# HamidGadirov/OpticalFlowSciVis

Measured on AMD Instinct MI355X. Metric: volume-pairs/sec, Flow-3D unsupervised train step (fwd+loss+bwd+AdamW), higher is better.
Workload: dtype f32

## Files before the change

### include/flowsci_hip.h

```cpp
#ifndef FLOWSCI_HIP_H
#define FLOWSCI_HIP_H

#ifdef __cplusplus
extern "C" {
#endif

typedef void* fs_stream_t;

enum {
  FS_OK = 0,
  FS_ERR_NULLPTR = 1,
  FS_ERR_SHAPE = 2,
  FS_ERR_ARG = 3,
  FS_ERR_LAUNCH = 4,
  FS_ERR_UNSUPPORTED = 5
};

#define FS_ABI_VERSION 460
int fs_version(void);
const char* fs_error_string(int code);

int fs_warp3d_fwd(const float* in, const float* flow, float* out,
                  int B, int C, const int* in_dhw, int D, int H, int W, fs_stream_t stream);
int fs_warp3d_bwd(const float* in, const float* flow, const float* grad_out,
                  float* grad_in, float* grad_flow,
                  int B, int C, const int* in_dhw, int D, int H, int W, fs_stream_t stream);

int fs_warp3d_pair_fwd(const float* img0, const float* img1, const float* flow6,
                       float* out0, float* out1,
                       int B, int C, const int* in_dhw, int D, int H, int W, fs_stream_t stream);
int fs_warp3d_pair_bwd(const float* img0, const float* img1, const float* flow6,
                       const float* grad_out0, const float* grad_out1,
                       float* grad_img0, float* grad_img1, float* grad_flow6,
                       int B, int C, const int* in_dhw, int D, int H, int W, fs_stream_t stream);
int fs_warp3d_pair_bwd_acc(const float* img0, const float* img1, const float* flow6,
                           const float* grad_out0, const float* grad_out1,
                           float* grad_img0, float* grad_img1,
                           const float* grad_flow_add, float* grad_flow6,
                           int B, int C, const int* in_dhw, int D, int H, int W, fs_stream_t stream);

int fs_upsample_warp3d_pair_fwd(const float* img0, const float* img1, const float* delta,
                                const float* prev_flow, float* flow_out, float* out0, float* out1,
                                int B, int C, const int* in_dhw, int Ds, int Hs, int Ws, int factor,
                                float scale, fs_stream_t stream);
int fs_upsample_warp3d_pair_bwd(const float* img0, const float* img1, const float* flow6,
                                const float* grad_out0, const float* grad_out1,
                                const float* grad_flow_add, float* grad_flow_total, float* grad_delta,
                                float* ws, int B, int C, const int* in_dhw, int Ds, int Hs, int Ws,
                                int factor, float scale, fs_stream_t stream);
int fs_warp3d_pair_bwd_acc3(const float* img0, const float* img1, const float* flow6,
                            const float* grad_out0, long long gout_batch_stride0, const float* grad_out1,
                            long long gout_batch_stride1, float* grad_img0, float* grad_img1,
                            const float* add0, long long batch_stride0, const float* add1, long long batch_stride1,
                            const float* add2, long long batch_stride2, float* grad_flow6,
                            int B, int C, const int* in_dhw, int D, int H, int W, fs_stream_t stream);
int fs_upsample_warp3d_pair_bwd3(const float* img0, const float* img1, const float* flow6,
                                 const float* grad_out0, long long gout_batch_stride0, const float* grad_out1,
                                 long long gout_batch_stride1, const float* add0, long long batch_stride0, const float* add1, long long batch_stride1,
                                 const float* add2, long long batch_stride2, float* grad_flow_total, float* grad_delta,
                                 float* ws, int B, int C, const int* in_dhw, int Ds, int Hs, int Ws,
                                 int factor, float scale, fs_stream_t stream);

enum { FS_W3_KERNEL_GATHER = 0, FS_W3_KERNEL_RC = 1 };
int fs_warp3d_kernel_id(const float* in0, const float* in1, const float* flow, int B, int C, const int* in_dhw,
                        int D, int H, int W, int backward, int with_grad_in);

enum { FS_WARP2D_RIFE = 0, FS_WARP2D_PWC = 1, FS_WARP2D_PHOTO = 2, FS_WARP2D_DILATED = 3 };

int fs_warp2d_fwd(const float* in, const float* flow, const float* start, float* out,
                  int B, int C, const int* in_hw, int H, int W, int mode, int with_mask,
                  fs_stream_t stream);
int fs_warp2d_bwd(const float* in, const float* flow, const float* start,
                  const float* grad_out, float* grad_in, float* grad_flow,
                  int B, int C, const int* in_hw, int H, int W, int mode, int with_mask,
                  fs_stream_t stream);

int fs_warp2d_pair_fwd(const float* img0, const float* img1, const float* flow4,
                       float* out0, float* out1,
                       int B, int C, const int* in_hw, int H, int W, int mode, fs_stream_t stream);
int fs_warp2d_pair_bwd(const float* img0, const float* img1, const float* flow4,
                       const float* grad_out0, const float* grad_out1,
                       float* grad_img0, float* grad_img1, float* grad_flow4,
                       int B, int C, const int* in_hw, int H, int W, int mode, fs_stream_t stream);

enum { FS_OCC_ALL = 0, FS_OCC_OBJ = 1, FS_OCC_OUT = 2 };
int fs_occ_check2d(const float* flow_f, const float* flow_b, float* occ_f, float* occ_b,
                   int B, int H, int W, float alpha1, float alpha2_over_scale, int mode,
                   fs_stream_t stream);

int fs_corr2d_fwd(const float* f1, const float* f2, float* out,
                  int B, int C, int H, int W, int max_displacement, fs_stream_t stream);
int fs_corr2d_bwd(const float* f1, const float* f2, const float* grad_out,
                  float* grad_f1, float* grad_f2,
                  int B, int C, int H, int W, int max_displacement, fs_stream_t stream);

int fs_plane_moments(const float* f, float* stats, int planes, int S, fs_stream_t stream);
int fs_plane_norm_bwd(const float* f, const float* stats, const float* grad_n, float* grad_f,
                      int planes, int S, fs_stream_t stream);
int fs_corr2d_norm_fwd(const float* f1, const float* f2, const float* stats1, const float* stats2,
                       float* out, int B, int C, int H, int W, int max_displacement,
                       fs_stream_t stream);
int fs_corr2d_norm_bwd(const float* f1, const float* f2, const float* stats1, const float* stats2,
                       const float* grad_out, float* grad_n1, float* grad_n2,
                       int B, int C, int H, int W, int max_displacement, fs_stream_t stream);

int fs_corr2d_pair_fwd(const float* f1a, const float* f2a, const float* f1b, const float* f2b,
                       const float* stats, float* outa, float* outb,
                       int B, int C, int H, int W, int max_displacement, fs_stream_t stream);
int fs_corr2d_pair_bwd(const float* f1a, const float* f2a, const float* f1b, const float* f2b,
                       const float* stats, const float* grad_outa, const float* grad_outb,
                       float* grad_f1a, float* grad_f2a, float* grad_f1b, float* grad_f2b,
                       int B, int C, int H, int W, int max_displacement, fs_stream_t stream);
int fs_plane_moments4(const float* fa, const float* fb, const float* fc, const float* fd, float* stats,
                      int planes, int S, fs_stream_t stream);
int fs_plane_norm_bwd4(const float* fa, const float* fb, const float* fc, const float* fd,
                       const float* stats, const float* grad_na, const float* grad_nb,
                       const float* grad_nc, const float* grad_nd, float* grad_fa, float* grad_fb,
                       float* grad_fc, float* grad_fd, int planes, int S, fs_stream_t stream);

int fs_corr3d_fwd(const float* f1, const float* f2, float* out,
                  int B, int C, int D, int H, int W, int max_displacement, fs_stream_t stream);
int fs_corr3d_bwd(const float* f1, const float* f2, const float* grad_out,
                  float* grad_f1, float* grad_f2,
                  int B, int C, int D, int H, int W, int max_displacement, fs_stream_t stream);

enum { FS_PEN_ABS_ROBUST = 0, FS_PEN_CHARBONNIER = 1, FS_PEN_L1_EPS = 2, FS_PEN_L1 = 3 };
#define FS_REDUCE_BLOCKS 1024

int fs_robust_sum(const float* x, const float* y, const float* w, float* sums, float* ws,
                  int B, int C, int S, int H, int W, int border, int mode, float q, float eps,
                  fs_stream_t stream);
int fs_robust_sum_bwd(const float* x, const float* y, const float* w, const float* coef,
                      float* grad_x, float* grad_y,
                      int B, int C, int S, int H, int W, int border, int mode, float q, float eps,
                      fs_stream_t stream);

int fs_wssim_fwd(const float* x, const float* y, const float* weight, float* sums, float* ws,
                 int B, int C, int H, int W, int use_occ, fs_stream_t stream);
int fs_wssim_bwd(const float* x, const float* y, const float* weight, const float* coef,
                 float* grad_x, float* grad_y, int B, int C, int H, int W, int use_occ,
                 fs_stream_t stream);

int fs_census_dist_fwd(const float* img1, const float* img2, float* dist,
                       int B, int H, int W, int max_distance, fs_stream_t stream);
int fs_census_dist_bwd(const float* img1, const float* img2, const float* grad_dist,
                       float* grad_img1, float* grad_img2,
                       int B, int H, int W, int max_distance, fs_stream_t stream);

int fs_merge_fwd(const float* w0, const float* w1, const float* mask_logit,
                 float* merged, float* sigmoid_out, int B, int C, int S, fs_stream_t stream);
int fs_merge_bwd(const float* w0, const float* w1, const float* mask_logit,
                 const float* grad_merged, const float* grad_sigmoid,
                 float* grad_w0, float* grad_w1, float* grad_mask_logit,
                 int B, int C, int S, fs_stream_t stream);
int fs_distill_fwd(const float* merged_i, const float* merged_tea, const float* gt,
                   const float* flow_i, const float* flow_tea, float* sums, float* ws,
                   int B, int C, int F, int S, fs_stream_t stream);
int fs_distill_bwd(const float* merged_i, const float* merged_tea, const float* gt,
                   const float* flow_i, const float* flow_tea, const float* coef,
                   float* grad_flow_i, int B, int C, int F, int S, fs_stream_t stream);
int fs_distill3_fwd(const float* merged0, const float* merged1, const float* merged2,
                    const float* merged_tea, const float* gt, const float* flow0, const float* flow1,
                    const float* flow2, const float* flow_tea, float* sums, float* ws,
                    int B, int C, int F, int S, fs_stream_t stream);
int fs_distill3_bwd(const float* merged0, const float* merged1, const float* merged2,
                    const float* merged_tea, const float* gt, const float* flow0, const float* flow1,
                    const float* flow2, const float* flow_tea, const float* coef,
                    float* grad_flow0, float* grad_flow1, float* grad_flow2,
                    int B, int C, int F, int S, fs_stream_t stream);

int fs_interp3d_bwd(const float* grad_out, float* grad_in, float* ws, int B, int C,
                    int Din, int Hin, int Win, int Dout, int Hout, int Wout,
                    int factor, int upsample, fs_stream_t stream);
int fs_interp3d_bwd_scaled(const float* grad_out, float* grad_in, float* ws, int B, int C,
                           int Din, int Hin, int Win, int Dout, int Hout, int Wout,
                           int factor, int upsample, float scale, fs_stream_t stream);

int fs_downsample3d_fwd(const float* in, float* out, int B, int C, int Din, int Hin, int Win,
                        int factor, float scale, fs_stream_t stream);
int fs_downsample3d_fwd_ms(const float* const* src, const long long* batch_strides, float* out, int B, int C,
                           int Din, int Hin, int Win, int factor, float scale, fs_stream_t stream);

int fs_resize2d_fwd(const float* in, float* out, int B, int C, int Hin, int Win, int Hout, int Wout,
                    int factor, int upsample, float scale, fs_stream_t stream);
int fs_resize2d_bwd(const float* grad_out, float* grad_in, int B, int C, int Hin, int Win, int Hout,
                    int Wout, int factor, int upsample, float scale, fs_stream_t stream);

int fs_upsample3d_scale_add(const float* small, const float* prev, float* out, int B, int C,
                            int Din, int Hin, int Win, int factor, float scale, fs_stream_t stream);

int fs_laploss2d_sizes(int N, int H, int W, int levels, long long* sgn_floats,
                       long long* ws_fwd_floats, long long* ws_bwd_floats);
int fs_laploss2d_fwd(const float* input, const float* target, float* sgn, float* ws, float* loss,
                     int N, int H, int W, int levels, fs_stream_t stream);
int fs_laploss2d_bwd(const float* sgn, const float* grad_loss, float* ws, float* grad_diff,
                     int N, int H, int W, int levels, fs_stream_t stream);

int fs_laploss3d_sizes(int N, int D, int H, int W, int levels, long long* sgn_floats,
                       long long* ws_fwd_floats, long long* ws_bwd_floats);
int fs_laploss3d_fwd(const float* input, const float* target, float* sgn, float* ws, float* loss,
                     int N, int D, int H, int W, int levels, fs_stream_t stream);
int fs_laploss3d_bwd(const float* sgn, const float* grad_loss, float* ws, float* grad_diff,
                     int N, int D, int H, int W, int levels, fs_stream_t stream);

long long fs_conv3d_fwd_ws_floats(int Cin, int Cout, int kernel);
int fs_conv3d_fwd(const float* x, const float* w, const float* bias, float* y, float* ws,
                  int B, int Cin, int Cout, int Di, int Hi, int Wi, int Do, int Ho, int Wo,
                  int kernel, int stride, int pad, int wmode, fs_stream_t stream);

int fs_conv3d_fwd_add(const float* x, const float* w, const float* bias, const float* addend, float* y,
                      float* ws, int B, int Cin, int Cout, int Di, int Hi, int Wi, int Do, int Ho, int Wo,
                      int kernel, int stride, int pad, int wmode, fs_stream_t stream);
long long fs_conv3d_fwd_dprelu_part_floats(int B, int Cout, int Do, int Ho, int Wo);
long long fs_conv3d_fwd_dprelu_part_floats_k3(int B, int Cout, int Do, int Ho, int Wo);
int fs_conv3d_fwd_dprelu(const float* x, const float* w, const float* act_y, const float* prelu_weight,
                         int num_prelu_weights, float* grad_act_y, float* grad_prelu_weight, float* grad_bias,
                         float* part, float* ws, int B, int Cin, int Cout, int Di, int Hi, int Wi, int Do, int Ho, int Wo,
                         int kernel, int stride, int pad, fs_stream_t stream);
int fs_conv3d_fwd_prelu(const float* x, const float* w, const float* bias, const float* prelu_weight,
                        const float* residual, float* y, float* z, float* ws,
                        int B, int Cin, int Cout, int Di, int Hi, int Wi, int Do, int Ho, int Wo,
                        int kernel, int stride, int pad, int num_prelu_weights, fs_stream_t stream);
int fs_conv3d_tr_prelu(const float* x, const float* w, const float* bias, const float* prelu_weight,
                       float* y, float* z, float* ws,
                       int B, int Cin, int Cout, int Di, int Hi, int Wi, int Dout, int Hout, int Wout,
                       int num_prelu_weights, fs_stream_t stream);
int fs_conv3d_tr_add(const float* x, const float* w, const float* bias, const float* addend, float* y,
                     float* ws, int B, int Cin, int Cout, int Di, int Hi, int Wi,
                     int Dout, int Hout, int Wout, fs_stream_t stream);
long long fs_conv3d_tr_ws_floats(int Cin, int Cout);
int fs_conv3d_tr(const float* x, const float* w, const float* bias, float* y, float* ws,
                 int B, int Cin, int Cout, int Di, int Hi, int Wi, int Dout, int Hout, int Wout,
                 fs_stream_t stream);

#define FS_PRELU_MAX_CHUNKS 64
int fs_prelu_bwd(const float* x, const float* grad_out, const float* weight,
                 float* grad_x, float* grad_weight, float* grad_bias, float* ws,
                 int B, int C, int S, int num_weights, fs_stream_t stream);

int fs_conv3d_wrw(const float* g, const float* src, float* dw, int B, int Cg, int Cs,
                  int Do, int Ho, int Wo, int Di, int Hi, int Wi,
                  int kernel, int stride, int pad, fs_stream_t stream);
enum { FS_WRW_KERNEL_BRICK = 0,
       FS_WRW_KERNEL_DMA = 1,
       FS_WRW_KERNEL_WINO23 = 2,
       FS_WRW_KERNEL_WINO43 = 3,
       FS_WRW_KERNEL_S3 = 4        };
int fs_conv3d_wrw_kernel_id(const float* g, const float* src, int B, int Cg, int Cs,
                            int Do, int Ho, int Wo, int Di, int Hi, int Wi, int kernel, int stride, int pad);

int fs_conv3d_fwd_prelu_ms(const float* const* src, const long long* batch_strides, const float* w, const float* bias,
                           const float* prelu_weight, float* y, float* z, float* ws,
                           int B, int Cin, int Cout, int Di, int Hi, int Wi, int Do, int Ho, int Wo,
                           int kernel, int stride, int pad, int num_prelu_weights, fs_stream_t stream);
int fs_conv3d_wrw_ms(const float* g, const float* const* src, const long long* batch_strides, float* dw,
                     int B, int Cg, int Cs, int Do, int Ho, int Wo, int Di, int Hi, int Wi,
                     int kernel, int stride, int pad, fs_stream_t stream);

long long fs_conv3d_wrw_det_ws_floats(const float* g, const float* src, const float* const* src_planes,
                                      const long long* batch_strides, int B, int Cg, int Cs,
                                      int Do, int Ho, int Wo, int Di, int Hi, int Wi, int kernel, int stride, int pad);
int fs_conv3d_wrw_det(const float* g, const float* src, const float* const* src_planes, const long long* batch_strides,
                      float* dw, float* ws, long long ws_floats, int B, int Cg, int Cs,
                      int Do, int Ho, int Wo, int Di, int Hi, int Wi, int kernel, int stride, int pad,
                      fs_stream_t stream);

typedef struct FsWprepJob {
  const float* w;
  float* ws;
  int kind;
  int total;
  int p[6];
} FsWprepJob;
int fs_conv3d_fwd_wprep_jobs(FsWprepJob* jobs_host, int cap, const float* x, const float* w, float* ws,
                             int B, int Cin, int Cout, int Di, int Hi, int Wi, int Do, int Ho, int Wo,
                             int kernel, int stride, int pad, int wmode);
int fs_conv3d_tr_wprep_jobs(FsWprepJob* jobs_host, int cap, const float* x, const float* w, float* ws, int B, int Cin,
                            int Cout, int Di, int Hi, int Wi, int Dout, int Hout, int Wout, int has_prelu_out);
int fs_conv3d_wprep_batch(const FsWprepJob* jobs_dev, int njobs, fs_stream_t stream);

long long fs_frame_metrics2d_ws_bytes(int N, int C, int H, int W);
long long fs_frame_metrics3d_ws_bytes(int N, int C, int D, int H, int W);
int fs_frame_metrics2d(const float* x, const float* y, int N, int C, int H, int W, double L, double* ws,
                       double* out_sse, double* out_ssim_sum, fs_stream_t stream);
int fs_frame_metrics3d(const float* x, const float* y, int N, int C, int D, int H, int W, double L, double* ws,
                       double* out_sse, double* out_ssim_sum, fs_stream_t stream);

#define FS_FLOW_METRICS_K 13
#define FS_FM_MAX_EPE 5
enum { FS_FLOW_DISP = 0, FS_FLOW_RIFE3D = 1 };
long long fs_flow_metrics2d_ws_bytes(int N, int C, int H, int W);
long long fs_flow_metrics3d_ws_bytes(int N, int C, int D, int H, int W, int convention);
int fs_flow_metrics2d(const float* pred, const float* gt, int N, int C, int H, int W, long long pred_bstride,
                      long long gt_bstride, const unsigned char* valid, const unsigned char* noc, float tau_abs,
                      float tau_rel, float* epe_map, double* ws, double* out, fs_stream_t stream);
int fs_flow_metrics3d(const float* pred, const float* gt, int N, int C, int D, int H, int W, long long pred_bstride,
                      long long gt_bstride, const unsigned char* valid, const unsigned char* noc, int convention,
                      float tau_abs, float tau_rel, float* epe_map, double* ws, double* out, fs_stream_t stream);

#define FS_FLOW_CONSISTENCY_K 13
#define FS_FC_MAX_R 7
enum { FS_FC_NOT_VALID = 0, FS_FC_CONSISTENT = 1, FS_FC_OCCLUDED = 2, FS_FC_OUTGOING = 3, FS_FC_NONFINITE = 4 };
long long fs_flow_consistency2d_ws_bytes(int N, int C, int H, int W);
long long fs_flow_consistency3d_ws_bytes(int N, int C, int D, int H, int W);
int fs_flow_consistency2d(const float* flow_f, const float* flow_b, int N, int C, int H, int W, long long f_bstride,
                          long long b_bstride, const float* img0, const float* img1, const unsigned char* valid,
                          double alpha1, double alpha2, unsigned char* class_map, float* res_map, double* ws,
                          double* out, fs_stream_t stream);
int fs_flow_consistency3d(const float* flow_f, const float* flow_b, int N, int C, int D, int H, int W,
                          long long f_bstride, long long b_bstride, const float* img0, const float* img1,
                          const unsigned char* valid, double alpha1, double alpha2, unsigned char* class_map,
                          float* res_map, double* ws, double* out, fs_stream_t stream);

enum { FS_ADV_ALIVE = 0, FS_ADV_OUT = 1, FS_ADV_NONFINITE = 2 };
enum { FS_ADV_EULER = 0, FS_ADV_RK2 = 1, FS_ADV_RK4 = 2 };
int fs_advect2d(const float* flows, int K, int C, int H, int W, long long flow_sstride, const float* pos_in,
                long long pos_cstride, long long P, float* traj, long long traj_sstride, long long traj_cstride,
                unsigned char* status, int* steps, int method, int substeps, double scale, fs_stream_t stream);
int fs_advect3d(const float* flows, int K, int C, int D, int H, int W, long long flow_sstride, const float* pos_in,
                long long pos_cstride, long long P, float* traj, long long traj_sstride, long long traj_cstride,
                unsigned char* status, int* steps, int method, int substeps, double scale, fs_stream_t stream);

#define FS_FTLE_K 9
#define FS_FTLE_MIN 7
#define FS_FTLE_MAX 8
enum { FS_FTLE_NOT_VALID = 0, FS_FTLE_OK = 1, FS_FTLE_ENDED = 2, FS_FTLE_NONFINITE = 3, FS_FTLE_COLLAPSED = 4 };
long long fs_ftle2d_ws_bytes(int C, int Gh, int Gw);
long long fs_ftle3d_ws_bytes(int C, int Gd, int Gh, int Gw);
int fs_ftle2d(const float* map, long long map_cstride, const unsigned char* status, const unsigned char* valid, int C,
              int Gh, int Gw, const double* inv_h, const double* inv_2h, double inv_T, int accept_out, float* ftle,
              unsigned char* cls, float* cg, double* ws, double* out, fs_stream_t stream);
int fs_ftle3d(const float* map, long long map_cstride, const unsigned char* status, const unsigned char* valid, int C,
              int Gd, int Gh, int Gw, const double* inv_h, const double* inv_2h, double inv_T, int accept_out,
              float* ftle, unsigned char* cls, float* cg, double* ws, double* out, fs_stream_t stream);

enum { FS_VG_DIV = 1, FS_VG_VORT = 2, FS_VG_VMAG = 4, FS_VG_Q = 8, FS_VG_L2 = 16, FS_VG_J = 32, FS_VG_ALL = 63 };
enum { FS_VG_FLAG_Q = 1, FS_VG_FLAG_L2 = 2, FS_VG_FLAG_NONFINITE = 128 };
#define FS_VG_K 20
#define FS_VG_STEPS_PER_LAUNCH 256
long long fs_velgrad2d_ws_bytes(int K, int C, int H, int W);
long long fs_velgrad3d_ws_bytes(int K, int C, int D, int H, int W);
int fs_velgrad2d(const float* flows, int K, int C, int H, int W, long long flow_sstride, const double* inv_h,
                 const double* inv_2h, const double* scale, unsigned fields, float* out, unsigned char* flags,
                 double* ws, double* summary, fs_stream_t stream);
int fs_velgrad3d(const float* flows, int K, int C, int D, int H, int W, long long flow_sstride, const double* inv_h,
                 const double* inv_2h, const double* scale, unsigned fields, float* out, unsigned char* flags,
                 double* ws, double* summary, fs_stream_t stream);

#define FS_REGION_TILE2_H 32
#define FS_REGION_TILE2_W 64
#define FS_REGION_TILE3_D 8
#define FS_REGION_TILE3_H 8
#define FS_REGION_TILE3_W 32
#define FS_REGION_MAX_WEIGHTS 8
#define FS_REGION_STEPS_PER_LAUNCH 32768
#define FS_REGION_FOLLOW_MAX_EXTENT 16777216
enum { FS_REGION_OUT = -1, FS_REGION_TO_BACKGROUND = -2 };
long long fs_label_regions2d_ws_bytes(int K, int H, int W);
long long fs_label_regions3d_ws_bytes(int K, int D, int H, int W);
int fs_label_regions2d(const unsigned char* mask, int K, int H, int W, long long mask_sstride, int require, int reject,
                       int conn, int* labels, int* n_regions, int* status, int* ws, fs_stream_t stream);
int fs_label_regions3d(const unsigned char* mask, int K, int D, int H, int W, long long mask_sstride, int require,
                       int reject, int conn, int* labels, int* n_regions, int* status, int* ws, fs_stream_t stream);
int fs_region_stats2d(const int* labels, const int* rank, const long long* offsets, const float* weights, int K, int F,
                      int H, int W, long long R, long long* count, long long* coord_sum, int* bbox, double* wsum,
                      float* wmin, float* wmax, fs_stream_t stream);
int fs_region_stats3d(const int* labels, const int* rank, const long long* offsets, const float* weights, int K, int F,
                      int D, int H, int W, long long R, long long* count, long long* coord_sum, int* bbox, double* wsum,
                      float* wmin, float* wmax, fs_stream_t stream);
int fs_region_follow2d(const int* labels, const float* flows, int K, int C, int H, int W, long long flow_sstride,
                       int* dst, fs_stream_t stream);
int fs_region_follow3d(const int* labels, const float* flows, int K, int C, int D, int H, int W, long long flow_sstride,
                       int* dst, fs_stream_t stream);

enum { FS_RC_DVR = 0, FS_RC_MIP = 1 };
#define FS_RC_BRICK 8
#define FS_RC_MAX_TF 1024
#define FS_RC_MAX_STEPS 4194304
int fs_brick_range3d(const float* volumes, int K, int D, int H, int W, long long sstride, float* range,
// ... 60 lines not shown
```

### opticalflowscivis_amd/_lib.py

```python
import ctypes
import os

import torch

_HERE = os.path.dirname(os.path.abspath(__file__))
PRODUCT_LIB_PATH = os.path.join(_HERE, "csrc", "libflowsci_hip.so")
LIB_PATH = os.environ.get("FLOWSCI_HIP_LIBRARY") or PRODUCT_LIB_PATH
ABLATION = LIB_PATH != PRODUCT_LIB_PATH


def ablation_env(name):
    return os.environ.get(name) if ABLATION else None


def switches():
    return {"library": "ablation build: " + LIB_PATH if ABLATION else "product",
            "env": {k: v for k, v in sorted(os.environ.items()) if k.startswith("FLOWSCI_")}}

ABI_VERSION = 460

_f32p = ctypes.c_void_p
_int = ctypes.c_int
_uint = ctypes.c_uint
_float = ctypes.c_float
_stream = ctypes.c_void_p
_intp = ctypes.POINTER(ctypes.c_int)
_i64p = ctypes.POINTER(ctypes.c_longlong)
_i64 = ctypes.c_longlong
_ptrv = ctypes.POINTER(ctypes.c_void_p)
_double = ctypes.c_double
_f64p = ctypes.POINTER(ctypes.c_double)

class FsWprepJob(ctypes.Structure):
    _fields_ = [("w", ctypes.c_void_p), ("ws", ctypes.c_void_p), ("kind", ctypes.c_int), ("total", ctypes.c_int),
                ("p", ctypes.c_int * 6)]


_jobp = ctypes.POINTER(FsWprepJob)

SIGNATURES = {
    "fs_version": [],
    "fs_error_string": [_int],
    "fs_warp3d_fwd": [_f32p] * 3 + [_int, _int, _intp, _int, _int, _int, _stream],
    "fs_warp3d_bwd": [_f32p] * 5 + [_int, _int, _intp, _int, _int, _int, _stream],
    "fs_warp3d_pair_fwd": [_f32p] * 5 + [_int, _int, _intp, _int, _int, _int, _stream],
    "fs_warp3d_pair_bwd": [_f32p] * 8 + [_int, _int, _intp, _int, _int, _int, _stream],
    "fs_warp3d_pair_bwd_acc": [_f32p] * 9 + [_int, _int, _intp, _int, _int, _int, _stream],
    "fs_warp3d_pair_bwd_acc3": [_f32p] * 3 + [_f32p, _i64, _f32p, _i64] + [_f32p] * 2 + [_f32p, _i64, _f32p, _i64, _f32p, _i64, _f32p, _int, _int, _intp, _int, _int,
                                _int, _stream],
    "fs_upsample_warp3d_pair_bwd3": [_f32p] * 3 + [_f32p, _i64, _f32p, _i64] + [_f32p, _i64, _f32p, _i64, _f32p, _i64] + [_f32p] * 3 +
                                    [_int, _int, _intp, _int, _int, _int, _int, _float, _stream],
    "fs_upsample_warp3d_pair_fwd": [_f32p] * 7 + [_int, _int, _intp, _int, _int, _int, _int, _float, _stream],
    "fs_upsample_warp3d_pair_bwd": [_f32p] * 9 + [_int, _int, _intp, _int, _int, _int, _int, _float, _stream],
    "fs_warp2d_pair_fwd": [_f32p] * 5 + [_int, _int, _intp, _int, _int, _int, _stream],
    "fs_warp2d_pair_bwd": [_f32p] * 8 + [_int, _int, _intp, _int, _int, _int, _stream],
    "fs_interp3d_bwd_scaled": [_f32p] * 3 + [_int] * 10 + [_float, _stream],
    "fs_downsample3d_fwd": [_f32p] * 2 + [_int] * 6 + [_float, _stream],
    "fs_downsample3d_fwd_ms": [_ptrv, _i64p, _f32p] + [_int] * 6 + [_float, _stream],
    "fs_resize2d_fwd": [_f32p] * 2 + [_int] * 8 + [_float, _stream],
    "fs_resize2d_bwd": [_f32p] * 2 + [_int] * 8 + [_float, _stream],
    "fs_occ_check2d": [_f32p] * 4 + [_int] * 3 + [_float, _float, _int, _stream],
    "fs_laploss2d_sizes": [_int] * 4 + [_i64p] * 3,
    "fs_laploss2d_fwd": [_f32p] * 5 + [_int] * 4 + [_stream],
    "fs_laploss2d_bwd": [_f32p] * 4 + [_int] * 4 + [_stream],
    "fs_laploss3d_sizes": [_int] * 5 + [_i64p] * 3,
    "fs_laploss3d_fwd": [_f32p] * 5 + [_int] * 5 + [_stream],
    "fs_laploss3d_bwd": [_f32p] * 4 + [_int] * 5 + [_stream],
    "fs_conv3d_fwd_ws_floats": [_int] * 3,
    "fs_conv3d_fwd": [_f32p] * 5 + [_int] * 13 + [_stream],
    "fs_upsample3d_scale_add": [_f32p] * 3 + [_int] * 6 + [_float, _stream],
    "fs_conv3d_fwd_dprelu_part_floats": [_int] * 5,
    "fs_conv3d_fwd_dprelu_part_floats_k3": [_int] * 5,
    "fs_conv3d_fwd_dprelu": [_f32p] * 4 + [_int] + [_f32p] * 5 + [_int] * 12 + [_stream],
    "fs_conv3d_fwd_prelu": [_f32p] * 8 + [_int] * 13 + [_stream],
    "fs_conv3d_fwd_add": [_f32p] * 6 + [_int] * 13 + [_stream],
    "fs_conv3d_tr_prelu": [_f32p] * 7 + [_int] * 10 + [_stream],
    "fs_conv3d_tr_add": [_f32p] * 6 + [_int] * 9 + [_stream],
    "fs_conv3d_tr_ws_floats": [_int] * 2,
    "fs_conv3d_tr": [_f32p] * 5 + [_int] * 9 + [_stream],
    "fs_plane_moments": [_f32p] * 2 + [_int] * 2 + [_stream],
    "fs_plane_norm_bwd": [_f32p] * 4 + [_int] * 2 + [_stream],
    "fs_corr2d_norm_fwd": [_f32p] * 5 + [_int] * 5 + [_stream],
    "fs_corr2d_norm_bwd": [_f32p] * 7 + [_int] * 5 + [_stream],
    "fs_corr2d_pair_fwd": [_f32p] * 7 + [_int] * 5 + [_stream],
    "fs_corr2d_pair_bwd": [_f32p] * 11 + [_int] * 5 + [_stream],
    "fs_plane_moments4": [_f32p] * 5 + [_int] * 2 + [_stream],
    "fs_plane_norm_bwd4": [_f32p] * 13 + [_int] * 2 + [_stream],
    "fs_corr2d_fwd": [_f32p] * 3 + [_int] * 5 + [_stream],
    "fs_corr2d_bwd": [_f32p] * 5 + [_int] * 5 + [_stream],
    "fs_robust_sum": [_f32p] * 5 + [_int] * 7 + [_float, _float, _stream],
    "fs_robust_sum_bwd": [_f32p] * 6 + [_int] * 7 + [_float, _float, _stream],
    "fs_census_dist_fwd": [_f32p] * 3 + [_int] * 4 + [_stream],
    "fs_census_dist_bwd": [_f32p] * 5 + [_int] * 4 + [_stream],
    "fs_merge_fwd": [_f32p] * 5 + [_int] * 3 + [_stream],
    "fs_merge_bwd": [_f32p] * 8 + [_int] * 3 + [_stream],
    "fs_distill3_fwd": [_f32p] * 11 + [_int] * 4 + [_stream],
    "fs_distill3_bwd": [_f32p] * 13 + [_int] * 4 + [_stream],
    "fs_distill_fwd": [_f32p] * 7 + [_int] * 4 + [_stream],
    "fs_distill_bwd": [_f32p] * 7 + [_int] * 4 + [_stream],
    "fs_interp3d_bwd": [_f32p] * 3 + [_int] * 10 + [_stream],
    "fs_prelu_bwd": [_f32p] * 7 + [_int] * 4 + [_stream],
    "fs_corr3d_fwd": [_f32p] * 3 + [_int] * 6 + [_stream],
    "fs_corr3d_bwd": [_f32p] * 5 + [_int] * 6 + [_stream],
    "fs_conv3d_wrw": [_f32p] * 3 + [_int] * 12 + [_stream],
    "fs_conv3d_wrw_kernel_id": [_f32p] * 2 + [_int] * 12,
    "fs_warp3d_kernel_id": [_f32p] * 3 + [_int, _int, _intp] + [_int] * 5,
    "fs_conv3d_wrw_det_ws_floats": [_f32p, _f32p, _ptrv, _i64p] + [_int] * 12,
    "fs_conv3d_wrw_det": [_f32p, _f32p, _ptrv, _i64p, _f32p, _f32p, _i64] + [_int] * 12 + [_stream],
    "fs_conv3d_fwd_prelu_ms": [_ptrv, _i64p] + [_f32p] * 6 + [_int] * 13 + [_stream],
    "fs_conv3d_wrw_ms": [_f32p, _ptrv, _i64p, _f32p] + [_int] * 12 + [_stream],
    "fs_wssim_fwd": [_f32p] * 5 + [_int] * 5 + [_stream],
    "fs_wssim_bwd": [_f32p] * 6 + [_int] * 5 + [_stream],
    "fs_conv3d_fwd_wprep_jobs": [_jobp, _int, _f32p, _f32p, _f32p] + [_int] * 13,
    "fs_conv3d_tr_wprep_jobs": [_jobp, _int, _f32p, _f32p, _f32p] + [_int] * 10,
    "fs_conv3d_wprep_batch": [_f32p, _int, _stream],
    "fs_warp2d_fwd": [_f32p, _f32p, _f32p, _f32p, _int, _int, _intp, _int, _int, _int, _int, _stream],
    "fs_warp2d_bwd": [_f32p, _f32p, _f32p, _f32p, _f32p, _f32p, _int, _int, _intp, _int, _int, _int, _int,
                      _stream],
    "fs_frame_metrics2d_ws_bytes": [_int] * 4,
    "fs_frame_metrics3d_ws_bytes": [_int] * 5,
    "fs_frame_metrics2d": [_f32p] * 2 + [_int] * 4 + [_double] + [_f32p] * 3 + [_stream],
    "fs_frame_metrics3d": [_f32p] * 2 + [_int] * 5 + [_double] + [_f32p] * 3 + [_stream],
    "fs_flow_metrics2d_ws_bytes": [_int] * 4,
    "fs_flow_metrics3d_ws_bytes": [_int] * 6,
    "fs_flow_metrics2d": [_f32p] * 2 + [_int] * 4 + [_i64] * 2 + [_f32p] * 2 + [_float] * 2 + [_f32p] * 3 + [_stream],
    "fs_flow_metrics3d": [_f32p] * 2 + [_int] * 5 + [_i64] * 2 + [_f32p] * 2 + [_int] + [_float] * 2 + [_f32p] * 3 +
                         [_stream],
    "fs_flow_consistency2d_ws_bytes": [_int] * 4,
    "fs_flow_consistency3d_ws_bytes": [_int] * 5,
    "fs_flow_consistency2d": [_f32p] * 2 + [_int] * 4 + [_i64] * 2 + [_f32p] * 3 + [_double] * 2 + [_f32p] * 4 + [_stream],
    "fs_flow_consistency3d": [_f32p] * 2 + [_int] * 5 + [_i64] * 2 + [_f32p] * 3 + [_double] * 2 + [_f32p] * 4 + [_stream],
    "fs_advect2d": [_f32p, _int, _int, _int, _int, _i64, _f32p, _i64, _i64, _f32p, _i64, _i64, _f32p, _f32p, _int, _int,
                    _double, _stream],
    "fs_advect3d": [_f32p, _int, _int, _int, _int, _int, _i64, _f32p, _i64, _i64, _f32p, _i64, _i64, _f32p, _f32p, _int,
                    _int, _double, _stream],
    "fs_ftle2d_ws_bytes": [_int] * 3,
    "fs_ftle3d_ws_bytes": [_int] * 4,
    "fs_ftle2d": [_f32p, _i64, _f32p, _f32p] + [_int] * 3 + [_f64p, _f64p, _double, _int] + [_f32p] * 5 + [_stream],
    "fs_ftle3d": [_f32p, _i64, _f32p, _f32p] + [_int] * 4 + [_f64p, _f64p, _double, _int] + [_f32p] * 5 + [_stream],
    "fs_velgrad2d_ws_bytes": [_int] * 4,
    "fs_velgrad3d_ws_bytes": [_int] * 5,
    "fs_velgrad2d": [_f32p] + [_int] * 4 + [_i64, _f64p, _f64p, _f64p, _uint] + [_f32p] * 4 + [_stream],
    "fs_velgrad3d": [_f32p] + [_int] * 5 + [_i64, _f64p, _f64p, _f64p, _uint] + [_f32p] * 4 + [_stream],
    "fs_label_regions2d_ws_bytes": [_int] * 3,
    "fs_label_regions3d_ws_bytes": [_int] * 4,
    "fs_label_regions2d": [_f32p] + [_int] * 3 + [_i64] + [_int] * 3 + [_f32p] * 4 + [_stream],
    "fs_label_regions3d": [_f32p] + [_int] * 4 + [_i64] + [_int] * 3 + [_f32p] * 4 + [_stream],
    "fs_region_stats2d": [_f32p] * 4 + [_int] * 4 + [_i64] + [_f32p] * 6 + [_stream],
    "fs_region_stats3d": [_f32p] * 4 + [_int] * 5 + [_i64] + [_f32p] * 6 + [_stream],
    "fs_region_follow2d": [_f32p] * 2 + [_int] * 4 + [_i64, _f32p, _stream],
    "fs_region_follow3d": [_f32p] * 2 + [_int] * 5 + [_i64, _f32p, _stream],
    "fs_brick_range3d": [_f32p] + [_int] * 4 + [_i64, _f32p, _f32p, _stream],
    "fs_raycast3d_ws_bytes": [_int] * 4,
    "fs_raycast3d": [_f32p] + [_int] * 4 + [_i64, _f32p, _f32p, _int, _double, _double, _double, _f64p, _int, _double,
                     _int, _int] + [_f32p] * 5 + [_stream],
    "fs_iso3d_ws_bytes": [_int] * 4,
    "fs_iso_count3d": [_f32p] + [_int] * 4 + [_i64, _double, _f32p, _stream],
    "fs_iso_emit3d": [_f32p] + [_int] * 4 + [_i64, _double, _f64p, _f32p, _f32p, _i64, _i64, _f32p, _int] + [_f32p] * 5 +
                     [_stream],
    "fs_lic2d_ws_bytes": [_int] * 3,
    "fs_lic3d_ws_bytes": [_int] * 4,
    "fs_lic2d": [_f32p, _int, _int, _int, _int, _i64, _f32p, _i64, _f32p, _int, _double, _double, _int, _f32p, _f32p, _f32p,
                 _f32p, _stream],
    "fs_lic3d": [_f32p, _int, _int, _int, _int, _int, _i64, _f32p, _i64, _f32p, _int, _double, _double, _int, _f32p, _f32p,
                 _f32p, _f32p, _stream],
    "fs_triplet_gather": [_f32p, _int, _i64, _int, _int, _int, _f32p, _int, _int, _int, _int, _f32p, _stream],
    "fs_series_stats_ws_bytes": [_int, _i64],
    "fs_series_stats": [_f32p, _int, _int, _i64, _f32p, _f32p, _stream],
    "fs_series_encode_ws_bytes": [_int] * 5,
    "fs_series_encode": [_f32p] + [_int] * 5 + [_f32p] + [_int] * 4 + [_float, _float, _f32p, _f32p, _stream],
    "fs_census3d_dist_fwd": [_f32p] * 3 + [_int] * 5 + [_stream],
    "fs_census3d_dist_bwd": [_f32p] * 5 + [_int] * 5 + [_stream],
    "fs_flow_smooth3d_fwd": [_f32p] * 4 + [_int] * 5 + [_float] * 3 + [_stream],
    "fs_flow_smooth3d_bwd": [_f32p] * 4 + [_int] * 5 + [_float] * 3 + [_stream],
}
_RESTYPES = {"fs_error_string": ctypes.c_char_p, "fs_conv3d_fwd_ws_floats": ctypes.c_longlong,
             "fs_conv3d_wrw_det_ws_floats": ctypes.c_longlong,
             "fs_frame_metrics2d_ws_bytes": ctypes.c_longlong, "fs_frame_metrics3d_ws_bytes": ctypes.c_longlong,
             "fs_flow_metrics2d_ws_bytes": ctypes.c_longlong, "fs_flow_metrics3d_ws_bytes": ctypes.c_longlong,
             "fs_flow_consistency2d_ws_bytes": ctypes.c_longlong, "fs_flow_consistency3d_ws_bytes": ctypes.c_longlong,
             "fs_ftle2d_ws_bytes": ctypes.c_longlong, "fs_ftle3d_ws_bytes": ctypes.c_longlong,
             "fs_velgrad2d_ws_bytes": ctypes.c_longlong, "fs_velgrad3d_ws_bytes": ctypes.c_longlong,
             "fs_label_regions2d_ws_bytes": ctypes.c_longlong, "fs_label_regions3d_ws_bytes": ctypes.c_longlong,
             "fs_raycast3d_ws_bytes": ctypes.c_longlong, "fs_iso3d_ws_bytes": ctypes.c_longlong,
             "fs_lic2d_ws_bytes": ctypes.c_longlong, "fs_lic3d_ws_bytes": ctypes.c_longlong,
             "fs_series_stats_ws_bytes": ctypes.c_longlong, "fs_series_encode_ws_bytes": ctypes.c_longlong,
             "fs_conv3d_tr_ws_floats": ctypes.c_longlong, "fs_conv3d_fwd_dprelu_part_floats": ctypes.c_longlong,
             "fs_conv3d_fwd_dprelu_part_floats_k3": ctypes.c_longlong}


class FlowsciLibraryError(RuntimeError):
    pass


class FlowsciKernelError(RuntimeError):
    pass


_lib = None


def lib():
    global _lib
    if _lib is not None:
        return _lib
    if not os.path.exists(LIB_PATH):
        raise FlowsciLibraryError(
            "libflowsci_hip.so not found at %s -- build it with "
            "`python -c 'import __graft_entry__ as g; g.build()'` or "
            "`make -C opticalflowscivis_amd/csrc`.  There is no CPU fallback." % LIB_PATH)
    handle = ctypes.CDLL(LIB_PATH)
    for name, argtypes in SIGNATURES.items():
        try:
            fn = getattr(handle, name)
        except AttributeError as e:
            raise FlowsciLibraryError("libflowsci_hip.so does not export %s" % name) from e
        fn.argtypes = argtypes
        fn.restype = _RESTYPES.get(name, _int)
    got = handle.fs_version()
    if got != ABI_VERSION:
        raise FlowsciLibraryError(
            "libflowsci_hip.so at %s reports ABI version %d, this binding was written for %d: argument lists "
            "differ between them (include/flowsci_hip.h, FS_ABI_VERSION) -- rebuild with "
            "`make -C opticalflowscivis_amd/csrc`" % (LIB_PATH, got, ABI_VERSION))
    _lib = handle
    return _lib


def check(code, what):
    if code != 0:
        msg = lib().fs_error_string(code)
        raise FlowsciKernelError("%s failed: %s (code %d)" % (what, msg.decode() if msg else "?", code))
```

### opticalflowscivis_amd/convgrad.py

```python
import os

import torch
import torch.nn as nn
import torch.nn.functional as F


def _tuple(v, nd):
    return tuple(v) if isinstance(v, (tuple, list)) else (v,) * nd


_stock_seen = set()


def _note_stock_path(what, x, w, stride, padding):
    if x.dim() != 5 or not x.is_cuda or x.dtype != torch.float32:
        return
    key = (what, tuple(x.shape[1:]), tuple(w.shape), tuple(stride), tuple(padding))
    if key in _stock_seen:
        return
    _stock_seen.add(key)
    import warnings
    warnings.warn("opticalflowscivis_amd: %s of a 3-D convolution runs on stock ATen / MIOpen kernels, not on the HIP "
                  "implicit-GEMM kernels (input %s, weight %s, stride %s, padding %s: unsupported geometry or beyond "
                  "32-bit offsets)" % (what, tuple(x.shape), tuple(w.shape), tuple(stride), tuple(padding)),
# ... 74 lines not shown
    _note_stock_path("the input gradient", gy, w, stride, padding)
    return torch.ops.aten.convolution_backward(
        gy, x, w, None, list(stride), list(padding), [1] * nd, transposed, [0] * nd, 1,
        [True, False, False])[0]


def _conv_grad_weight(x, w, gy, stride, padding, transposed):
    k = tuple(w.shape[2:])
    nd = x.dim() - 2
    src, g = (gy, x) if transposed else (x, gy)
    if nd == 3 and src.is_cuda and src.dtype == torch.float32:
        from . import ops
        if ops.conv3d_wrw_supported(k, stride, padding) and ops.conv3d_wrw_fits(src.shape[2:], g.shape[2:]):
            return ops.conv3d_wrw(g, src, k[0], stride[0], padding[0])
    _note_stock_path("the weight gradient", x, w, stride, padding)
    return torch.ops.aten.convolution_backward(
        gy, x, w, None, list(stride), list(padding), [1] * nd, transposed, [0] * nd, 1,
        [False, True, False])[1]


class _ConvFn(torch.autograd.Function):
    @staticmethod
    def forward(ctx, x, w, b, stride, padding, transposed):
        y = _conv_forward(x, w, b, stride, padding, transposed)
        ctx.save_for_backward(x, w)
        ctx.cfg = (stride, padding, transposed, b is not None)
        return y

    @staticmethod
    def backward(ctx, gy):
        x, w = ctx.saved_tensors
        stride, padding, transposed, has_bias = ctx.cfg
        nd = x.dim() - 2
        gy = gy.contiguous()
        gx = gw = gb = None
        if ctx.needs_input_grad[0]:
            gx = _conv_grad_input(x, w, gy, stride, padding, transposed)
        if ctx.needs_input_grad[1]:
            gw = _conv_grad_weight(x, w, gy, stride, padding, transposed)
        if has_bias and ctx.needs_input_grad[2]:
            gb = gy.sum(dim=(0,) + tuple(range(2, 2 + nd)))
        return gx, gw, gb, None, None, None


class _ConvTrAddFn(torch.autograd.Function):

    @staticmethod
    def forward(ctx, x, w, b, addend, stride, padding):
        from . import ops
        y = ops.conv3d_tr(x, w, b, None, None, addend)
        ctx.save_for_backward(x, w)
        ctx.cfg = (stride, padding, b is not None)
        return y

    @staticmethod
    def backward(ctx, gy):
        x, w = ctx.saved_tensors
        stride, padding, has_bias = ctx.cfg
        gy = gy.contiguous()
        gx = gw = gb = None
        if ctx.needs_input_grad[0]:
            gx = _conv_grad_input(x, w, gy, stride, padding, True)
        if ctx.needs_input_grad[1]:
            gw = _conv_grad_weight(x, w, gy, stride, padding, True)
        if has_bias and ctx.needs_input_grad[2]:
            gb = gy.sum(dim=(0, 2, 3, 4))
        return gx, gw, gb, (gy if ctx.needs_input_grad[3] else None), None, None


class _ConvPReLUFn(torch.autograd.Function):

    @staticmethod
    def forward(ctx, x, w, b, a, stride, padding, transposed):
        y, z = _conv_forward(x, w, b, stride, padding, transposed, a)
        ctx.save_for_backward(x, w, y, a)
        ctx.cfg = (stride, padding, transposed, b is not None)
        return z

    @staticmethod
    def backward(ctx, gz):
        from . import ops
        x, w, y, a = ctx.saved_tensors
        stride, padding, transposed, has_bias = ctx.cfg
        gy, ga, gb = ops.prelu_backward(y, gz.contiguous(), a, want_bias_grad=has_bias)
        gx = gw = None
        if ctx.needs_input_grad[0]:
            gx = _conv_grad_input(x, w, gy, stride, padding, transposed)
        if ctx.needs_input_grad[1]:
            gw = _conv_grad_weight(x, w, gy, stride, padding, transposed)
        return gx, gw, gb, ga, None, None, None


class _ConvPReLUCatFn(torch.autograd.Function):

    @staticmethod
    def forward(ctx, w, b, a, stride, padding, *pieces):
        from . import ops
        k = w.shape[2]
        res = ops.conv3d_fwd_prelu_ms(pieces, w, b, a, k, stride[0], padding[0])
        ctx.ms = res is not None
        if res is None:
            x = torch.cat(pieces, 1)
            y, z = _conv_forward(x, w, b, stride, padding, False, a)
            ctx.save_for_backward(w, y, a, x)
        else:
            y, z = res
            ctx.save_for_backward(w, y, a, *pieces)
        ctx.cfg = (stride, padding, b is not None, [int(t.shape[1]) for t in pieces])
        return z

    @staticmethod
    def backward(ctx, gz):
        from . import ops
        w, y, a = ctx.saved_tensors[:3]
        src = ctx.saved_tensors[3:]
        stride, padding, has_bias, splits = ctx.cfg
        gy, ga, gb = ops.prelu_backward(y, gz.contiguous(), a, want_bias_grad=has_bias)
        need = ctx.needs_input_grad[5:]
        gx = None
        if any(need):
            k3 = tuple(w.shape[2:])
            hip = _hip_tr_ok(gy, w.shape[1], k3, stride, padding) and all(
                n in (2 * m, 2 * m + 1) for n, m in zip(src[0].shape[2:], gy.shape[2:]))
            gx = _conv_grad_input(src[0] if (hip or not ctx.ms) else torch.cat(src, 1), w, gy, stride, padding, False)
        gw = None
        if ctx.needs_input_grad[0]:
            if ctx.ms:
                gw = ops.conv3d_wrw_ms(gy, src, w.shape[2], stride[0], padding[0])
                if gw is None:
                    gw = _conv_grad_weight(torch.cat(src, 1), w, gy, stride, padding, False)
            else:
                gw = _conv_grad_weight(src[0], w, gy, stride, padding, False)
        gp = [None] * len(splits)
        if gx is not None:
            gp = [g if n else None for g, n in zip(gx.split(splits, 1), need)]
        return (gw, gb, ga, None, None) + tuple(gp)


def conv_prelu_cat(block, pieces):
    conv, act = block[0], block[1]
    x0 = pieces[0]
    if _ab_env("FLOWSCI_CONV0_CAT") == "1":
        return None
    if not (_hip_autograd(x0) and x0.dim() == 5 and x0.dtype == torch.float32 and isinstance(conv, Conv3d)
            and act.weight.numel() in (1, conv.out_channels) and conv.groups == 1
            and _tuple(conv.dilation, 3) == (1, 1, 1) and conv.padding_mode == "zeros"
            and tuple(conv.weight.shape[2:]) == (4, 4, 4) and _tuple(conv.stride, 3) == (2, 2, 2)
            and sum(int(t.shape[1]) for t in pieces) == conv.in_channels <= 12 and conv.out_channels <= 32):
        return None
    return _ConvPReLUCatFn.apply(conv.weight, conv.bias, act.weight, _tuple(conv.stride, 3), _tuple(conv.padding, 3),
                                 *pieces)


class _HeadFn(torch.autograd.Function):

    @staticmethod
    def forward(ctx, x, w1, b1, a1, w2, b2, addend):
        from . import ops
        y1, z1 = ops.conv3d_tr(x, w1, b1, None, a1)
        out = ops.conv3d_tr(z1, w2, b2, None, None, addend)
        ctx.save_for_backward(x, w1, a1, y1, z1, w2)
        ctx.has = (b1 is not None, b2 is not None, addend is not None)
        return out

    @staticmethod
    def backward(ctx, gout):
        from . import ops
        x, w1, a1, y1, z1, w2 = ctx.saved_tensors
        s3, p3 = (2, 2, 2), (1, 1, 1)
        gout = gout.contiguous()
        gw2 = _conv_grad_weight(z1, w2, gout, s3, p3, True) if ctx.needs_input_grad[4] else None
        gb2 = gout.sum(dim=(0, 2, 3, 4)) if (ctx.has[1] and ctx.needs_input_grad[5]) else None
        fused = ops.conv3d_deconv_grad_input_dprelu(gout, w2, y1, a1)
        if fused is not None:
            gy1, ga1, gb1 = fused
        else:
            gz1 = _conv_grad_input(z1, w2, gout, s3, p3, True)
            gy1, ga1, gb1 = ops.prelu_backward(y1, gz1, a1, want_bias_grad=ctx.has[0])
        if not ctx.has[0]:
            gb1 = None
        gw1 = _conv_grad_weight(x, w1, gy1, s3, p3, True) if ctx.needs_input_grad[1] else None
        gx = _conv_grad_input(x, w1, gy1, s3, p3, True) if ctx.needs_input_grad[0] else None
        return gx, gw1, gb1, ga1, gw2, gb2, (gout if (ctx.has[2] and ctx.needs_input_grad[6]) else None)


def head_fused_ok(head, x, addend):
    d1, act, d2 = head[0], head[1], head[2]
    if not (_hip_autograd(x) and x.dim() == 5 and x.dtype == torch.float32 and isinstance(d1, ConvTranspose3d)
            and isinstance(d2, ConvTranspose3d) and isinstance(act, nn.PReLU)):
        return False
    for d in (d1, d2):
        if not (_tuple(d.kernel_size, 3) == (4, 4, 4) and _tuple(d.stride, 3) == (2, 2, 2) and _tuple(d.padding, 3) == (1, 1, 1)
                and d.groups == 1 and _tuple(d.dilation, 3) == (1, 1, 1) and _tuple(d.output_padding, 3) == (0, 0, 0)):
            return False
    if act.weight.numel() not in (1, d1.out_channels):
        return False
    if not (_hip_tr_ok(x, d1.out_channels, (4, 4, 4), (2, 2, 2), (1, 1, 1))):
        return False
    mid = tuple(2 * n for n in x.shape[2:])
    from . import ops
    return ops.conv3d_tr_supported(d2.out_channels, (4, 4, 4), (2, 2, 2), (1, 1, 1)) and ops.conv3d_tr_fits(mid) and \
        (addend is None or (addend.is_cuda and addend.dtype == torch.float32))


_FUSE_2D = _ab_env("FLOWSCI_CONV2D_UNFUSED") != "1"


class ConvPReLU(nn.Sequential):

    def forward(self, x):
        conv, act = self[0], self[1]
        nd = x.dim() - 2
        kinds = {3: (Conv3d, ConvTranspose3d), 2: (nn.Conv2d, nn.ConvTranspose2d) if _FUSE_2D else ()}.get(nd, ())
        if (_hip_autograd(x) and x.dtype == torch.float32 and kinds and isinstance(conv, kinds)
                and act.weight.numel() in (1, conv.out_channels) and conv.groups == 1
                and _tuple(conv.dilation, nd) == (1,) * nd and getattr(conv, "padding_mode", "zeros") == "zeros"
                and _tuple(getattr(conv, "output_padding", 0), nd) == (0,) * nd):
            return _ConvPReLUFn.apply(x, conv.weight, conv.bias, act.weight, _tuple(conv.stride, nd),
                                      _tuple(conv.padding, nd), isinstance(conv, kinds[1]))
        return act(conv(x))


class _ResUnitFn(torch.autograd.Function):

    @staticmethod
    def forward(ctx, x, w1, b1, a1, w2, b2, a2):
        from . import ops
        k, p = w1.shape[2], (w1.shape[2] - 1) // 2
        y1, z1 = ops.conv3d_fwd(x, w1, b1, k, 1, p, 0, a1)
        y2, out = ops.conv3d_fwd(z1, w2, b2, k, 1, p, 0, a2, x)
        ctx.save_for_backward(x, w1, a1, y1, z1, w2, a2, y2)
        ctx.has_bias = (b1 is not None, b2 is not None)
        return out

    @staticmethod
    def backward(ctx, gout):
        from . import ops
        x, w1, a1, y1, z1, w2, a2, y2 = ctx.saved_tensors
        k, p = w1.shape[2], (w1.shape[2] - 1) // 2
        s3, p3 = (1, 1, 1), (p, p, p)
        gout = gout.contiguous()
        gy2, ga2, gb2 = ops.prelu_backward(y2, gout, a2, want_bias_grad=ctx.has_bias[1])
        gw2 = _conv_grad_weight(z1, w2, gy2, s3, p3, False) if ctx.needs_input_grad[4] else None
        fused = ops.conv3d_k3_grad_input_dprelu(gy2, w2, y1, a1) if k == 3 else None
        if fused is not None:
            gy1, ga1, gb1 = fused
            if not ctx.has_bias[0]:
                gb1 = None
        else:
            gz1 = ops.conv3d_fwd(gy2, w2, None, k, 1, p, 1)
            gy1, ga1, gb1 = ops.prelu_backward(y1, gz1, a1, want_bias_grad=ctx.has_bias[0])
        gw1 = _conv_grad_weight(x, w1, gy1, s3, p3, False) if ctx.needs_input_grad[1] else None
        gx = ops.conv3d_fwd(gy1, w1, None, k, 1, p, 1, None, gout) if ctx.needs_input_grad[0] else None
        return gx, gw1, gb1, ga1, gw2, gb2, ga2


def res_unit(block, x):
    ok = (_hip_autograd(x) and x.dim() == 5 and x.dtype == torch.float32 and len(block) == 2 and
          all(isinstance(m, ConvPReLU) and isinstance(m[0], Conv3d) and isinstance(m[1], nn.PReLU) for m in block))
    if ok:
        for m in block:
            c = m[0]
            kk = tuple(c.weight.shape[2:])
            ok = ok and (kk == (3, 3, 3) and _tuple(c.stride, 3) == (1, 1, 1) and _tuple(c.padding, 3) == (1, 1, 1)
                         and c.groups == 1 and _tuple(c.dilation, 3) == (1, 1, 1) and c.padding_mode == "zeros"
                         and c.in_channels == c.out_channels == x.shape[1]
                         and m[1].weight.numel() in (1, c.out_channels)
                         and _hip_fwd_ok(x, c.out_channels, x.shape[2:], kk, (1, 1, 1), (1, 1, 1)))
    if not ok:
        return block(x) + x
    (c1, p1), (c2, p2) = block[0], block[1]
    return _ResUnitFn.apply(x, c1.weight, c1.bias, p1.weight, c2.weight, c2.bias, p2.weight)


def _hip_autograd(x):
    return x.is_cuda and torch.is_grad_enabled()


class Conv3d(nn.Conv3d):
    def forward(self, x):
        if not _hip_autograd(x):
            st, pd, k = _tuple(self.stride, 3), _tuple(self.padding, 3), tuple(self.weight.shape[2:])
            if x.dim() == 5 and self.padding_mode == "zeros" and self.groups == 1 and _tuple(self.dilation, 3) == (1, 1, 1) \
                    and _hip_fwd_ok(x, self.weight.shape[0], [_conv_out(n, kk, s, p) for n, kk, s, p in
                                                              zip(x.shape[2:], k, st, pd)], k, st, pd):
                from . import ops
                return ops.conv3d_fwd(x, self.weight, None if self.bias is None else self.bias.detach(),
                                      k[0], st[0], pd[0], 0)
            return super().forward(x)
        return _ConvFn.apply(x, self.weight, self.bias, _tuple(self.stride, 3), _tuple(self.padding, 3), False)


class ConvTranspose3d(nn.ConvTranspose3d):
    def _plain(self):
        return (self.groups == 1 and _tuple(self.dilation, 3) == (1, 1, 1) and
                _tuple(self.output_padding, 3) == (0, 0, 0))

    def forward(self, x, addend=None):
        st, pd, k = _tuple(self.stride, 3), _tuple(self.padding, 3), tuple(self.weight.shape[2:])
        hip = x.dim() == 5 and self._plain() and _hip_tr_ok(x, self.weight.shape[1], k, st, pd)
        if addend is not None:
            if hip and tuple(addend.shape[2:]) == tuple(2 * n for n in x.shape[2:]) and \
                    addend.shape[1] == self.weight.shape[1] and addend.dtype == torch.float32:
                if _hip_autograd(x):
                    return _ConvTrAddFn.apply(x, self.weight, self.bias, addend, st, pd)
                from . import ops
# ... 19 lines not shown
```

### opticalflowscivis_amd/csrc/convfwd.hip

```cpp
#include <cstdint>
#include <cstdlib>
#include <type_traits>

#include "common.hpp"

namespace {

typedef float f32x16 __attribute__((ext_vector_type(16)));

struct FP {
  int B, Cin, Cout, CoutP;
  int Di, Hi, Wi, Do, Ho, Wo;
  int pad;
  int tz, ty, tx;
  long long tiles;
  const float* slope;
  float* Z;
  int nslope;
  const float* addend;
  const float* dy;
  const float* dslope;
  int dnslope;
  float* dpart;
  int nsrc;
// ... 244 lines not shown
#pragma unroll
    for (int k = 0; k < NXW; ++k) {
      const int i = 256 * (wv + 4 * k) + 4 * lane;
      const int c = i / CHS, r1 = i - c * CHS;
      const int z = r1 / PS, r2 = r1 - z * PS;
      const int y = r2 / XP, x = r2 - y * XP;
      const int gz = gz0 + z, gy = gy0 + y, gx = gx0 + x;
      const bool ok = i < NX && gz >= 0 && gz < p.Di && gy >= 0 && gy < p.Hi && gx >= 0 && gx < p.Wi;
      xoff[k] = ok ? (((unsigned)gz * p.Hi + gy) * p.Wi + gx) * 4u : DMA_OOB;
      xch[k] = i < NX ? c : CI - 1;
    }
#pragma unroll
    for (int k = 0; k < NWW; ++k) {
      const int i = 256 * (wv + 4 * k) + 4 * lane;
      const int row = i / CP, j = i - row * CP;
      woff[k] = i < NW ? ((unsigned)row * (unsigned)p.CoutP + (unsigned)j) * 4u : DMA_OOB;
    }
    auto stage = [&](int c0, int buf) {
      __amdgpu_buffer_rsrc_t rx[CI];
#pragma unroll
      for (int c = 0; c < CI; ++c) {
        const int ch = c0 + c;
        const bool live = ch < p.Cin;
        const int chc = live ? ch : 0;
        const float* base = p.nsrc ? p.src[chc] + (size_t)b * (size_t)p.sbs[chc]
                                   : X + ((size_t)b * p.Cin + chc) * xvol;
        rx[c] = __builtin_amdgcn_make_buffer_rsrc((void*)base, (short)0, live ? (int)((unsigned)xvol * 4u) : 0, 0x00020000);
      }
      __amdgpu_buffer_rsrc_t rw = __builtin_amdgcn_make_buffer_rsrc(
          (void*)(Wt + (size_t)c0 * K3 * p.CoutP + co0), (short)0, 0x7fffffff, 0x00020000);
      float* base = lds + buf * BUF;
#pragma unroll
      for (int k = 0; k < NXW; ++k)
        if (256 * (wv + 4 * k) < NXL) {
#pragma unroll
          for (int c = 0; c < CI; ++c)
            if (256 * (wv + 4 * k) < (c + 1) * CHS && 256 * (wv + 4 * k) + 256 > c * CHS)
              if (xch[k] == c)
                __builtin_amdgcn_raw_ptr_buffer_load_lds(rx[c], (lds_ptr_t)(base + 256 * (wv + 4 * k)), 16, xoff[k], 0, 0, 0);
        }
#pragma unroll
      for (int k = 0; k < NWW; ++k)
        if (256 * (wv + 4 * k) < NWL)
          __builtin_amdgcn_raw_ptr_buffer_load_lds(rw, (lds_ptr_t)(base + NXL + 256 * (wv + 4 * k)), 16, woff[k], 0, 0, 0);
    };
    stage(0, 0);
    asm volatile("s_waitcnt vmcnt(0)" ::: "memory");
    __builtin_amdgcn_s_barrier();
    int buf = 0;
    for (int c0 = 0; c0 < p.Cin; c0 += CI) {
      if (c0 + CI < p.Cin) stage(c0 + CI, buf ^ 1);
      asm volatile("s_waitcnt vmcnt(0)" ::: "memory");
      __builtin_amdgcn_s_barrier();
      buf ^= 1;
    }
#else
    (void)xvol; (void)NXW; (void)NWW; (void)DMA_OOB;
#endif
    return;
  }

  const int ly = col / TW, lx = col % TW;
  const int rr0 = wv * NT;
  const int wz = rr0 / TY, wy = rr0 % TY;
  const int bBo = kh * (CI / 2) * CHS + (wz * S) * PS + ((wy * R + ly) * S) * XP + lx * S + XL - p.pad;
  const int aBo = NXL + kh * (CI / 2) * K3 * CP + col;

  f32x16 acc[MT][NT];
#pragma unroll
  for (int m = 0; m < MT; ++m)
#pragma unroll
    for (int n = 0; n < NT; ++n)
#pragma unroll
      for (int r = 0; r < 16; ++r) acc[m][n][r] = 0.f;

  __builtin_amdgcn_s_barrier();
  int buf = 0;
  for (int c0 = 0; c0 < p.Cin; c0 += CI) {
    const float* bB = lds + buf * BUF + bBo;
    const float* aB = lds + buf * BUF + aBo;
    auto lds_ops = [&](int j, float (&a)[MT], float (&bq)[NT]) {
      const int cl = j / K3, tap = j - cl * K3;
      const int kz = tap / (K * K), ky = (tap / K) % K, kx = tap % K;
#pragma unroll
      for (int m = 0; m < MT; ++m) a[m] = aB[(cl * K3 + tap) * CP + m * 32];
#pragma unroll
      for (int n = 0; n < NT; ++n) bq[n] = bB[cl * CHS + kz * PS + (ky + n * R * S) * XP + kx];
    };
    auto mma = [&](const float (&a)[MT], const float (&bq)[NT]) {
#pragma unroll
      for (int n = 0; n < NT; ++n)
#pragma unroll
        for (int m = 0; m < MT; ++m)
          acc[m][n] = __builtin_amdgcn_mfma_f32_32x32x2f32(a[m], bq[n], acc[m][n], 0, 0, 0);
    };
    float a0[MT], b0[NT], a1[MT], b1[NT];
    lds_ops(0, a0, b0);
#pragma unroll
    for (int j = 0; j < NP; j += 2) {
      if (j + 1 < NP) lds_ops(j + 1, a1, b1);
      __builtin_amdgcn_sched_barrier(0);
#ifdef FS_ABLATION
      if (p.ab & 8) continue;
#endif
      mma(a0, b0);
      if (j + 2 < NP) lds_ops(j + 2, a0, b0);
      __builtin_amdgcn_sched_barrier(0);
      if (j + 1 < NP) mma(a1, b1);
    }
    __builtin_amdgcn_s_barrier();
    buf ^= 1;
  }

#include "convfwd_epilogue.hpp"
}

#ifdef FS_ABLATION
#include "convwino.hpp"
#include "convwino4.hpp"
#endif
#include "convwino2d.hpp"
#include "convfwd_s3.hpp"

template <int K, int S, int CI, int MT, int NT, int TZ, int TY, int TW>
int launch_ws(const float* X, const float* Wt, const float* bias, float* Y, FP& p, hipStream_t st) {
  constexpr int TYR = TY * (32 / TW);
  p.tz = fs::cdiv(p.Do, TZ); p.ty = fs::cdiv(p.Ho, TYR); p.tx = fs::cdiv(p.Wo, TW);
  p.tiles = (long long)p.B * p.tz * p.ty * p.tx;
  const int mgroups = p.CoutP / (32 * MT);
  if (p.tiles >= (1ll << 31) || mgroups > 65535) return FS_ERR_SHAPE;
#ifdef FS_ABLATION
  static const int fwd_ab = (int)FS_AB_ENV_LL("FLOWSCI_FWD_AB", 0);
  p.ab = fwd_ab;
#endif
  hipLaunchKernelGGL((conv3d_fwd_ws_kernel<K, S, CI, MT, NT, TZ, TY, TW>), dim3((unsigned)p.tiles, mgroups),
                     dim3(512), 0, st, X, Wt, bias, Y, p);
  FS_LAUNCH_CHECK();
  return FS_OK;
}

template <int K, int S, int CI, int MT, int NT, int TZ, int TY, int TW>
int launch(const float* X, const float* Wt, const float* bias, float* Y, FP& p, hipStream_t st) {
  constexpr int TYR = TY * (32 / TW);
  p.tz = fs::cdiv(p.Do, TZ); p.ty = fs::cdiv(p.Ho, TYR); p.tx = fs::cdiv(p.Wo, TW);
  p.tiles = (long long)p.B * p.tz * p.ty * p.tx;
  const int mgroups = p.CoutP / (32 * MT);
  if (p.tiles >= (1ll << 31) || mgroups > 65535) return FS_ERR_SHAPE;
  hipLaunchKernelGGL((conv3d_fwd_kernel<K, S, CI, MT, NT, TZ, TY, TW>), dim3((unsigned)p.tiles, mgroups),
                     dim3(256), 0, st, X, Wt, bias, Y, p);
  FS_LAUNCH_CHECK();
  return FS_OK;
}

constexpr int kFinishBlocks = 128;
__global__ __launch_bounds__(256) void dprelu_finish1_kernel(const float* __restrict__ part, int rows, int CP,
                                                             double* __restrict__ partial) {
  const int CP2 = 2 * CP;
  const int col = threadIdx.x % CP2, sub = threadIdx.x / CP2, nsub = 256 / CP2;
  const int chunk = (rows + kFinishBlocks - 1) / kFinishBlocks;
  const int r0 = blockIdx.x * chunk, r1 = min(rows, r0 + chunk);
  const float* src = part + (size_t)blockIdx.y * rows * CP2;
  double s = 0.0;
  for (int r = r0 + sub; r < r1; r += nsub) s += (double)src[(size_t)r * CP2 + col];
  __shared__ double red[256];
  red[threadIdx.x] = s;
  __syncthreads();
  if (sub == 0) {
    double t = red[col];
    for (int k = 1; k < nsub; ++k) t += red[k * CP2 + col];
    partial[((size_t)blockIdx.y * kFinishBlocks + blockIdx.x) * CP2 + col] = t;
  }
}
__global__ __launch_bounds__(64) void dprelu_finish2_kernel(const double* __restrict__ partial, int CP, int Cout,
                                                            float* __restrict__ ga, float* __restrict__ gb, int nslope) {
  const bool bias_blk = (int)blockIdx.x >= nslope;
  const int c = bias_blk ? blockIdx.x - nslope : blockIdx.x;
  const bool all = !bias_blk && nslope == 1 && Cout != 1;
  const int c_lo = all ? 0 : c, c_hi = all ? Cout : c + 1;
  double s = 0.0;
  for (int cc = c_lo; cc < c_hi; ++cc) {
    const double* src = partial + (size_t)(cc / CP) * kFinishBlocks * 2 * CP + (cc % CP) * 2 + (bias_blk ? 1 : 0);
    for (int g = threadIdx.x; g < kFinishBlocks; g += 64) s += src[(size_t)g * 2 * CP];
  }
  __shared__ double red[64];
  red[threadIdx.x] = s;
  __syncthreads();
  for (int st = 32; st > 0; st >>= 1) {
    if ((int)threadIdx.x < st) red[threadIdx.x] += red[threadIdx.x + st];
    __syncthreads();
  }
  if (threadIdx.x == 0) (bias_blk ? gb : ga)[c] = (float)red[0];
}

void wt_dims(int Cin, int Cout, int kernel, int* CinP, int* CoutP) {
  const int ci = (kernel == 3) ? 4 : 2;
  *CinP = (Cin + ci - 1) / ci * ci;
  *CoutP = (Cout <= 32 && kernel == 4) ? 32 : (Cout + 63) / 64 * 64;
}

}

extern "C" long long fs_conv3d_fwd_ws_floats(int Cin, int Cout, int kernel) {
  if (Cin < 1 || Cout < 1 || (kernel != 3 && kernel != 4)) return -1;
  int cinp, coutp;
  wt_dims(Cin, Cout, kernel, &cinp, &coutp);
  const long long direct = (long long)cinp * kernel * kernel * kernel * coutp;
  constexpr int wino_uch = FS_WINO2D_UCH > FS_WINO4_UCH ? FS_WINO2D_UCH : (FS_WINO4_UCH > FS_WINO_UCH ? FS_WINO4_UCH : FS_WINO_UCH);
  const long long wino = (kernel == 3 && coutp == 64) ? (long long)cinp * wino_uch : 0;
  const long long s3 = (kernel == 4 && coutp <= 64) ? s3_slab_words(Cin, coutp) : 0;
  const long long m = direct > wino ? direct : wino;
  return m > s3 ? m : s3;
}

struct DPrelu {
  const float* act_y = nullptr;
  const float* slope = nullptr;
  int nslope = 0;
  float* part = nullptr;
  float* ga = nullptr;
  float* gb = nullptr;
};

struct MultiSrc {
  const float* const* src;
  const long long* batch_strides;
};

static int conv3d_fwd_impl(const float* x, const float* w, const float* bias, const float* slope, int nslope,
                           const float* addend, float* y, float* z, float* ws, int B, int Cin, int Cout, int Di, int Hi, int Wi, int Do,
                           int Ho, int Wo, int kernel, int stride, int pad, int wmode, fs_stream_t stream,
                           const DPrelu* dp = nullptr, const MultiSrc* ms = nullptr, WprepPlan* plan = nullptr) {
  if (ms == nullptr && plan == nullptr) FS_REQUIRE_PTR(x);
  if (plan == nullptr) FS_REQUIRE_PTR(y);
  FS_REQUIRE_PTR(ws);
  if (z != nullptr && (slope == nullptr || (nslope != 1 && nslope != Cout))) return FS_ERR_ARG;
  if ((((uintptr_t)y | (uintptr_t)z | (uintptr_t)addend | (uintptr_t)(dp ? dp->act_y : nullptr)) & 15) != 0) return FS_ERR_ARG;
  if (B < 1 || Cin < 1 || Cout < 1 || Di < 1 || Hi < 1 || Wi < 1 || Do < 1 || Ho < 1 || Wo < 1)
    return FS_ERR_SHAPE;
  if (!((kernel == 3 && stride == 1) || (kernel == 4 && stride == 2)) || pad < 0 || pad >= kernel ||
      (wmode != 0 && wmode != 1))
    return FS_ERR_ARG;
  if (Do != (Di + 2 * pad - kernel) / stride + 1 || Ho != (Hi + 2 * pad - kernel) / stride + 1 ||
      Wo != (Wi + 2 * pad - kernel) / stride + 1)
    return FS_ERR_SHAPE;
  if ((long long)Di * Hi * Wi >= (1ll << 31) || (long long)Do * Ho * Wo >= (1ll << 31)) return FS_ERR_SHAPE;
  if ((long long)(kernel == 3 ? 4 : 2) * Di * Hi * Wi * 4 >= (1ll << 32)) return FS_ERR_SHAPE;
  FP p;
  p.B = B; p.Cin = Cin; p.Cout = Cout; p.Di = Di; p.Hi = Hi; p.Wi = Wi; p.Do = Do; p.Ho = Ho; p.Wo = Wo;
  p.pad = pad;
  p.slope = slope; p.Z = z; p.nslope = nslope; p.addend = addend;
  p.dy = dp ? dp->act_y : nullptr; p.dslope = dp ? dp->slope : nullptr; p.dnslope = dp ? dp->nslope : 0;
  p.dpart = dp ? dp->part : nullptr;
  p.nsrc = 0;
  bool ms_aligned = true;
  if (ms != nullptr) {
    if (Cin > 12) return FS_ERR_UNSUPPORTED;
    p.nsrc = Cin;
    const long long vol = (long long)Di * Hi * Wi;
    for (int c = 0; c < Cin; ++c) {
      if (ms->src[c] == nullptr) return FS_ERR_NULLPTR;
      if (ms->batch_strides[c] < vol) return FS_ERR_ARG;
      p.src[c] = ms->src[c]; p.sbs[c] = ms->batch_strides[c];
      ms_aligned = ms_aligned && ((uintptr_t)ms->src[c] & 15) == 0 && ms->batch_strides[c] % 4 == 0;
    }
  }
  int cinp;
  wt_dims(Cin, Cout, kernel, &cinp, &p.CoutP);
  hipStream_t st = (hipStream_t)stream;
  auto dp_finish = [&](int CP, int rows_per_brick = 4) {
    const long long rows = p.tiles * rows_per_brick;
    const int mg = p.CoutP / CP;
    double* partial = reinterpret_cast<double*>(dp->part + (rows * mg * CP * 2 + 1) / 2 * 2);
    hipLaunchKernelGGL(dprelu_finish1_kernel, dim3(kFinishBlocks, mg), dim3(256), 0, st, dp->part, (int)rows, CP, partial);
    hipLaunchKernelGGL(dprelu_finish2_kernel, dim3(dp->nslope + Cout), dim3(64), 0, st, partial, CP, Cout, dp->ga, dp->gb,
                       dp->nslope);
    return hipGetLastError() == hipSuccess ? FS_OK : FS_ERR_LAUNCH;
  };
  const int K3 = kernel * kernel * kernel;
  p.Di = Di; p.Hi = Hi; p.Wi = Wi;
  if (wino2d_ok(p, x, ws, Cin, Cout, kernel, stride, ms != nullptr) &&
      (dp == nullptr || (bias == nullptr && z == nullptr && addend == nullptr))) {
    wprep_do(wprep_job(FS_WPREP_WINO2D, w, ws, (long long)cinp * FS_WINO2D_UCH, Cout, Cin, cinp, wmode), plan, st);
    if (plan != nullptr) return FS_OK;
    const int rc = launch_wino2d(x, ws, bias, y, p, st);
    if (rc != FS_OK || dp == nullptr) return rc;
    return dp_finish(64, wino2d_part_rows());
  }
#ifdef FS_ABLATION
  if (wino4_ok(p, x, ws, Cin, Cout, kernel, stride, ms != nullptr) &&
      (dp == nullptr || (bias == nullptr && z == nullptr && addend == nullptr))) {
    wprep_do(wprep_job(FS_WPREP_WINO4, w, ws, (long long)cinp * FS_WINO4_UCH, Cout, Cin, cinp, wmode), plan, st);
    if (plan != nullptr) return FS_OK;
    const int rc = launch_wino4(x, ws, bias, y, p, st);
    if (rc != FS_OK || dp == nullptr) return rc;
    return dp_finish(64);
  }
  if (wino_ok(p, x, ws, Cin, Cout, kernel, stride, ms != nullptr) &&
      (dp == nullptr || (bias == nullptr && z == nullptr && addend == nullptr))) {
    wprep_do(wprep_job(FS_WPREP_WINO, w, ws, (long long)cinp * FS_WINO_UCH, Cout, Cin, cinp, wmode), plan, st);
    if (plan != nullptr) return FS_OK;
    const int rc = launch_wino(x, ws, bias, y, p, st);
    if (rc != FS_OK || dp == nullptr) return rc;
    return dp_finish(64);
  }
#endif
  static const bool no_s3 = FS_AB_ENV("FLOWSCI_FWD_NO_S3");
  if (!no_s3 && kernel == 4 && stride == 2 && pad == 1 && wmode == 0 && (p.CoutP == 32 || p.CoutP == 64) && Wi % 4 == 0 &&
      ms_aligned && (((ms ? (uintptr_t)0 : (uintptr_t)x) | (uintptr_t)ws) & 15) == 0 &&
      (long long)Di * Hi * Wi * 4 < (1ll << 31) &&
      (long long)B * Do * fs::cdiv(Ho, S3_TY) * fs::cdiv(Wo, S3_TW) >= 256 &&
      (dp == nullptr || (p.CoutP == 32 && bias == nullptr && z == nullptr && addend == nullptr))) {
    const int cp = p.CoutP;
    wprep_do(wprep_job(FS_WPREP_S3K4, w, ws, s3_slab_words(Cin, p.CoutP), Cout, Cin, (Cin + 1) / 2, cp, 0, 0), plan, st);
    if (plan != nullptr) return FS_OK;
    int rc;
#ifdef FS_ABLATION
    static const int s3_nlw = (int)FS_AB_ENV_LL("FLOWSCI_S3_NLW", 4);
    if (s3_nlw == 8) rc = p.CoutP == 32 ? launch_s3<1, S3_NMW, 8>(x, ws, bias, y, p, st) : launch_s3<2, S3_NMW, 8>(x, ws, bias, y, p, st);
    else
#endif
    rc = p.CoutP == 32 ? launch_s3<1, S3_NMW, 4>(x, ws, bias, y, p, st) : launch_s3<2, S3_NMW, 4>(x, ws, bias, y, p, st);
    if (rc != FS_OK || dp == nullptr) return rc;
    return dp_finish(32, S3_NMW);
  }
  wprep_do(wprep_job(FS_WPREP_FWD, w, ws, (long long)cinp * K3 * p.CoutP, Cout, Cin, K3, cinp, p.CoutP, wmode), plan, st);
  if (plan != nullptr) return FS_OK;
  static const bool reg_only = FS_AB_ENV("FLOWSCI_FWD_REG");
  const bool ws_ok = !reg_only && Wi % 4 == 0 && Wo > 16 && (((ms ? (uintptr_t)0 : (uintptr_t)x) | (uintptr_t)ws) & 15) == 0 &&
                     ms_aligned && (long long)(kernel == 3 ? 4 : 2) * Di * Hi * Wi * 4 < (1ll << 31);
  if (ms != nullptr && !(kernel == 4 && ws_ok && dp == nullptr)) return FS_ERR_UNSUPPORTED;
  if (kernel == 3) {
    const bool wide = Wo > 16;
    const long long big = (long long)B * fs::cdiv(Do, 2) * fs::cdiv(Ho, wide ? 8 : 16) * fs::cdiv(Wo, wide ? 32 : 16) *
                          (p.CoutP / 64);
    const bool ws3 = !reg_only && Wi % 4 == 0 && (((ms ? (uintptr_t)0 : (uintptr_t)x) | (uintptr_t)ws) & 15) == 0 &&
                     (long long)4 * Di * Hi * Wi * 4 < (1ll << 31);
    if (dp != nullptr && (bias != nullptr || z != nullptr || addend != nullptr || !ws3)) return FS_ERR_UNSUPPORTED;
    int rc = FS_ERR_UNSUPPORTED, cp = 0;
    const long long small = (long long)B * Do * fs::cdiv(Ho, wide ? 4 : 8) * fs::cdiv(Wo, wide ? 32 : 16) * (p.CoutP / 64);
    if (big >= 512) {
      if (ws3 && wide) { rc = launch_ws<3, 1, 4, 2, 4, 2, 8, 32>(x, ws, bias, y, p, st); cp = 64; }
      else if (dp != nullptr) return FS_ERR_UNSUPPORTED;
      else if (wide) return launch<3, 1, 4, 2, 4, 2, 8, 32>(x, ws, bias, y, p, st);
      else return launch<3, 1, 4, 2, 4, 2, 8, 16>(x, ws, bias, y, p, st);
    } else if (small < 256) {
// ... 142 lines not shown
```

### opticalflowscivis_amd/csrc/convtr.hip

```cpp
#include <cstdint>
#include <cstdlib>

#include "common.hpp"

namespace {

typedef float f32x16 __attribute__((ext_vector_type(16)));

struct TP {
  int B, Cin, Cout;
  int CoutT;
  int Di, Hi, Wi;
  int Dout, Hout, Wout;
  int Dq, Hq, Wq;
  int tz, ty, tx;
  long long tiles;
  const float* slope;
  float* Z;
  int nslope;
  const float* addend;
  const float* Ybase;
  long long wslice;
#ifdef FS_ABLATION
  int ab = 0;
#endif
};

__device__ __forceinline__ void tr_slice(TP& p, const float*& Wt, const float*& bias, float*& Y) {
  const int sl = blockIdx.y;
  if (sl == 0) return;
  const size_t off = (size_t)sl * 32 * ((size_t)p.Dout * p.Hout * p.Wout);
  Wt += (size_t)sl * p.wslice;
  if (bias) bias += 32 * sl;
  Y += off;
  if (p.Z) p.Z += off;
  if (p.slope && p.nslope != 1) p.slope += 32 * sl;
  if (p.addend) p.addend += off;
  p.Ybase += off;
}

__device__ __forceinline__ constexpr int tap_d(int p, int a) { return p == 0 ? (a == 0 ? 0 : -1) : (a == 0 ? 1 : 0); }
__device__ __forceinline__ constexpr int tap_k(int p, int a) { return p == 0 ? (a == 0 ? 1 : 3) : (a == 0 ? 0 : 2); }

#include "wprep.hpp"

__device__ __forceinline__ void store8(float* __restrict__ yc, const float (&v)[8], int qz, int qy, int qx,
                                       const TP& p, float* __restrict__ zc = nullptr, float sl = 0.f) {
  const float* __restrict__ ac = p.addend ? p.addend + (yc - p.Ybase) : nullptr;
#pragma unroll
  for (int pz = 0; pz < 2; ++pz)
#pragma unroll
    for (int py = 0; py < 2; ++py) {
      const int z = 2 * qz + pz, y = 2 * qy + py, x = 2 * qx;
      if (z >= p.Dout || y >= p.Hout || x >= p.Wout) continue;
      float* row = yc + ((size_t)z * p.Hout + y) * p.Wout + x;
      float v0 = v[(pz * 2 + py) * 2], v1 = v[(pz * 2 + py) * 2 + 1];
      if (ac != nullptr) {
        const float* arow = ac + (row - yc);
        v0 += arow[0];
        if (x + 1 < p.Wout) v1 += arow[1];
      }
      if ((p.Wout & 1) == 0) {
        *reinterpret_cast<float2*>(row) = make_float2(v0, v1);
      } else {
        row[0] = v0;
        if (x + 1 < p.Wout) row[1] = v1;
      }
      if (zc != nullptr) {
        float* zrow = zc + (row - yc);
        const float z0 = v0 > 0.f ? v0 : sl * v0, z1 = v1 > 0.f ? v1 : sl * v1;
        if ((p.Wout & 1) == 0) {
          *reinterpret_cast<float2*>(zrow) = make_float2(z0, z1);
        } else {
          zrow[0] = z0;
          if (x + 1 < p.Wout) zrow[1] = z1;
        }
      }
    }
}

__device__ __forceinline__ void store8_quad(float* __restrict__ yc, const float (&v)[8], int qz, int qy, int qx, bool ok,
                                            const TP& p, float* __restrict__ zc = nullptr, float sl = 0.f) {
  const float* __restrict__ ac = p.addend ? p.addend + (yc - p.Ybase) : nullptr;
  const bool evn = (qx & 1) == 0;
#pragma unroll
  for (int pz = 0; pz < 2; ++pz) {
    const float a0 = v[(pz * 2 + 0) * 2], a1 = v[(pz * 2 + 0) * 2 + 1];
    const float b0 = v[(pz * 2 + 1) * 2], b1 = v[(pz * 2 + 1) * 2 + 1];
    const float k0 = evn ? a0 : b0, k1 = evn ? a1 : b1;
    const float r0 = __uint_as_float(__builtin_amdgcn_update_dpp(0u, __float_as_uint(evn ? b0 : a0), 0xB1, 0xF, 0xF, false));
    const float r1 = __uint_as_float(__builtin_amdgcn_update_dpp(0u, __float_as_uint(evn ? b1 : a1), 0xB1, 0xF, 0xF, false));
    float4 o = evn ? make_float4(k0, k1, r0, r1) : make_float4(r0, r1, k0, k1);
    const int z = 2 * qz + pz, y = 2 * qy + (evn ? 0 : 1), x0 = 2 * (evn ? qx : qx - 1);
    if (!ok || z >= p.Dout || y >= p.Hout || x0 >= p.Wout) continue;
    float* row = yc + ((size_t)z * p.Hout + y) * p.Wout + x0;
    if (x0 + 3 < p.Wout) {
      if (ac != nullptr) {
        const float4 a4 = *reinterpret_cast<const float4*>(ac + (row - yc));
        o.x += a4.x; o.y += a4.y; o.z += a4.z; o.w += a4.w;
      }
      *reinterpret_cast<float4*>(row) = o;
      if (zc != nullptr)
        *reinterpret_cast<float4*>(zc + (row - yc)) = make_float4(o.x > 0.f ? o.x : sl * o.x, o.y > 0.f ? o.y : sl * o.y,
                                                                  o.z > 0.f ? o.z : sl * o.z, o.w > 0.f ? o.w : sl * o.w);
    } else {
      const float ov[4] = {o.x, o.y, o.z, o.w};
#pragma unroll
      for (int e = 0; e < 4; ++e)
        if (x0 + e < p.Wout) {
          const float w = ov[e] + (ac != nullptr ? ac[(row - yc) + e] : 0.f);
          row[e] = w;
          if (zc != nullptr) zc[(row - yc) + e] = w > 0.f ? w : sl * w;
        }
    }
  }
}

template <int TZ, int TY>
__global__ __launch_bounds__(256, 2) void convtr_mfma_kernel(const float* __restrict__ X,
                                                          const float* __restrict__ Wt_,
                                                          const float* __restrict__ bias_,
                                                          float* __restrict__ Y_, TP p) {
  const float* Wt = Wt_;
  const float* bias = bias_;
  float* Y = Y_;
  tr_slice(p, Wt, bias, Y);
  static_assert(TZ * TY == 4, "one 32-position row per wave");
  constexpr int CI = 4;
  constexpr int ZT = TZ + 2, YT = TY + 2, XT = 34;
  constexpr int PS = YT * XT, CHS = ZT * PS;
  constexpr int NX = CI * CHS, NW = CI * 64 * 32;
  __shared__ float sX[NX];
  __shared__ __attribute__((aligned(16))) float sW[NW];

  const int t = threadIdx.x, lane = t & 63, wv = t >> 6;
  const int col = lane & 31, kh = lane >> 5;
  long long tile = blockIdx.x;
  {
    const long long per = p.tiles / 8;
    if (per > 0 && tile < per * 8) tile = (tile & 7) * per + (tile >> 3);
  }
  const int txi = (int)(tile % p.tx); tile /= p.tx;
  const int tyi = (int)(tile % p.ty); tile /= p.ty;
  const int tzi = (int)(tile % p.tz);
  const int b = (int)(tile / p.tz);
  const int qz0 = tzi * TZ, qy0 = tyi * TY, qx0 = txi * 32;
  const int wz = wv / TY, wy = wv % TY;

  const float* bB = sX + kh * 2 * CHS + (wz + 1) * PS + (wy + 1) * XT + (col + 1);
  const float* aB = sW + kh * 2 * 64 * 32 + col;

  f32x16 acc[8];
#pragma unroll
  for (int c = 0; c < 8; ++c)
#pragma unroll
    for (int r = 0; r < 16; ++r) acc[c][r] = 0.f;

  const size_t xvol = (size_t)p.Di * p.Hi * p.Wi;
  constexpr int ITX = (NX + 255) / 256, ITW = NW / 4 / 256;
  unsigned xoff[ITX];
#pragma unroll
  for (int it = 0; it < ITX; ++it) {
    const int i = t + 256 * it;
    const int c = i / CHS, r1 = i - c * CHS;
    const int z = r1 / PS, r2 = r1 - z * PS;
    const int y = r2 / XT, x = r2 - y * XT;
    const int gz = qz0 - 1 + z, gy = qy0 - 1 + y, gx = qx0 - 1 + x;
    const bool ok = i < NX && gz >= 0 && gz < p.Di && gy >= 0 && gy < p.Hi && gx >= 0 && gx < p.Wi;
    xoff[it] = ok ? ((unsigned)c * (unsigned)xvol + ((unsigned)gz * p.Hi + gy) * p.Wi + gx) * 4u : ~0u;
  }
  float rX[ITX];
  float4 rW[ITW];
  auto fetch = [&](int c0) {
    const char* xb = reinterpret_cast<const char*>(X + ((size_t)b * p.Cin + c0) * xvol);
#pragma unroll
// ... 719 lines not shown
              }
          };
          t3_bf16x8 ba[2][3], bb[2][3];
          load_b(0, ba[0]);
          if (NT > 1) load_b(1, ba[1]);
#pragma unroll
          for (int n = 0; n < NT; n += 4) {
            if (n + 2 < NT) { load_b(n + 2, bb[0]); if (n + 3 < NT) load_b(n + 3, bb[1]); }
            __builtin_amdgcn_sched_barrier(0);
            mma_pair(n, ba[0], ba[1], n + 1 < NT);
            if (n + 2 < NT) {
              if (n + 4 < NT) { load_b(n + 4, ba[0]); if (n + 5 < NT) load_b(n + 5, ba[1]); }
              __builtin_amdgcn_sched_barrier(0);
              mma_pair(n + 2, bb[0], bb[1], n + 3 < NT);
            }
          }
          done = true;
        }
      }
      if (!done) {
        const float* aB = lds + (size_t)(c0 + kq) * WSCI + col;
        float av[8][RT];
#pragma unroll
        for (int d = 0; d < 8; ++d)
#pragma unroll
          for (int rt = 0; rt < RT; ++rt) av[d][rt] = aB[(d * RT + rt) * 16];
        const float* bB = lds + bBo + buf * NXL;
        float xa[2][8], xb[2][8];
        auto load_x = [&](int n, float (&xn)[8]) {
#pragma unroll
          for (int d = 0; d < 8; ++d) xn[d] = bB[16 * n - ((d >> 2) & 1) * PS - ((d >> 1) & 1) * XP - (d & 1)];
        };
        auto mma_pair = [&](int n, const float (&x0)[8], const float (&x1)[8], bool two) {
#pragma unroll
          for (int d = 0; d < 8; ++d)
#pragma unroll
            for (int rt = 0; rt < RT; ++rt) {
              acc[rt][n] = __builtin_amdgcn_mfma_f32_16x16x4f32(av[d][rt], x0[d], acc[rt][n], 0, 0, 0);
              if (two) acc[rt][n + 1] = __builtin_amdgcn_mfma_f32_16x16x4f32(av[d][rt], x1[d], acc[rt][n + 1], 0, 0, 0);
            }
        };
        if constexpr (RT == 6) {
#pragma unroll
          for (int n = 0; n < NT; n += 2) {
            load_x(n, xa[0]);
            if (n + 1 < NT) load_x(n + 1, xa[1]);
            __builtin_amdgcn_sched_barrier(0);
            mma_pair(n, xa[0], xa[1], n + 1 < NT);
            __builtin_amdgcn_sched_barrier(0);
          }
        } else {
          load_x(0, xa[0]);
          if (NT > 1) load_x(1, xa[1]);
#pragma unroll
          for (int n = 0; n < NT; n += 4) {
            if (n + 2 < NT) { load_x(n + 2, xb[0]); if (n + 3 < NT) load_x(n + 3, xb[1]); }
            __builtin_amdgcn_sched_barrier(0);
            mma_pair(n, xa[0], xa[1], n + 1 < NT);
            if (n + 2 < NT) {
              if (n + 4 < NT) { load_x(n + 4, xa[0]); if (n + 5 < NT) load_x(n + 5, xa[1]); }
              __builtin_amdgcn_sched_barrier(0);
              mma_pair(n + 2, xb[0], xb[1], n + 3 < NT);
            }
          }
        }
      }
      TSTAMP(0);
      __builtin_amdgcn_s_barrier();
      TSTAMP(1);
      buf ^= 1;
    }

    const int qz = qz0 + wz, qy = qy0 + wy;
    if (qz <= p.Di && qy <= p.Hi) {
      const size_t yvol = (size_t)p.Dout * p.Hout * p.Wout;
      const bool evn = (col & 1) == 0;
      const int slot = 4 * (kq & 1) + (evn ? 0 : 1) + 2 * (lane >> 5);
#pragma unroll
      for (int rt = 0; rt < RT; ++rt) {
        const int item = 8 * rt + slot;
        const int pzy = item / p.Cout, co = item - pzy * p.Cout;
        const int zo = 2 * qz - (pzy >> 1), yo = 2 * qy - (pzy & 1);
        const bool iok = item < 4 * p.Cout && zo >= 0 && zo < p.Dout && yo >= 0 && yo < p.Hout;
        const float bv = (bias && iok) ? bias[co] : 0.f;
        float* __restrict__ row = Y + (((size_t)b * p.Cout + (iok ? co : 0)) * p.Dout + (iok ? zo : 0)) * ((size_t)p.Hout * p.Wout) +
                                  (size_t)(iok ? yo : 0) * p.Wout;
        const float* __restrict__ arow = p.addend ? p.addend + (row - Y) : nullptr;
        (void)yvol;
        float4 apre[NT];
        if (arow != nullptr) {
#pragma unroll
          for (int n = 0; n < NT; ++n) {
            const int qa = evn ? q0 + 16 * n + col : q0 + 16 * n + col - 1;
            const int x0 = 2 * qa - 1;
            const bool full = iok && qa >= 1 && qa + 1 < qend && x0 + 3 < p.Wout;
            apre[n] = full ? *reinterpret_cast<const float4*>(arow + x0) : make_float4(0.f, 0.f, 0.f, 0.f);
          }
        }
#pragma unroll
        for (int n = 0; n < NT; ++n) {
          const int q = q0 + 16 * n + col;
          const auto s0 = __builtin_amdgcn_permlane32_swap(__float_as_uint(acc[rt][n][0]), __float_as_uint(acc[rt][n][2]),
                                                           false, false);
          const auto s1 = __builtin_amdgcn_permlane32_swap(__float_as_uint(acc[rt][n][1]), __float_as_uint(acc[rt][n][3]),
                                                           false, false);
          const unsigned keep_e = evn ? s0[0] : s1[0], keep_o = evn ? s0[1] : s1[1];
          const unsigned send_e = evn ? s1[0] : s0[0], send_o = evn ? s1[1] : s0[1];
          const float re = __uint_as_float(__builtin_amdgcn_update_dpp(0u, send_e, 0xB1, 0xF, 0xF, false)) + bv;
          const float ro = __uint_as_float(__builtin_amdgcn_update_dpp(0u, send_o, 0xB1, 0xF, 0xF, false)) + bv;
          const float ke = __uint_as_float(keep_e) + bv, ko = __uint_as_float(keep_o) + bv;
          const int qa = evn ? q : q - 1;
          float4 v = evn ? make_float4(ko, ke, ro, re) : make_float4(ro, re, ko, ke);
          if (iok) {
            const int x0 = 2 * qa - 1;
            const bool full = qa >= 1 && qa + 1 < qend && x0 + 3 < p.Wout;
            if (full) {
              if (arow) { v.x += apre[n].x; v.y += apre[n].y; v.z += apre[n].z; v.w += apre[n].w; }
              *reinterpret_cast<float4*>(row + x0) = v;
            } else {
              const float vv[4] = {v.x, v.y, v.z, v.w};
#pragma unroll
              for (int e = 0; e < 4; ++e) {
                const int x = x0 + e, pos = qa + (e >> 1);
                if (pos >= 0 && pos < qend && x >= 0 && x < p.Wout) row[x] = vv[e] + (arow ? arow[x] : 0.f);
              }
            }
          }
        }
      }
    }
    TSTAMP(2);
  }
#ifdef FS_TR_STAMPS
  if (blockIdx.x == 3 && lane == 0) {
    for (int i = 0; i < 8; ++i) fs_tr_dbg[wv * 8 + i] = dt[i];
    fs_tr_dbg[wv * 8 + 7] = (unsigned long long)(t1 - t0);
  }
#endif
}

static int tr_ncu() {
  static int ncu_of[64] = {};
  int dev = 0;
  if (hipGetDevice(&dev) != hipSuccess || dev < 0 || dev >= 64) dev = 0;
  int ncu = ncu_of[dev];
  if (ncu == 0) {
    int n = 0;
    if (hipDeviceGetAttribute(&n, hipDeviceAttributeMultiprocessorCount, dev) != hipSuccess || n < 1) n = 256;
    ncu_of[dev] = ncu = n;
  }
  return ncu;
}

template <int RT, int NT, int CINP = 32>
void launch_p8(const float* x, const float* ws, const float* bias, float* y, const TP& p, hipStream_t st) {
  const int ncu = tr_ncu();
  const long long nwg = p.tiles < ncu ? p.tiles : ncu;
  const int per = (int)((p.tiles + nwg - 1) / nwg);
  const unsigned grid = (unsigned)((p.tiles + per - 1) / per);
  hipLaunchKernelGGL((convtr_p8_kernel<RT, NT, CINP>), dim3(grid), dim3(512), 0, st, x, ws, bias, y, p, per);
}

template <int CO, int NP>
__global__ __launch_bounds__(256) void convtr_valu_kernel(const float* __restrict__ X, const float* __restrict__ W,
                                                          const float* __restrict__ bias, float* __restrict__ Y,
                                                          TP p) {
  const int Hq2 = (p.Hq + NP - 1) / NP;
  const long long nq = (long long)p.B * p.Dq * Hq2 * p.Wq;
  const long long e = (long long)blockIdx.x * 256 + threadIdx.x;
  if (e >= nq) return;
  const int qx = (int)(e % p.Wq);
  long long r = e / p.Wq;
  const int qy = (int)(r % Hq2) * NP; r /= Hq2;
  const int qz = (int)(r % p.Dq);
  const int b = (int)(r / p.Dq);

  constexpr int NY = NP + 2;
  int off[3 * NY * 3];
#pragma unroll
  for (int dz = 0; dz < 3; ++dz)
#pragma unroll
    for (int dy = 0; dy < NY; ++dy)
#pragma unroll
      for (int dx = 0; dx < 3; ++dx) {
        const int z = qz + dz - 1, y = qy + dy - 1, x = qx + dx - 1;
        const bool ok = z >= 0 && z < p.Di && y >= 0 && y < p.Hi && x >= 0 && x < p.Wi;
        off[(dz * NY + dy) * 3 + dx] = ok ? (z * p.Hi + y) * p.Wi + x : -1;
      }

  float acc[NP][CO][8];
#pragma unroll
  for (int co = 0; co < CO; ++co) {
    const float bv = (bias && co < p.Cout) ? bias[co] : 0.f;
#pragma unroll
    for (int q = 0; q < NP; ++q)
#pragma unroll
      for (int c = 0; c < 8; ++c) acc[q][co][c] = bv;
  }
  const size_t xvol = (size_t)p.Di * p.Hi * p.Wi;
  const float* xc = X + (size_t)b * p.Cin * xvol;
  for (int ci = 0; ci < p.Cin; ++ci, xc += xvol) {
    float xn[3 * NY * 3];
#pragma unroll
    for (int i = 0; i < 3 * NY * 3; ++i) xn[i] = off[i] >= 0 ? xc[off[i]] : 0.f;
    const float* wc = W + (size_t)ci * p.Cout * 64;
#pragma unroll
    for (int co = 0; co < CO; ++co) {
      if (co < p.Cout) {
#pragma unroll
        for (int cls = 0; cls < 8; ++cls) {
          const int pz = cls >> 2, py = (cls >> 1) & 1, px = cls & 1;
#pragma unroll
          for (int tp = 0; tp < 8; ++tp) {
            const int a = tp >> 2, bb = (tp >> 1) & 1, c = tp & 1;
            const int kidx = (tap_k(pz, a) * 4 + tap_k(py, bb)) * 4 + tap_k(px, c);
            const float wv = wc[co * 64 + kidx];
#pragma unroll
            for (int q = 0; q < NP; ++q) {
              const int didx = ((tap_d(pz, a) + 1) * NY + (tap_d(py, bb) + 1 + q)) * 3 + (tap_d(px, c) + 1);
              acc[q][co][cls] = fmaf(xn[didx], wv, acc[q][co][cls]);
            }
          }
        }
      }
    }
  }
  const size_t yvol = (size_t)p.Dout * p.Hout * p.Wout;
#pragma unroll
  for (int q = 0; q < NP; ++q)
#pragma unroll
    for (int co = 0; co < CO; ++co)
      if (co < p.Cout && qy + q < p.Hq)
        store8(Y + ((size_t)b * p.Cout + co) * yvol, acc[q][co], qz, qy + q, qx, p,
               p.Z ? p.Z + ((size_t)b * p.Cout + co) * yvol : nullptr, p.Z ? p.slope[p.nslope == 1 ? 0 : co] : 0.f);
}

template <int CO>
void launch_valu(const float* x, const float* w, const float* bias, float* y, const TP& p, hipStream_t st) {
  constexpr int NP = 2;
  const long long nq = (long long)p.B * p.Dq * ((p.Hq + NP - 1) / NP) * p.Wq;
  hipLaunchKernelGGL((convtr_valu_kernel<CO, NP>), dim3((unsigned)((nq + 255) / 256)), dim3(256), 0, st, x, w, bias,
                     y, p);
}

}

#ifdef FS_TR_STAMPS
extern "C" int fs_debug_tr_stamps(unsigned long long* out) {
  return hipMemcpyFromSymbol(out, HIP_SYMBOL(fs_tr_dbg), sizeof(unsigned long long) * 32) == hipSuccess ? 0 : 1;
}
#endif

extern "C" long long fs_conv3d_tr_ws_floats(int Cin, int Cout) {
  if (Cin < 1 || Cout < 1 || (Cout > 32 && (Cout % 32 != 0 || Cout > 128))) return -1;
  const int slices = Cout > 32 ? Cout / 32 : 1;
  if (Cout > 32) Cout = 32;
  const long long cinp = (Cin + 3) / 4 * 4;
  long long p8 = Cout <= 12 ? cinp * p8_ws_ci(Cout <= 2 ? 1 : (Cout <= 6 ? 3 : 6)) : 0;
  if (Cout <= 6 && cinp <= 32 && p8_split_words((int)cinp, Cout <= 2 ? 1 : 3) > p8) p8 = p8_split_words((int)cinp, Cout <= 2 ? 1 : 3);
  long long cls = Cout <= 6 ? 0 : cinp * 64 * (Cout <= 16 ? 16 : 32);
  if (Cout > 16 && t3_slab_words(Cin) > cls) cls = t3_slab_words(Cin);
  if (Cout <= 16 && t3_slab_words16(Cin) > cls) cls = t3_slab_words16(Cin);
  return (p8 > cls ? p8 : cls) * slices;
}

static int conv3d_tr_slice(const float* x, const float* w, const float* bias, const float* slope, int nslope,
                          const float* addend, float* y, float* z, float* ws, int B, int Cin, int Cout, int Di,
                          int Hi, int Wi, int Dout, int Hout, int Wout, fs_stream_t stream, int CoutT = 0, int slices = 1,
                          WprepPlan* plan = nullptr) {
  FS_REQUIRE_PTR(x);
  if (plan == nullptr) FS_REQUIRE_PTR(y);
  if (z != nullptr && (slope == nullptr || (nslope != 1 && nslope != Cout))) return FS_ERR_ARG;
  if (B < 1 || Cin < 1 || Cout < 1 || Di < 1 || Hi < 1 || Wi < 1) return FS_ERR_SHAPE;
  if (Cout > 32) return FS_ERR_ARG;
  if (CoutT == 0) CoutT = Cout;
  if ((Dout != 2 * Di && Dout != 2 * Di + 1) || (Hout != 2 * Hi && Hout != 2 * Hi + 1) ||
      (Wout != 2 * Wi && Wout != 2 * Wi + 1))
    return FS_ERR_SHAPE;
  if ((long long)Di * Hi * Wi >= (1ll << 31) || (long long)Dout * Hout * Wout >= (1ll << 31))
    return FS_ERR_SHAPE;
  if ((long long)4 * Di * Hi * Wi * 4 >= (1ll << 32)) return FS_ERR_SHAPE;
  TP p;
  p.B = B; p.Cin = Cin; p.Cout = Cout; p.CoutT = CoutT; p.Di = Di; p.Hi = Hi; p.Wi = Wi;
  p.Dout = Dout; p.Hout = Hout; p.Wout = Wout;
  p.Dq = (Dout + 1) / 2; p.Hq = (Hout + 1) / 2; p.Wq = (Wout + 1) / 2;
  p.slope = slope; p.Z = z; p.nslope = nslope;
  p.addend = addend; p.Ybase = y;
  p.wslice = 0;
  hipStream_t st = (hipStream_t)stream;
  if ((long long)B * p.Dq * p.Hq * p.Wq >= (1ll << 31) * 256) return FS_ERR_SHAPE;
  static const bool reg_only = FS_AB_ENV("FLOWSCI_TR_REG");
  static const bool p8_all = FS_AB_ENV("FLOWSCI_TR_P8_ALL");
  static const bool s3_small = FS_AB_ENV("FLOWSCI_TR_S3_SMALL");
  if (!s3_small && Cout <= (p8_all ? 12 : 6) && !reg_only && z == nullptr && ws != nullptr && Cin <= (Cout <= 6 ? 64 : 32) && Dout == 2 * Di && Hout == 2 * Hi &&
      Wout == 2 * Wi && Wi % 4 == 0 && (((uintptr_t)x | (uintptr_t)ws) & 15) == 0 &&
      (long long)4 * Di * Hi * Wi * 4 < (1ll << 31)) {
    const int rt = Cout <= 2 ? 1 : (Cout <= 6 ? 3 : 6);
    const bool wide = Wi > 64 && rt < 6;
    p.tz = fs::cdiv(Di + 1, 2); p.ty = fs::cdiv(Hi + 1, 2); p.tx = fs::cdiv(Wi, wide ? 128 : 64);
    p.tiles = (long long)B * p.tz * p.ty * p.tx;
    if (p.tiles >= 16 && p.tiles < (1ll << 31)) {
      const int cinp = (Cin + 3) / 4 * 4;
      static const bool p8_no_s3 = FS_AB_ENV("FLOWSCI_TR_P8_NO_S3");
      const bool split = Cin <= 32 && rt <= 3 && !p8_no_s3;
#ifdef FS_ABLATION
      if (!split) p.ab = 256;
#endif
      wprep_do(wprep_job(FS_WPREP_P8, w, ws, split ? p8_split_words(cinp, rt) : (long long)cinp * p8_ws_ci(rt), Cin, Cout, cinp, rt,
                         split ? 1 : 0), plan, st);
      if (plan != nullptr) return FS_OK;
      if (Cin > 32) {
        if (rt == 1) { if (wide) launch_p8<1, 9, 64>(x, ws, bias, y, p, st); else launch_p8<1, 5, 64>(x, ws, bias, y, p, st); }
        else { if (wide) launch_p8<3, 9, 64>(x, ws, bias, y, p, st); else launch_p8<3, 5, 64>(x, ws, bias, y, p, st); }
      } else if (rt == 1) { if (wide) launch_p8<1, 9>(x, ws, bias, y, p, st); else launch_p8<1, 5>(x, ws, bias, y, p, st); }
      else if (rt == 3) { if (wide) launch_p8<3, 9>(x, ws, bias, y, p, st); else launch_p8<3, 5>(x, ws, bias, y, p, st); }
      else launch_p8<6, 5>(x, ws, bias, y, p, st);
      FS_LAUNCH_CHECK();
      return FS_OK;
    }
  }
  if (Cout <= 6 && !s3_small) {
    if (plan != nullptr) return FS_OK;
    if (w == nullptr) return FS_ERR_NULLPTR;
    if (Cout == 1) launch_valu<1>(x, w, bias, y, p, st);
    else if (Cout <= 2) launch_valu<2>(x, w, bias, y, p, st);
    else if (Cout <= 4) launch_valu<4>(x, w, bias, y, p, st);
    else launch_valu<6>(x, w, bias, y, p, st);
    FS_LAUNCH_CHECK();
    return FS_OK;
  }
  FS_REQUIRE_PTR(ws);
  const int cinp = (Cin + 3) / 4 * 4;
  p.tz = fs::cdiv(p.Dq, 2); p.ty = fs::cdiv(p.Hq, 2); p.tx = fs::cdiv(p.Wq, 32);
  p.tiles = (long long)B * p.tz * p.ty * p.tx;
  if (p.tiles >= (1ll << 31)) return FS_ERR_SHAPE;
#ifdef FS_ABLATION
  static const int tr_ab = (int)FS_AB_ENV_LL("FLOWSCI_TR_AB", 0);
  p.ab = tr_ab;
#endif
  const bool ws_ok = !reg_only && Wi % 4 == 0 && (((uintptr_t)x | (uintptr_t)ws) & 15) == 0 && p.tiles * slices >= 128 &&
                     (long long)4 * Di * Hi * Wi * 4 < (1ll << 31);
  static const bool no_s3 = FS_AB_ENV("FLOWSCI_TR_NO_S3");
  const long long t3 = (long long)B * fs::cdiv(Di, T3_TZ) * fs::cdiv(Hi, T3_TY) * fs::cdiv(Wi, T3_TW);
  const bool t3_ok = !no_s3 && !reg_only && Dout == 2 * Di && Hout == 2 * Hi && Wout == 2 * Wi && Wi % 4 == 0 &&
                     (((uintptr_t)x | (uintptr_t)ws) & 15) == 0 && (long long)Di * Hi * Wi * 4 < (1ll << 31) &&
                     t3 * slices >= 256 && t3 < (1ll << 31) && (long long)32 * Dout * Hout * Wout * 4 < (1ll << 32);
  if (Cout <= 16) {
    if (t3_ok && slices == 1) {
      wprep_do(wprep_job(FS_WPREP_TRS3_16, w, ws, t3_slab_words16(Cin), Cin, Cout, (Cin + 3) / 4, p.CoutT), plan, st);
      if (plan != nullptr) return FS_OK;
      p.tz = fs::cdiv(Di, T3_TZ); p.ty = fs::cdiv(Hi, T3_TY); p.tx = fs::cdiv(Wi, T3_TW);
      p.tiles = t3;
      const int ncu = tr_ncu();
      const long long gx = ncu < p.tiles ? ncu : p.tiles;
      hipLaunchKernelGGL(convtr_s3_kernel<true>, dim3((unsigned)gx, 1), dim3(64 * (T3_NMW + T3_NLW)), 0, st, x,
                         reinterpret_cast<const unsigned*>(ws), bias, y, p);
      FS_LAUNCH_CHECK();
      return FS_OK;
    }
    wprep_do(wprep_job(FS_WPREP_TR16, w, ws, (long long)cinp * 64 * 16, Cin, Cout, cinp), plan, st);
    if (plan != nullptr) return FS_OK;
    if (ws_ok)
      hipLaunchKernelGGL((convtr_mfma16_ws_kernel<2, 2>), dim3((unsigned)p.tiles), dim3(512), 0, st, x, ws, bias, y, p);
    else
      hipLaunchKernelGGL((convtr_mfma16_kernel<2, 2>), dim3((unsigned)p.tiles), dim3(256), 0, st, x, ws, bias, y, p);
  } else {
    if (t3_ok) {
      p.wslice = t3_slab_words(Cin);
      for (int sl = 0; sl < slices; ++sl)
        wprep_do(wprep_job(FS_WPREP_TRS3, w ? w + (size_t)sl * 32 * 64 : nullptr, ws + (size_t)sl * p.wslice, p.wslice, Cin,
                           Cout, (Cin + 3) / 4, p.CoutT), plan, st);
      if (plan != nullptr) return FS_OK;
      p.tz = fs::cdiv(Di, T3_TZ); p.ty = fs::cdiv(Hi, T3_TY); p.tx = fs::cdiv(Wi, T3_TW);
      p.tiles = t3;
      const int ncu = tr_ncu();
      long long gx = ncu / slices < 1 ? 1 : ncu / slices;
      if (gx > p.tiles) gx = p.tiles;
      hipLaunchKernelGGL(convtr_s3_kernel<false>, dim3((unsigned)gx, slices), dim3(64 * (T3_NMW + T3_NLW)), 0, st, x,
                         reinterpret_cast<const unsigned*>(ws), bias, y, p);
      FS_LAUNCH_CHECK();
      return FS_OK;
    }
    p.wslice = (long long)cinp * 64 * 32;
    for (int sl = 0; sl < slices; ++sl)
      wprep_do(wprep_job(FS_WPREP_TR32, w ? w + (size_t)sl * 32 * 64 : nullptr, ws + (size_t)sl * p.wslice, p.wslice, Cin,
                         Cout, cinp, p.CoutT), plan, st);
    if (plan != nullptr) return FS_OK;
    if (ws_ok)
      hipLaunchKernelGGL((convtr_mfma_ws_kernel<2, 2>), dim3((unsigned)p.tiles, slices), dim3(512), 0, st, x, ws, bias, y, p);
    else
      hipLaunchKernelGGL((convtr_mfma_kernel<2, 2>), dim3((unsigned)p.tiles, slices), dim3(256), 0, st, x, ws, bias, y, p);
  }
  FS_LAUNCH_CHECK();
  return FS_OK;
}

static int conv3d_tr_impl(const float* x, const float* w, const float* bias, const float* slope, int nslope,
                          const float* addend, float* y, float* z, float* ws, int B, int Cin, int Cout, int Di,
                          int Hi, int Wi, int Dout, int Hout, int Wout, fs_stream_t stream, WprepPlan* plan = nullptr) {
  if (plan == nullptr && (((uintptr_t)y | (uintptr_t)z | (uintptr_t)addend) & 15) != 0) return FS_ERR_ARG;
  if (Cout <= 32) return conv3d_tr_slice(x, w, bias, slope, nslope, addend, y, z, ws, B, Cin, Cout, Di, Hi, Wi, Dout, Hout,
                                         Wout, stream, 0, 1, plan);
  if (Cout % 32 != 0 || Cout > 128 || Dout < 1 || Hout < 1 || Wout < 1) return FS_ERR_ARG;
  return conv3d_tr_slice(x, w, bias, slope, nslope == 1 ? 1 : (nslope ? 32 : 0), addend, y, z, ws, B, Cin, 32, Di, Hi, Wi, Dout,
                         Hout, Wout, stream, Cout, Cout / 32, plan);
}

extern "C" int fs_conv3d_tr_wprep_jobs(FsWprepJob* jobs_host, int cap, const float* x, const float* w, float* ws, int B,
                                       int Cin, int Cout, int Di, int Hi, int Wi, int Dout, int Hout, int Wout,
                                       int has_prelu_out) {
  FS_ENTER();
  if (jobs_host == nullptr || w == nullptr) return -FS_ERR_NULLPTR;
  if (cap < 0) return -FS_ERR_ARG;
  WprepPlan plan = {jobs_host, cap, 0};
  static const float one = 1.f;
  float* zdummy = has_prelu_out ? ws : nullptr;
  const int rc = conv3d_tr_impl(x, w, nullptr, has_prelu_out ? &one : nullptr, has_prelu_out ? 1 : 0, nullptr, nullptr,
                                zdummy, ws, B, Cin, Cout, Di, Hi, Wi, Dout, Hout, Wout, nullptr, &plan);
  return rc == FS_OK ? plan.n : -rc;
}

extern "C" int fs_conv3d_tr(const float* x, const float* w, const float* bias, float* y, float* ws, int B,
                            int Cin, int Cout, int Di, int Hi, int Wi, int Dout, int Hout, int Wout,
                            fs_stream_t stream) {
  FS_ENTER();
  return conv3d_tr_impl(x, w, bias, nullptr, 0, nullptr, y, nullptr, ws, B, Cin, Cout, Di, Hi, Wi, Dout, Hout, Wout,
                        stream);
}

extern "C" int fs_conv3d_tr_add(const float* x, const float* w, const float* bias, const float* addend, float* y,
                                float* ws, int B, int Cin, int Cout, int Di, int Hi, int Wi, int Dout, int Hout,
                                int Wout, fs_stream_t stream) {
  FS_ENTER();
  FS_REQUIRE_PTR(addend);
  return conv3d_tr_impl(x, w, bias, nullptr, 0, addend, y, nullptr, ws, B, Cin, Cout, Di, Hi, Wi, Dout, Hout, Wout,
                        stream);
}

extern "C" int fs_conv3d_tr_prelu(const float* x, const float* w, const float* bias, const float* prelu_weight,
                                  float* y, float* z, float* ws, int B, int Cin, int Cout, int Di, int Hi, int Wi,
                                  int Dout, int Hout, int Wout, int num_prelu_weights, fs_stream_t stream) {
  FS_ENTER();
  FS_REQUIRE_PTR(prelu_weight); FS_REQUIRE_PTR(z);
  return conv3d_tr_impl(x, w, bias, prelu_weight, num_prelu_weights, nullptr, y, z, ws, B, Cin, Cout, Di, Hi, Wi,
                        Dout, Hout, Wout, stream);
}
```

### opticalflowscivis_amd/csrc/convtr_s3.hpp

```cpp
#pragma once

typedef __bf16 t3_bf16x8 __attribute__((ext_vector_type(8)));
typedef unsigned t3_u32x4 __attribute__((ext_vector_type(4)));
typedef unsigned t3_u32x2 __attribute__((ext_vector_type(2)));
typedef int t3_i32x4 __attribute__((ext_vector_type(4)));
typedef const volatile __attribute__((address_space(3))) t3_u32x2* t3_lds_v64;

constexpr int T3_TZ = 2, T3_TY = 3, T3_TW = 32;
constexpr int T3_NMW = 8, T3_NLW = 4;
constexpr int T3_ZT = T3_TZ + 2, T3_YT = T3_TY + 2, T3_XP = 40;
constexpr int T3_NROW = T3_ZT * T3_YT;
constexpr int T3_NQ = T3_XP / 4;
constexpr int T3_ROWB = T3_XP * 8;
constexpr int T3_PIECEB = (T3_NROW + 1) * T3_ROWB;
constexpr int T3_INB = 3 * T3_PIECEB;
constexpr int T3_WB32 = 8 * 2 * 3 * 1024;
constexpr int T3_WORDS32 = T3_WB32 / 4;
static_assert(T3_NROW * T3_NQ <= 64 * T3_NLW, "one (row, piece) item per loader lane");

inline long long t3_slab_words(int Cin) { return (long long)((Cin + 3) / 4) * T3_WORDS32; }
constexpr int T3_WB16 = 8 * 3 * 1024;
inline long long t3_slab_words16(int Cin) { return (long long)((Cin + 3) / 4) * (T3_WB16 / 4); }

constexpr int T3_PA[6] = {2, 0, 1, 1, 0, 0}, T3_PB[6] = {0, 2, 1, 0, 1, 0};

__device__ __forceinline__ void t3_split_store(const t3_u32x4 (&ld)[4], unsigned char* dst, int pieceb) {
  const unsigned u[4][4] = {{ld[0].x, ld[0].y, ld[0].z, ld[0].w}, {ld[1].x, ld[1].y, ld[1].z, ld[1].w},
                            {ld[2].x, ld[2].y, ld[2].z, ld[2].w}, {ld[3].x, ld[3].y, ld[3].z, ld[3].w}};
  unsigned h[3][4][2];
#pragma unroll
  for (int i = 0; i < 4; ++i)
#pragma unroll
    for (int cp = 0; cp < 2; ++cp) {
      float ra = __uint_as_float(u[2 * cp][i]), rc = __uint_as_float(u[2 * cp + 1][i]);
      h[0][i][cp] = s3_pack(ra, rc);
      ra -= __uint_as_float(h[0][i][cp] << 16); rc -= __uint_as_float(h[0][i][cp] & 0xffff0000u);
      asm volatile("" : "+v"(ra), "+v"(rc));
      h[1][i][cp] = s3_pack(ra, rc);
      ra -= __uint_as_float(h[1][i][cp] << 16); rc -= __uint_as_float(h[1][i][cp] & 0xffff0000u);
      asm volatile("" : "+v"(ra), "+v"(rc));
      h[2][i][cp] = s3_pack(ra, rc);
    }
#pragma unroll
  for (int pc = 0; pc < 3; ++pc) {
    const t3_u32x4 v0 = {h[pc][0][0], h[pc][0][1], h[pc][1][0], h[pc][1][1]};
    const t3_u32x4 v1 = {h[pc][2][0], h[pc][2][1], h[pc][3][0], h[pc][3][1]};
    *reinterpret_cast<t3_u32x4*>(dst + pc * pieceb) = v0;
    *reinterpret_cast<t3_u32x4*>(dst + pc * pieceb + 16) = v1;
  }
}

template <bool M16>
__global__ __launch_bounds__(64 * (T3_NMW + T3_NLW), 1) void convtr_s3_kernel(const float* __restrict__ X,
                                                                             const unsigned* __restrict__ Ws_,
                                                                             const float* __restrict__ bias_,
                                                                             float* __restrict__ Y_, TP p) {
  constexpr int NMW = T3_NMW, NLW = T3_NLW;
  constexpr int WOFF = 2 * T3_INB;
  constexpr int T3_WB = M16 ? T3_WB16 : T3_WB32;
  [[maybe_unused]] constexpr int T3_WORDS = T3_WB / 4;
  constexpr int NWW = T3_WB / 1024 / NLW;
  constexpr int STG1 = 4 * 256 * 16;
  constexpr int NSTG = M16 ? 2 : 1;
  constexpr int STGB = NSTG * STG1;
  static_assert(WOFF + 2 * T3_WB + STGB + 256 <= 160 * 1024, "the stages fit the CU's LDS");
  __shared__ __attribute__((aligned(16))) unsigned char lds[WOFF + 2 * T3_WB + STGB + 256];
  float* const sBias = reinterpret_cast<float*>(lds + WOFF + 2 * T3_WB + STGB);
  float* const sSlope = sBias + 32;

  const float* wd = reinterpret_cast<const float*>(Ws_);
  const float* bias = bias_;
  float* Y = Y_;
  tr_slice(p, wd, bias, Y);

  const int t = threadIdx.x, lane = t & 63;
  const int wave = __builtin_amdgcn_readfirstlane(t >> 6);
  const int col = lane & 31, kh = lane >> 5;
  const int NS = (p.Cin + 3) / 4;
  const size_t xvol = (size_t)p.Di * p.Hi * p.Wi;
  const int G = gridDim.x;
  int place = blockIdx.x;
  if ((G & 7) == 0) place = (place & 7) * (G >> 3) + (place >> 3);
  const int nbr = (int)((p.tiles - place + G - 1) / G);
  auto brick_origin = [&](int i, int& b, int& qz0, int& qy0, int& qx0) {
    unsigned tile = (unsigned)((long long)i * G + place);
    const int txi = (int)(tile % (unsigned)p.tx); tile /= (unsigned)p.tx;
    const int tyi = (int)(tile % (unsigned)p.ty); tile /= (unsigned)p.ty;
    const int tzi = (int)(tile % (unsigned)p.tz);
    b = __builtin_amdgcn_readfirstlane((int)(tile / (unsigned)p.tz));
    qz0 = __builtin_amdgcn_readfirstlane(tzi * T3_TZ);
    qy0 = __builtin_amdgcn_readfirstlane(tyi * T3_TY);
    qx0 = __builtin_amdgcn_readfirstlane(txi * T3_TW);
  };

  if (wave >= NMW) {
#if defined(__HIP_DEVICE_COMPILE__)
    __builtin_amdgcn_s_setprio(3);
    const unsigned* Ws = reinterpret_cast<const unsigned*>(wd);
    const int lw = wave - NMW;
    const int item = lw * 64 + lane;
    const bool act = item < T3_NROW * T3_NQ;
    const int row = act ? item / T3_NQ : T3_NROW, jq = item % T3_NQ;
    const int zr = row / T3_YT, yr = row - zr * T3_YT;
    const unsigned loff = (unsigned)(row * T3_ROWB + jq * 32);
    const unsigned volB = (unsigned)(xvol * 4u);
    unsigned char* const stg = lds + WOFF + 2 * T3_WB + (lw * 64 + lane) * 16;
    int l_i = 0, l_s = 0, l_b = 0;
    unsigned goffA = DMA_OOB, goffB = DMA_OOB;
    auto l_brick = [&]() {
      int qz0, qy0, qx0;
      brick_origin(l_i, l_b, qz0, qy0, qx0);
      const int gz = qz0 - 1 + zr, gy = qy0 - 1 + yr, gx = qx0 - 4 + 4 * jq;
      const bool ok = act && gz >= 0 && gz < p.Di && gy >= 0 && gy < p.Hi && gx >= 0 && gx + 3 < p.Wi;
      const unsigned v = ok ? (((unsigned)gz * (unsigned)p.Hi + (unsigned)gy) * (unsigned)p.Wi + (unsigned)gx) * 4u : DMA_OOB;
      if (l_i & 1) goffB = v; else goffA = v;
    };
    l_brick();
    auto issue_stage = [&](int sbuf) {
      unsigned char* const dst = lds + WOFF + 2 * T3_WB + sbuf * STG1 + lw * 64 * 16;
#pragma unroll
      for (int c = 0; c < 4; ++c) {
        const int ch = 4 * l_s + c;
        const int chc = ch < p.Cin ? ch : 0;
        const unsigned long long a = (unsigned long long)(X + ((size_t)l_b * p.Cin + chc) * xvol);
        t3_i32x4 r;
        r[0] = __builtin_amdgcn_readfirstlane((int)(unsigned)a);
        r[1] = __builtin_amdgcn_readfirstlane((int)((unsigned)(a >> 32) & 0xffffu));
        r[2] = __builtin_amdgcn_readfirstlane(ch < p.Cin ? (int)volB : 0);
        r[3] = 0x00020000;
        const unsigned m0v = (unsigned)(unsigned long long)(lds_ptr_t)(dst + c * 4096);
        if (l_i & 1)
          asm volatile("s_nop 4\n\ts_mov_b32 m0, %0\n\ts_nop 0\n\tbuffer_load_dwordx4 %1, %2, 0 offen lds" ::"s"(m0v), "v"(goffB), "s"(r) : "memory");
        else
          asm volatile("s_nop 4\n\ts_mov_b32 m0, %0\n\ts_nop 0\n\tbuffer_load_dwordx4 %1, %2, 0 offen lds" ::"s"(m0v), "v"(goffA), "s"(r) : "memory");
      }
    };
    auto advance = [&]() {
      if (++l_s == NS) { l_s = 0; if (l_i + 1 < nbr) { ++l_i; l_brick(); } }
    };
    unsigned woff[NWW];
#pragma unroll
    for (int k = 0; k < NWW; ++k) {
      woff[k] = (unsigned)(1024 * (lw + NLW * k) + 16 * lane);
      asm volatile("" : "+v"(woff[k]));
    }
    auto issue_wdma = [&](int s, int buf) {
      const unsigned* src = Ws + (size_t)s * T3_WORDS;
      __amdgpu_buffer_rsrc_t rw = __builtin_amdgcn_make_buffer_rsrc((void*)src, (short)0, T3_WB, 0x00020000);
      unsigned char* dst = lds + WOFF + buf * T3_WB;
#pragma unroll
      for (int k = 0; k < NWW; ++k) {
        const int i = lw + NLW * k;
        __builtin_amdgcn_raw_ptr_buffer_load_lds(rw, (lds_ptr_t)(dst + 1024 * i), 16, woff[k], 0, 0, 0);
      }
    };
    auto convert = [&](int buf, const t3_u32x4 (&ld)[4]) { t3_split_store(ld, lds + buf * T3_INB + loff, T3_PIECEB); };
    const int total = nbr * NS;
    issue_stage(0);
    if constexpr (NSTG == 2) {
      if (total > 1) { advance(); issue_stage(1); }
    }
    int s = 0;
    for (int g = 0; g < total; ++g) {
      if (NSTG == 2 && g + 1 < total) asm volatile("s_waitcnt vmcnt(4)" ::: "memory");
      else asm volatile("s_waitcnt vmcnt(0)" ::: "memory");
      t3_u32x4 ld[4];
      const unsigned char* sp = stg + (NSTG == 2 ? (g & 1) * STG1 : 0);
#pragma unroll
      for (int c = 0; c < 4; ++c) ld[c] = *reinterpret_cast<const t3_u32x4*>(sp + c * 4096);
      asm volatile("s_waitcnt lgkmcnt(0)" ::: "memory");
      __builtin_amdgcn_sched_barrier(0);
      issue_wdma(s, g & 1);
      const bool more = g + NSTG < total;
      if (more) {
        advance();
        issue_stage(NSTG == 2 ? (g & 1) : 0);
      }
      __builtin_amdgcn_sched_barrier(0);
#ifdef FS_ABLATION
      if (!(p.ab & 32))
#endif
      convert(g & 1, ld);
      if (more) asm volatile("s_waitcnt vmcnt(4)" ::: "memory");
      else asm volatile("s_waitcnt vmcnt(0)" ::: "memory");
      asm volatile("s_waitcnt lgkmcnt(0)" ::: "memory");
      __builtin_amdgcn_s_barrier();
      if (++s == NS) s = 0;
    }
#else
    (void)xvol; (void)NWW;
#endif
    return;
  }

  if constexpr (M16) {
    typedef float t3_f32x4 __attribute__((ext_vector_type(4)));
    const int cg = wave & 3, g = wave >> 2;
    const int pz = cg >> 1, py = cg & 1;
    const int n16 = lane & 15, kq = lane >> 4, ay = kq >> 1, ax = kq & 1;
    if (t < 32) {
      sBias[t] = (bias != nullptr && t < p.Cout) ? bias[t] : 0.f;
      sSlope[t] = (p.Z != nullptr) ? p.slope[p.nslope == 1 ? 0 : (t < p.Cout ? t : 0)] : 0.f;
    }
    const unsigned bO = (unsigned)(((g + 1) * T3_YT + (1 + py - ay)) * T3_ROWB + (n16 + 4 - ax) * 8);
    const unsigned aO = (unsigned)(WOFF + (cg * 2) * 3 * 1024 + (kq * 16 + n16) * 16);
    const int dz0 = pz * T3_YT * T3_ROWB, dz1 = (pz - 1) * T3_YT * T3_ROWB;
    const size_t yvol = (size_t)p.Dout * p.Hout * p.Wout;
    int gs = 0;
    for (int bi = 0; bi < nbr; ++bi) {
      t3_f32x4 acc[2][T3_TY][2];
#pragma unroll
      for (int px = 0; px < 2; ++px)
#pragma unroll
        for (int y = 0; y < T3_TY; ++y)
#pragma unroll
          for (int h = 0; h < 2; ++h) acc[px][y][h] = t3_f32x4{0.f, 0.f, 0.f, 0.f};
      for (int s = 0; s < NS; ++s, ++gs) {
        __builtin_amdgcn_s_barrier();
        const unsigned char* sb = lds + (gs & 1) * T3_INB + bO;
        const unsigned char* sw = lds + (gs & 1) * T3_WB + aO;
#ifdef FS_ABLATION
        if (p.ab & 64) continue;
#endif
        auto read_b = [&](int px, int i, t3_bf16x8 (&bq)[3]) {
          const int y = i >> 1, h = i & 1;
#pragma unroll
          for (int pc = 0; pc < 3; ++pc) {
            const unsigned char* q = sb + pc * T3_PIECEB + y * T3_ROWB + (16 * h + px) * 8;
            const t3_u32x2 lo = *(t3_lds_v64)(lds_ptr_t)(q + dz0), hi = *(t3_lds_v64)(lds_ptr_t)(q + dz1);
            const t3_u32x4 v = {lo.x, lo.y, hi.x, hi.y};
            bq[pc] = __builtin_bit_cast(t3_bf16x8, v);
          }
        };
#pragma unroll
        for (int px = 0; px < 2; ++px) {
          t3_bf16x8 a[3], b0[3], b1[3];
#pragma unroll
          for (int pc = 0; pc < 3; ++pc)
            a[pc] = __builtin_bit_cast(t3_bf16x8, *reinterpret_cast<const t3_u32x4*>(sw + (px * 3 + pc) * 1024));
          read_b(px, 0, b0);
#pragma unroll
          for (int i = 0; i < 2 * T3_TY; i += 2) {
            read_b(px, i + 1, b1);
            __builtin_amdgcn_sched_barrier(0);
#ifdef FS_ABLATION
            if (!(p.ab & 128))
#endif
#pragma unroll
            for (int q6 = 0; q6 < 6; ++q6)
              acc[px][i >> 1][i & 1] = __builtin_amdgcn_mfma_f32_16x16x32_bf16(a[T3_PA[q6]], b0[T3_PB[q6]], acc[px][i >> 1][i & 1], 0, 0, 0);
            if (i + 2 < 2 * T3_TY) read_b(px, i + 2, b0);
            __builtin_amdgcn_sched_barrier(0);
#ifdef FS_ABLATION
            if (!(p.ab & 128))
#endif
#pragma unroll
            for (int q6 = 0; q6 < 6; ++q6)
              acc[px][(i + 1) >> 1][(i + 1) & 1] = __builtin_amdgcn_mfma_f32_16x16x32_bf16(a[T3_PA[q6]], b1[T3_PB[q6]], acc[px][(i + 1) >> 1][(i + 1) & 1], 0, 0, 0);
          }
        }
      }
#ifdef FS_ABLATION
      if (p.ab & 4) continue;
#endif
      int b, qz0, qy0, qx0;
      brick_origin(bi, b, qz0, qy0, qx0);
      const int qz = qz0 + g;
      if (qz >= p.Dq) continue;
      const unsigned yv = (unsigned)yvol;
      const size_t sb0 = (size_t)b * p.CoutT * yvol;
      float* const yb = Y + sb0;
      const float* const ab = p.addend != nullptr ? p.addend + (Y - p.Ybase) + sb0 : nullptr;
      float* const zb = p.Z != nullptr ? p.Z + sb0 : nullptr;
      int kqe = kq;
      asm volatile("" : "+v"(kqe));
      const bool evn = (n16 & 1) == 0;
#pragma unroll
      for (int y = 0; y < T3_TY; ++y) {
        const int qy = qy0 + y;
        if (qy >= p.Hq) break;
#pragma unroll
        for (int h = 0; h < 2; ++h) {
          const int qx = qx0 + 16 * h + n16, qxe = evn ? qx : qx - 1;
          const bool xin = qxe < p.Wq;
          const unsigned lo = 4u * (unsigned)kqe * yv + ((unsigned)(2 * qz + pz) * (unsigned)p.Hout + (unsigned)(2 * qy + py)) * (unsigned)p.Wout + 2u * (unsigned)qxe;
#pragma unroll
          for (int r = 0; r < 4; r += 2) {
            const float a0 = acc[0][y][h][r], a1 = acc[1][y][h][r], b0 = acc[0][y][h][r + 1], b1 = acc[1][y][h][r + 1];
            const float s0 = evn ? b0 : a0, s1 = evn ? b1 : a1;
            const float r0 = __uint_as_float(__builtin_amdgcn_update_dpp(0u, __float_as_uint(s0), 0xB1, 0xF, 0xF, false));
            const float r1 = __uint_as_float(__builtin_amdgcn_update_dpp(0u, __float_as_uint(s1), 0xB1, 0xF, 0xF, false));
            float4 o = evn ? make_float4(a0, a1, r0, r1) : make_float4(r0, r1, b0, b1);
            const int rr = evn ? r : r + 1;
            const int co = 4 * kqe + rr;
            if (co >= p.Cout || !xin) continue;
            const unsigned lo2 = lo + (unsigned)rr * yv;
            const float bv = sBias[co];
            o.x += bv; o.y += bv; o.z += bv; o.w += bv;
            if (ab != nullptr) {
              const float4 a4 = *reinterpret_cast<const float4*>(ab + lo2);
              o.x += a4.x; o.y += a4.y; o.z += a4.z; o.w += a4.w;
            }
            *reinterpret_cast<float4*>(yb + lo2) = o;
            if (zb != nullptr) {
              const float sl = sSlope[co];
              *reinterpret_cast<float4*>(zb + lo2) = make_float4(o.x > 0.f ? o.x : sl * o.x, o.y > 0.f ? o.y : sl * o.y,
                                                                 o.z > 0.f ? o.z : sl * o.z, o.w > 0.f ? o.w : sl * o.w);
            }
          }
        }
      }
    }
    return;
  }
  const int wv = wave;
  if (t < 32) {
    sBias[t] = (bias != nullptr && t < p.Cout) ? bias[t] : 0.f;
    sSlope[t] = (p.Z != nullptr) ? p.slope[p.nslope == 1 ? 0 : (t < p.Cout ? t : 0)] : 0.f;
  }
  const int cg = wv & 3, g = wv >> 2;
  const int pz = cg >> 1, py = cg & 1;
  const unsigned bO = (unsigned)(((g + 1) * T3_YT + (1 + py - kh)) * T3_ROWB + (col + 4) * 8);
  const unsigned aO = (unsigned)(WOFF + (cg * 2) * 2 * 3 * 1024 + (kh * 32 + col) * 16);
  const size_t yvol = (size_t)p.Dout * p.Hout * p.Wout;
  int gs = 0;
  for (int bi = 0; bi < nbr; ++bi) {
    f32x16 acc[2][T3_TY];
#pragma unroll
    for (int px = 0; px < 2; ++px)
#pragma unroll
      for (int y = 0; y < T3_TY; ++y)
#pragma unroll
        for (int r = 0; r < 16; ++r) acc[px][y][r] = 0.f;
    for (int s = 0; s < NS; ++s, ++gs) {
      __builtin_amdgcn_s_barrier();
      const unsigned char* sb = lds + (gs & 1) * T3_INB + bO;
      const unsigned char* sw = lds + (gs & 1) * T3_WB + aO;
#ifdef FS_ABLATION
      if (p.ab & 64) continue;
#endif
#pragma unroll
      for (int az = 0; az < 2; ++az) {
        const int dzr = (pz - az) * T3_YT * T3_ROWB;
        t3_bf16x8 a[2][3];
#pragma unroll
        for (int px = 0; px < 2; ++px)
#pragma unroll
          for (int pc = 0; pc < 3; ++pc)
            a[px][pc] = __builtin_bit_cast(t3_bf16x8, *reinterpret_cast<const t3_u32x4*>(sw + ((px * 2 + az) * 3 + pc) * 1024));
#pragma unroll
        for (int y = 0; y < T3_TY; ++y) {
          t3_u32x2 P[3][3];
#pragma unroll
          for (int pc = 0; pc < 3; ++pc)
#pragma unroll
            for (int d = 0; d < 3; ++d)
              P[pc][d] = *(t3_lds_v64)(lds_ptr_t)(sb + dzr + pc * T3_PIECEB + y * T3_ROWB + (d - 1) * 8);
          t3_bf16x8 bq[2][3];
#pragma unroll
          for (int px = 0; px < 2; ++px)
#pragma unroll
            for (int pc = 0; pc < 3; ++pc) {
              const t3_u32x4 v = {P[pc][px].x, P[pc][px].y, P[pc][px + 1].x, P[pc][px + 1].y};
              bq[px][pc] = __builtin_bit_cast(t3_bf16x8, v);
            }
#ifdef FS_ABLATION
          if (p.ab & 128) continue;
#endif
#pragma unroll
          for (int q = 0; q < 6; ++q)
#pragma unroll
            for (int px = 0; px < 2; ++px)
              acc[px][y] = __builtin_amdgcn_mfma_f32_32x32x16_bf16(a[px][T3_PA[q]], bq[px][T3_PB[q]], acc[px][y], 0, 0, 0);
        }
      }
    }

#ifdef FS_ABLATION
    if (p.ab & 4) continue;
#endif
    int b, qz0, qy0, qx0;
    brick_origin(bi, b, qz0, qy0, qx0);
    const int qz = qz0 + g, qx = qx0 + col;
    if (qz >= p.Dq) continue;
    const unsigned yv = (unsigned)yvol;
    const size_t sb0 = (size_t)b * p.CoutT * yvol;
    float* const yb = Y + sb0;
    const float* const ab = p.addend != nullptr ? p.addend + (Y - p.Ybase) + sb0 : nullptr;
    float* const zb = p.Z != nullptr ? p.Z + sb0 : nullptr;
    int khe = kh;
    asm volatile("" : "+v"(khe));
    const unsigned khv = 4u * (unsigned)khe * yv;
    const bool evn = (col & 1) == 0;
    const int qxe = evn ? qx : qx - 1;
    const bool xin = qxe < p.Wq;
#pragma unroll
    for (int y = 0; y < T3_TY; ++y) {
      const int qy = qy0 + y;
      if (qy >= p.Hq) break;
      const unsigned lo = khv + ((unsigned)(2 * qz + pz) * (unsigned)p.Hout + (unsigned)(2 * qy + py)) * (unsigned)p.Wout + 2u * (unsigned)qxe;
#pragma unroll
      for (int r = 0; r < 16; r += 2) {
        const int cr = (r & 3) + 8 * (r >> 2);
        const float a0 = acc[0][y][r], a1 = acc[1][y][r], b0 = acc[0][y][r + 1], b1 = acc[1][y][r + 1];
        const float s0 = evn ? b0 : a0, s1 = evn ? b1 : a1;
        const float r0 = __uint_as_float(__builtin_amdgcn_update_dpp(0u, __float_as_uint(s0), 0xB1, 0xF, 0xF, false));
        const float r1 = __uint_as_float(__builtin_amdgcn_update_dpp(0u, __float_as_uint(s1), 0xB1, 0xF, 0xF, false));
        float4 o = evn ? make_float4(a0, a1, r0, r1) : make_float4(r0, r1, b0, b1);
        const int crr = evn ? cr : cr + 1;
        const int co = crr + 4 * khe;
        if (co >= p.Cout || !xin) continue;
        const size_t ro = (size_t)cr * yvol;
        const unsigned lo2 = lo + (evn ? 0u : yv);
        const float bv = sBias[co];
        o.x += bv; o.y += bv; o.z += bv; o.w += bv;
        if (ab != nullptr) {
          const float4 a4 = *reinterpret_cast<const float4*>(ab + ro + lo2);
          o.x += a4.x; o.y += a4.y; o.z += a4.z; o.w += a4.w;
        }
        *reinterpret_cast<float4*>(yb + ro + lo2) = o;
        if (zb != nullptr) {
          const float sl = sSlope[co];
          *reinterpret_cast<float4*>(zb + ro + lo2) = make_float4(o.x > 0.f ? o.x : sl * o.x, o.y > 0.f ? o.y : sl * o.y,
                                                                  o.z > 0.f ? o.z : sl * o.z, o.w > 0.f ? o.w : sl * o.w);
        }
      }
    }
  }
}
```

### opticalflowscivis_amd/ifnet.py

```python
import torch
import torch.nn as nn
import torch.nn.functional as F

from . import convgrad, ops

_CONV = {2: nn.Conv2d, 3: convgrad.Conv3d}
_DECONV = {2: nn.ConvTranspose2d, 3: convgrad.ConvTranspose3d}
_INTERP = {2: "bilinear", 3: "trilinear"}


def _conv(nd, cin, cout, kernel_size=3, stride=1, padding=1):
    return convgrad.ConvPReLU(_CONV[nd](cin, cout, kernel_size, stride, padding, bias=True), convgrad.PReLU(cout))


class _Head(nn.Sequential):

    def forward(self, x, addend=None):
        if isinstance(self[0], convgrad.ConvTranspose3d):
            if convgrad.head_fused_ok(self, x, addend):
                return convgrad._HeadFn.apply(x, self[0].weight, self[0].bias, self[1].weight, self[2].weight,
                                              self[2].bias, addend)
            h = convgrad.ConvPReLU.forward(self, x)
            return self[2](h) if addend is None else self[2](h, addend)
        y = self[2](convgrad.ConvPReLU.forward(self, x))
        return y if addend is None else y + addend


def _head(nd, c, cout):
    return _Head(_DECONV[nd](c, c // 2, 4, 2, 1), convgrad.PReLU(c // 2),
                 _DECONV[nd](c // 2, cout, 4, 2, 1))


def _resize(t, factor, mode, mul=1.0):
    if factor == 1:
        return t if mul == 1.0 else t * mul
    if mode == "trilinear":
        return ops.interpolate3d(t, factor, mul)
    return ops.interpolate2d(t, factor, mul)


def _min_spatial(a, b):
    return tuple(min(x, y) for x, y in zip(a.shape[2:], b.shape[2:]))


def _crop(t, spatial):
    if tuple(t.shape[2:]) == tuple(spatial):
        return t
    return t[(slice(None), slice(None)) + tuple(slice(0, s) for s in spatial)]


class IFBlock(nn.Module):

    def __init__(self, nd, in_planes, c=64):
        super().__init__()
        self.nd = nd
        k0 = 3 if nd == 2 else 4
        self.conv0 = nn.Sequential(_conv(nd, in_planes, c // 2, k0, 2, 1),
                                   _conv(nd, c // 2, c, k0, 2, 1))
        self.convblock0 = nn.Sequential(_conv(nd, c, c), _conv(nd, c, c))
        self.convblock1 = nn.Sequential(_conv(nd, c, c), _conv(nd, c, c))
        self.convblock2 = nn.Sequential(_conv(nd, c, c), _conv(nd, c, c))
        self.convblock3 = nn.Sequential(_conv(nd, c, c), _conv(nd, c, c))
        self.conv1 = _head(nd, c, 2 * nd)
        self.conv2 = _head(nd, c, 1)

    def forward(self, x, flow, scale, flow_base=None, mask_base=None, accumulate=False):
        mode = _INTERP[self.nd]
        h0 = None
        scale_x = scale
        if isinstance(x, (tuple, list)):
            if scale == 1 and flow is not None:
                if self.nd == 3:
                    h0 = convgrad.conv_prelu_cat(self.conv0[0], tuple(x) + (flow,))
                if h0 is None:
                    x = torch.cat(tuple(x) + (flow,), 1)
                flow = None
            else:
                xd = ops.interpolate3d_cat(tuple(x), scale) if (self.nd == 3 and x[0].is_cuda and scale in (2, 4)) else None
                if xd is not None:
                    x, scale_x = xd, 1
                else:
                    x = torch.cat(tuple(x), 1)
        if scale_x != 1 and h0 is None:
            x = _resize(x, 1. / scale, mode)
        if flow is not None:
            if scale != 1:
                flow = _resize(flow, 1. / scale, mode, 1. / scale)
            x = torch.cat((x, flow), 1)
        x = self.conv0(x) if h0 is None else self.conv0[1](h0)
        res = convgrad.res_unit if self.nd == 3 else (lambda blk, t: blk(t) + t)
        x = res(self.convblock0, x)
        x = res(self.convblock1, x)
        x = res(self.convblock2, x)
        x = res(self.convblock3, x)
        if accumulate and self.nd == 3 and x.is_cuda and x.dtype == torch.float32 and scale in (1, 2, 4):
            full = tuple(4 * scale * n for n in x.shape[2:])
            if all(b is None or tuple(b.shape[2:]) == full for b in (flow_base, mask_base)):
                if scale == 1:
                    return self.conv1(x, flow_base), self.conv2(x, mask_base), "sum"
                return self.conv1(x), ops.upsample3d_scale_add(self.conv2(x), mask_base, scale, 1.0), "lowres"
        flow = self.conv1(x)
        mask = self.conv2(x)
        if scale != 1:
            flow = _resize(flow, scale, mode, scale)
            mask = _resize(mask, scale, mode)
        return (flow, mask, "delta") if accumulate else (flow, mask)


class IFNet(nn.Module):

    def __init__(self, nd):
        super().__init__()
        assert nd in (2, 3)
        self.nd = nd
        fc = 2 * nd
        c1 = 96 if nd == 2 else 64
        self.block0 = IFBlock(nd, 2, c=128)
        self.block1 = IFBlock(nd, 5 + fc, c=c1)
        self.block2 = IFBlock(nd, 5 + fc, c=64)
        self.block_tea = IFBlock(nd, 6 + fc, c=64)
        self.keep_warped_pair = False
        self.warped_pair = None

    def forward(self, x, scale=(4, 2, 1), timestep=0.5):
        if isinstance(x, (tuple, list)):
            x, gt = x
        else:
            gt = x[:, 2:3] if self.nd == 2 else x[:, 2:]
        img0, img1 = x[:, :1].contiguous(), x[:, 1:2].contiguous()
        gt = gt.contiguous()
        flow_list, merged, mask_list, mask_logits = [], [], [], []
        warped_img0, warped_img1 = img0, img1
        flow = mask = None
        f_in = f_base = f_dist = None
        loss_distill = 0
        stu = [self.block0, self.block1, self.block2]
        for i in range(3):
            if flow is not None:
                sp = _min_spatial(img0, warped_img0)
                img0, img1 = _crop(img0, sp), _crop(img1, sp)
                warped_img0, warped_img1 = _crop(warped_img0, sp), _crop(warped_img1, sp)
                mask, f_in, f_base = _crop(mask, sp), _crop(f_in, sp), _crop(f_base, sp)
                flow_d, mask_d, kind = stu[i]((img0, img1, warped_img0, warped_img1, mask),
                                              f_in, scale[i], f_base, mask, accumulate=True)
            else:
                flow_d, mask_d, kind = stu[i](torch.cat((img0, img1), 1), None, scale[i], accumulate=True)
            warped = None
            aliases = None
            if kind == "lowres":
                full = tuple(scale[i] * n for n in flow_d.shape[2:])
                if all(f <= n for f, n in zip(full, img0.shape[2:])):
                    aliases, w0, w1 = ops.upsample_warp_pair(img0, img1, flow_d, f_base, scale[i])
                    flow = aliases[0]
                    warped = (w0, w1)
                else:
                    flow = ops.upsample3d_scale_add(flow_d, f_base, scale[i], float(scale[i]))
                mask = mask_d
            elif kind == "sum":
                flow, mask = flow_d, mask_d
            elif flow is not None:
                flow = f_base + _crop(flow_d, img0.shape[2:])
                mask = mask + _crop(mask_d, img0.shape[2:])
            else:
                flow, mask = flow_d, mask_d
            if self.nd == 2:
                flow, mask = _crop(flow, img0.shape[2:]), _crop(mask, img0.shape[2:])
            sp = _min_spatial(img0, warped_img0)
            if self.nd == 3:
                flow, mask = _crop(flow, sp), _crop(mask, sp)
                if aliases is not None:
                    aliases = tuple(_crop(a, sp) for a in aliases)
            img0, img1 = _crop(img0, sp), _crop(img1, sp)
            mask_logits.append(mask)
            if warped is None:
                if self.nd == 3:
                    w0, w1, aliases = ops.warp_pair_acc(img0, img1, flow)
                    warped = (w0, w1)
                else:
                    warped = ops.warp_pair(img0, img1, flow)
            f_in, f_base, f_dist = aliases if aliases is not None else (flow, flow, flow)
            warped_img0, warped_img1 = warped
            flow_list.append(f_dist)
            merged.append((warped_img0, warped_img1))
        self.warped_pair = merged[2] if self.keep_warped_pair else None

        if gt.shape[1] == 1:
            sp = _min_spatial(img0, warped_img0)
            img0, img1 = _crop(img0, sp), _crop(img1, sp)
            warped_img0, warped_img1 = _crop(warped_img0, sp), _crop(warped_img1, sp)
            mask, f_in, f_base, gt = _crop(mask, sp), _crop(f_in, sp), _crop(f_base, sp), _crop(gt, sp)
            flow_d, mask_d, kind = self.block_tea(
                (img0, img1, warped_img0, warped_img1, mask, gt), f_in, 1, f_base, mask, accumulate=True)
            if kind == "sum":
                flow_teacher, mask_teacher = flow_d, mask_d
            else:
                flow_teacher, mask_teacher = f_base + _crop(flow_d, sp), mask + _crop(mask_d, sp)
            w0t, w1t = ops.warp_pair(img0, img1, flow_teacher)
            merged_teacher, _ = ops.merge(w0t, w1t, mask_teacher)
        else:
            flow_teacher = None
            merged_teacher = None

        for i in range(3):
            m, sig = ops.merge(merged[i][0], merged[i][1], mask_logits[i])
            mask_list.append(sig)
            merged[i] = _crop(m, _min_spatial(m, gt))
            if gt.shape[1] == 1:
                flow_list[i] = _crop(flow_list[i], flow_teacher.shape[2:])
        if gt.shape[1] == 1:
            ft = flow_teacher.detach()
            if (x.is_cuda and all(m.shape == merged[0].shape == merged_teacher.shape for m in merged) and
                    all(f.shape == ft.shape for f in flow_list)):
                loss_distill = ops.distill_terms3(merged, merged_teacher, gt, flow_list, ft)
            else:
                for i in range(3):
                    loss_distill = loss_distill + ops.distill_term(merged[i], merged_teacher, gt, flow_list[i], ft)
        masks = mask_list if self.nd == 2 else mask_list[2]
        return flow_list, masks, merged, flow_teacher, merged_teacher, loss_distill
```

### opticalflowscivis_amd/ops.py

```python
import ctypes
from fractions import Fraction

import torch

from . import _lib

WARP2D_RIFE, WARP2D_PWC, WARP2D_PHOTO, WARP2D_DILATED = 0, 1, 2, 3


def _stream(t):
    return torch.cuda.current_stream(t.device).cuda_stream


def _need_cuda_f32(name, t, ndim):
    if not isinstance(t, torch.Tensor):
        raise ValueError("%s must be a tensor" % name)
    if t.dtype != torch.float32:
        raise ValueError("%s must be float32, got %s" % (name, t.dtype))
    if t.dim() != ndim:
        raise ValueError("%s must be %d-D, got shape %s" % (name, ndim, tuple(t.shape)))
    if not t.is_cuda:
        raise ValueError("%s must live on a GPU (the HIP hot path has no CPU fallback); got %s" %
                         (name, t.device))
    return t.contiguous()
# ... 1445 lines not shown
                    tab.upload()


class _PrepEntry:
    __slots__ = ("wref", "ws", "jobs", "stamp", "used", "pinned")


_PREP_KEEP_EPOCHS = 8
_PREP_MAX_JOBS = 65535


class _PrepTable:
    def __init__(self, device):
        self.device, self.entries, self.dirty, self.dev_jobs, self.njobs = device, {}, False, None, 0
        self.captured = []

    def _live(self):
        live = []
        for k, e in list(self.entries.items()):
            w = e.wref()
            if w is None:
                del self.entries[k]
                self.dirty = True
            elif e.jobs:
                live.append((e, w))
        return live

    def _evict(self):
        for k, e in list(self.entries.items()):
            if not e.pinned and _prep_epoch - e.used > _PREP_KEEP_EPOCHS:
                del self.entries[k]
                self.dirty = True

    def upload(self):
        self._evict()
        live = self._live()
        jobs = [j for e, _ in live for j in e.jobs]
        if len(jobs) > _PREP_MAX_JOBS:
            jobs = []
        if jobs:
            arr = (_lib.FsWprepJob * len(jobs))(*jobs)
            host = torch.frombuffer(bytearray(bytes(arr)), dtype=torch.uint8).pin_memory()
            self.dev_jobs, self.njobs = host.to(self.device, non_blocking=True), len(jobs)
        else:
            self.dev_jobs, self.njobs = None, 0
        self.dirty = False

    def refresh(self):
        if self.dirty or self.dev_jobs is None:
            if torch.cuda.is_current_stream_capturing():
                return False
            self.upload()
        live = self._live()
        if self.dirty:
            return False
        if not self.njobs:
            return False
        if torch.cuda.is_current_stream_capturing():
            self.captured.append(self.dev_jobs)
            for e, _ in live:
                e.pinned = True
        with torch.cuda.device(self.device):
            _call("fs_conv3d_wprep_batch", self.dev_jobs.data_ptr(), self.njobs,
                  torch.cuda.current_stream(self.device).cuda_stream,
                  algo_bytes=8 * sum(j.total for e, _ in live for j in e.jobs))
        for e, w in live:
            e.stamp = (w._version, _prep_epoch)
        return True


def _prepared(w, nfloats, key, plan):
    if not (_PREP_ON and _prep_depth > 0 and w.is_leaf and w.requires_grad):
        return w.data_ptr(), w.new_empty(max(int(nfloats), 1))
    tab = _prep_tables.get((w.device.type, w.device.index))
    if tab is None:
        tab = _prep_tables[(w.device.type, w.device.index)] = _PrepTable(w.device)
    global _last_prep
    k = (w.data_ptr(), tuple(w.shape)) + key
    e = tab.entries.get(k)
    capturing = torch.cuda.is_current_stream_capturing()
    if e is not None and e.wref() is not None:
        e.used = _prep_epoch
        if capturing and not e.pinned:
            e.pinned = True
            tab.captured.append(e.ws)
    _last_prep = None
    if e is None or e.wref() is None:
        e = _last_prep = _PrepEntry()
        e.wref, e.stamp, e.used, e.pinned = _weakref.ref(w), None, _prep_epoch, capturing
        e.ws = torch.empty(max(int(nfloats), 1), device=w.device, dtype=torch.float32)
        buf = (_lib.FsWprepJob * 4)()
        n = int(plan(buf, 4, e.ws))
        if n < 0 or n > 4:
            raise _lib.FlowsciKernelError("weight re-layout plan failed (%d)" % n)
        e.jobs = [_lib.FsWprepJob.from_buffer_copy(buf[i]) for i in range(n)]
        tab.entries[k] = e
        tab.dirty = True
        if capturing:
            tab.captured.append(e.ws)
        e.stamp = (w._version, _prep_epoch)
        return w.data_ptr(), e.ws
    if not e.jobs:
        return w.data_ptr(), e.ws
    if e.stamp != (w._version, _prep_epoch) and not tab.refresh():
        e.stamp = (w._version, _prep_epoch)
        return w.data_ptr(), e.ws
    return 0, e.ws


_last_prep = None


def _prep_not_written():
    if _last_prep is not None:
        _last_prep.stamp = None


def _prepared_fwd(w, xptr, geo):
    L = _lib.lib()
    return _prepared(w, L.fs_conv3d_fwd_ws_floats(geo[1], geo[2], geo[9]), ("fwd", xptr % 16) + geo,
                     lambda jobs, cap, ws: L.fs_conv3d_fwd_wprep_jobs(jobs, cap, xptr, w.data_ptr(), ws.data_ptr(), *geo))


def conv3d_wrw_supported(k, stride, padding):
    return (len(k) == 3 and k[0] == k[1] == k[2] and stride[0] == stride[1] == stride[2] and
            padding[0] == padding[1] == padding[2] and (k[0], stride[0]) in ((3, 1), (4, 2)) and
            0 <= padding[0] < k[0])


def _vol(dhw):
    return int(dhw[0]) * int(dhw[1]) * int(dhw[2])


def conv3d_fwd_fits(in_dhw, out_dhw, k):
    return (4 if k == 3 else 2) * _vol(in_dhw) * 4 < (1 << 32) and _vol(out_dhw) < (1 << 31)


def conv3d_tr_fits(in_dhw):
    return 4 * _vol(in_dhw) * 4 < (1 << 32) and 8 * _vol(in_dhw) < (1 << 31)


def conv3d_wrw_fits(src_dhw, g_dhw):
    return 8 * _vol(src_dhw) * 4 < (1 << 32) and 64 * _vol(g_dhw) * 4 < (1 << 32)


_dw_arena = {}
_dw_need = {}


def _dw_zeros(like, shape):
    n = 1
    for v in shape:
        n *= int(v)
    if _prep_depth == 0 or not _PREP_ON or torch.cuda.is_current_stream_capturing():
        return like.new_zeros(shape)
    dev = like.device
    st = _dw_arena.get(dev)
    if st is None or st[0] != _prep_epoch:
        if st is not None:
            _dw_need[dev] = st[3]
        need = _dw_need.get(dev, 0)
        st = _dw_arena[dev] = [_prep_epoch, like.new_zeros(need) if need else None, 0, 0]
    pad = (n + 3) // 4 * 4
    st[3] += pad
    if st[1] is None or st[2] + pad > st[1].numel():
        return like.new_zeros(shape)
    out = st[1].narrow(0, st[2], n).view(shape)
    st[2] += pad
    return out


def _conv3d_wrw_det(g, src_ptr, pv, sv, geo, nbytes, acct, allow_unsupported=False):
    L = _lib.lib()
    need = int(L.fs_conv3d_wrw_det_ws_floats(g.data_ptr(), src_ptr, pv, sv, *geo))
    if need == -FS_ERR_UNSUPPORTED and allow_unsupported:
        return None
    if need < 0:
        _lib.check(-need, "fs_conv3d_wrw_det_ws_floats")
    B, Cg, Cs = geo[:3]
    k = geo[9]
    dw = g.new_empty(Cg, Cs, k, k, k)
    ws = g.new_empty(max(need, 1))
    sym, fl, fq = acct
    with torch.cuda.device(g.device):
        _call("fs_conv3d_wrw_det", g.data_ptr(), src_ptr, pv, sv, dw.data_ptr(), ws.data_ptr(), need, *geo, _stream(g),
              algo_bytes=nbytes, algo_flops=fl, equiv_flops=fq, record_as="fs_conv3d_wrw", kernel=sym)
    return dw


def conv3d_wrw(g, src, k, stride, pad):
    g = _need_cuda_f32("g", g, 5)
    src = _need_cuda_f32("src", src, 5)
    B, Cg = g.shape[:2]
    Cs = src.shape[1]
    if src.shape[0] != B:
        raise ValueError("batch mismatch")
    geo = (B, Cg, Cs, g.shape[2], g.shape[3], g.shape[4], src.shape[2], src.shape[3], src.shape[4], int(k), int(stride), int(pad))
    acct = _kernel_accounting("wrw", (g.data_ptr() % 16, src.data_ptr() % 16), *geo)
    if torch.are_deterministic_algorithms_enabled():
        return _conv3d_wrw_det(g, src.data_ptr(), None, None, geo, 4 * (g.numel() + src.numel()), acct)
    dw = _dw_zeros(g, (Cg, Cs, k, k, k))
    sym, fl, fq = acct
    with torch.cuda.device(g.device):
        _call("fs_conv3d_wrw", g.data_ptr(), src.data_ptr(), dw.data_ptr(), *geo, _stream(g),
              algo_bytes=4 * (g.numel() + src.numel()), algo_flops=fl, equiv_flops=fq, kernel=sym)
    return dw


WRW_KERNEL_BRICK, WRW_KERNEL_DMA, WRW_KERNEL_WINO23, WRW_KERNEL_WINO43, WRW_KERNEL_S3 = 0, 1, 2, 3, 4


def conv3d_wrw_kernel_id(g_ptr, src_ptr, B, Cg, Cs, g_dhw, src_dhw, k, stride, pad):
    kid = _plan("wrw", (int(g_ptr) % 16, int(src_ptr) % 16),
                tuple(int(v) for v in (B, Cg, Cs, *g_dhw, *src_dhw, k, stride, pad)))[0]
    if kid < 0:
        _lib.check(-kid, "fs_conv3d_wrw_kernel_id")
    return kid


def conv3d_wrw_takes_winograd(B, Cg, Cs, g_dhw, src_dhw, k, stride, pad, g_misalign=0, src_misalign=0):
    return conv3d_wrw_kernel_id(0x1000 + g_misalign, 0x1000 + src_misalign, B, Cg, Cs, g_dhw, src_dhw, k, stride,
                                pad) in (WRW_KERNEL_WINO23, WRW_KERNEL_WINO43)


FS_ERR_UNSUPPORTED = 5


def _channel_planes(pieces):
    B, dhw = pieces[0].shape[0], tuple(pieces[0].shape[2:])
    vol = dhw[0] * dhw[1] * dhw[2]
    inner = (vol, dhw[1] * dhw[2], dhw[2], 1)
    ptrs, strides = [], []
    for t in pieces:
        if (not isinstance(t, torch.Tensor) or not t.is_cuda or t.dtype != torch.float32 or t.dim() != 5 or
                t.shape[0] != B or tuple(t.shape[2:]) != dhw or tuple(t.stride()[1:]) != inner or
                t.stride(0) < t.shape[1] * vol or t.stride(0) % 4 or t.data_ptr() % 16 or vol % 4):
            return None
        for c in range(t.shape[1]):
            ptrs.append(t.data_ptr() + 4 * c * vol)
            strides.append(t.stride(0))
    n = len(ptrs)
    if n > 12:
        return None
    return (ctypes.c_void_p * n)(*ptrs), (ctypes.c_longlong * n)(*strides), n


def conv3d_fwd_prelu_ms(pieces, w, bias, prelu_weight, k, stride, pad):
    planes = _channel_planes(pieces)
    if planes is None:
        return None
    pv, sv, Cin = planes
    w = _need_cuda_f32("w", w, 5)
    a = _need_cuda_f32("prelu_weight", prelu_weight, 1)
    Cout = w.shape[0]
    if w.shape[1] != Cin or tuple(w.shape[2:]) != (k, k, k):
        raise ValueError("weight %s does not fit %d input channels" % (tuple(w.shape), Cin))
    if bias is not None:
        bias = _need_cuda_f32("bias", bias, 1)
    x0 = pieces[0]
    B = x0.shape[0]
    Di, Hi, Wi = x0.shape[2:]
    Do, Ho, Wo = [(n + 2 * pad - k) // stride + 1 for n in (Di, Hi, Wi)]
    if min(Do, Ho, Wo) < 1:
        return None
    y = x0.new_empty((B, Cout, Do, Ho, Wo))
    z = torch.empty_like(y)
    geo = (B, Cin, Cout, Di, Hi, Wi, Do, Ho, Wo, int(k), int(stride), int(pad), 0)
    wp, ws = _prepared_fwd(w, x0.data_ptr(), geo)
    sym, fl, fq = _kernel_accounting("fwd", (x0.data_ptr() % 16,), *geo)
    xbytes = 4 * B * Cin * Di * Hi * Wi
    with torch.cuda.device(x0.device):
        rc = _call("fs_conv3d_fwd_prelu_ms", pv, sv, wp, _ptr(bias), a.data_ptr(), y.data_ptr(), z.data_ptr(),
                   ws.data_ptr(), B, Cin, Cout, Di, Hi, Wi, Do, Ho, Wo, int(k), int(stride), int(pad), int(a.numel()),
                   _stream(x0), algo_bytes=xbytes + 8 * y.numel(), algo_flops=fl, equiv_flops=fq, kernel=sym,
                   record_as="fs_conv3d_fwd", allow=(FS_ERR_UNSUPPORTED,))
    if rc == FS_ERR_UNSUPPORTED:
        _prep_not_written()
        return None
    return y, z


def conv3d_wrw_ms(g, pieces, k, stride, pad):
    planes = _channel_planes(pieces)
    if planes is None:
        return None
    pv, sv, Cs = planes
    g = _need_cuda_f32("g", g, 5)
    B, Cg = g.shape[:2]
    Di, Hi, Wi = pieces[0].shape[2:]
    geo = (B, Cg, Cs, g.shape[2], g.shape[3], g.shape[4], Di, Hi, Wi, int(k), int(stride), int(pad))
    acct = _kernel_accounting("wrw", (g.data_ptr() % 16, pieces[0].data_ptr() % 16), *geo)
    if torch.are_deterministic_algorithms_enabled():
        return _conv3d_wrw_det(g, 0, pv, sv, geo, 4 * (g.numel() + B * Cs * Di * Hi * Wi), acct, allow_unsupported=True)
    dw = _dw_zeros(g, (Cg, Cs, k, k, k))
    sym, fl, fq = acct
    with torch.cuda.device(g.device):
        rc = _call("fs_conv3d_wrw_ms", g.data_ptr(), pv, sv, dw.data_ptr(), *geo, _stream(g),
                   algo_bytes=4 * (g.numel() + B * Cs * Di * Hi * Wi), algo_flops=fl, equiv_flops=fq, kernel=sym,
                   record_as="fs_conv3d_wrw", allow=(FS_ERR_UNSUPPORTED,))
    if rc == FS_ERR_UNSUPPORTED:
        return None
    return dw


def conv3d_deconv_grad_input_dprelu(gy, w, act_y, prelu_weight):
    gy = _need_cuda_f32("grad_output", gy, 5)
    w = _need_cuda_f32("w", w, 5)
# ... 35 lines not shown
    act_y = _aligned16(_need_cuda_f32("act_y", act_y, 5))
    a = _need_cuda_f32("prelu_weight", prelu_weight, 1)
    B, Cg = gy.shape[:2]
    Cx = w.shape[1]
    if w.shape[0] != Cg or tuple(w.shape[2:]) != (3, 3, 3) or tuple(act_y.shape) != (B, Cx) + tuple(gy.shape[2:]):
        raise ValueError("shapes do not belong to one convolution: %s %s %s" % (tuple(gy.shape), tuple(w.shape), tuple(act_y.shape)))
    if a.numel() not in (1, Cx):
        raise ValueError("prelu_weight must have 1 or %d elements" % Cx)
    D, H, W = gy.shape[2:]
    L = _lib.lib()
    npart = int(L.fs_conv3d_fwd_dprelu_part_floats_k3(B, Cx, D, H, W))
    if npart < 0:
        return None
    out = torch.empty_like(act_y)
    ga, gb = torch.empty_like(a), act_y.new_empty(Cx)
    part = act_y.new_empty(npart)
    geo = (B, Cg, Cx, D, H, W, D, H, W, 3, 1, 1, 1)
    wp, ws = _prepared_fwd(w, gy.data_ptr(), geo)
    sym, fl, fq = _kernel_accounting("fwd", (gy.data_ptr() % 16,), *geo)
    with torch.cuda.device(gy.device):
        rc = _call("fs_conv3d_fwd_dprelu", gy.data_ptr(), wp, act_y.data_ptr(), a.data_ptr(), a.numel(),
                   out.data_ptr(), ga.data_ptr(), gb.data_ptr(), part.data_ptr(), ws.data_ptr(), B, Cg, Cx, D, H, W,
                   D, H, W, 3, 1, 1, _stream(gy), algo_bytes=4 * (gy.numel() + 2 * out.numel()), algo_flops=fl,
                   equiv_flops=fq, kernel=sym, record_as="fs_conv3d_fwd", allow=(FS_ERR_UNSUPPORTED,))
    if rc == FS_ERR_UNSUPPORTED:
        _prep_not_written()
        return None
    return out, ga, gb


def conv3d_fwd_workgroups(B, Cout, out_dhw, k):
    Do, Ho, Wo = out_dhw
    cd = lambda a, b: -(-a // b)
    tw = 32 if Wo > 16 else 16
    r = 32 // tw
    if k == 3:
        mg = cd(Cout, 64)
        big = B * cd(Do, 2) * cd(Ho, 8 * r) * cd(Wo, tw) * mg
        if big >= 512:
            return big
        small = B * Do * cd(Ho, 4 * r) * cd(Wo, tw) * mg
        return small if small >= 256 else 2 * small
    if Cout <= 32:
        return B * Do * cd(Ho, 8 * r) * cd(Wo, tw)
    mg = cd(Cout, 64)
    big = B * cd(Do, 2) * cd(Ho, 8 * r) * cd(Wo, tw) * mg
    if big >= 256:
        return big
    small = B * Do * cd(Ho, 4 * r) * cd(Wo, tw) * mg
    return small if small >= 256 else 2 * small


def conv3d_fwd(x, w, bias, k, stride, pad, wmode=0, prelu_weight=None, addend=None):
    x = _need_cuda_f32("x", x, 5)
    w = _need_cuda_f32("w", w, 5)
    B, Cin = x.shape[:2]
    Cout = w.shape[1] if wmode else w.shape[0]
    if (w.shape[0] if wmode else w.shape[1]) != Cin or tuple(w.shape[2:]) != (k, k, k):
        raise ValueError("weight %s does not fit input %s (wmode %d)" % (tuple(w.shape), tuple(x.shape), wmode))
    if bias is not None:
        bias = _need_cuda_f32("bias", bias, 1)
        if bias.numel() != Cout:
            raise ValueError("bias must have %d elements" % Cout)
    Di, Hi, Wi = x.shape[2:]
    Do, Ho, Wo = [(n + 2 * pad - k) // stride + 1 for n in (Di, Hi, Wi)]
    if min(Do, Ho, Wo) < 1:
        raise ValueError("convolution output is empty for input %s" % (tuple(x.shape),))
    y = x.new_empty((B, Cout, Do, Ho, Wo))
    geo = (B, Cin, Cout, Di, Hi, Wi, Do, Ho, Wo, int(k), int(stride), int(pad), int(wmode))
    wp, ws = _prepared_fwd(w, x.data_ptr(), geo)
    sym, fl, fq = _kernel_accounting("fwd", (x.data_ptr() % 16,), *geo)
    acct = dict(algo_flops=fl, equiv_flops=fq, kernel=sym, record_as="fs_conv3d_fwd")
    nb = 4 * (x.numel() + y.numel())
    if addend is not None:
        addend = _aligned16(_need_cuda_f32("addend", addend, 5))
        if addend.shape != y.shape:
            raise ValueError("addend %s must have the output shape %s" % (tuple(addend.shape), tuple(y.shape)))
        nb += 4 * y.numel()
    with torch.cuda.device(x.device):
        if prelu_weight is None and addend is not None:
            _call("fs_conv3d_fwd_add", x.data_ptr(), wp, _ptr(bias), addend.data_ptr(), y.data_ptr(),
                  ws.data_ptr(), *geo, _stream(x), algo_bytes=nb, **acct)
            return y
        if prelu_weight is None:
            _call("fs_conv3d_fwd", x.data_ptr(), wp, _ptr(bias), y.data_ptr(), ws.data_ptr(), *geo, _stream(x),
                  algo_bytes=nb, **acct)
            return y
        if wmode:
            raise ValueError("the fused PReLU epilogue is forward-only (wmode 0)")
        a = _need_cuda_f32("prelu_weight", prelu_weight, 1)
        if a.numel() not in (1, Cout):
            raise ValueError("prelu_weight must have 1 or %d elements" % Cout)
        z = torch.empty_like(y)
        _call("fs_conv3d_fwd_prelu", x.data_ptr(), wp, _ptr(bias), a.data_ptr(), _ptr(addend),
              y.data_ptr(), z.data_ptr(), ws.data_ptr(), B, Cin, Cout, Di, Hi, Wi, Do, Ho, Wo, int(k), int(stride),
              int(pad), a.numel(), _stream(x), algo_bytes=nb + 4 * y.numel(), **acct)
    return y, z


def conv3d_tr_supported(cout, k, stride, padding):
    return (tuple(k) == (4, 4, 4) and tuple(stride) == (2, 2, 2) and tuple(padding) == (1, 1, 1) and
            (cout <= 32 or (cout % 32 == 0 and cout <= 128)))


def conv3d_tr(x, w, bias, out_dhw=None, prelu_weight=None, addend=None):
    x = _need_cuda_f32("x", x, 5)
    w = _need_cuda_f32("w", w, 5)
    B, Cin = x.shape[:2]
    Cout = w.shape[1]
    if w.shape[0] != Cin or tuple(w.shape[2:]) != (4, 4, 4):
        raise ValueError("weight %s does not fit input %s" % (tuple(w.shape), tuple(x.shape)))
    if bias is not None:
        bias = _need_cuda_f32("bias", bias, 1)
        if bias.numel() != Cout:
            raise ValueError("bias must have %d elements" % Cout)
    Di, Hi, Wi = x.shape[2:]
    Do, Ho, Wo = (2 * Di, 2 * Hi, 2 * Wi) if out_dhw is None else tuple(int(v) for v in out_dhw)
    y = x.new_empty((B, Cout, Do, Ho, Wo))
    nws = int(_lib.lib().fs_conv3d_tr_ws_floats(Cin, Cout))
    if nws < 0:
        raise ValueError("fs_conv3d_tr supports up to 32 output channels or 64 / 96 / 128, got %d" % Cout)
    L = _lib.lib()
    has_z = int(prelu_weight is not None)
    geo = (B, Cin, Cout, Di, Hi, Wi, Do, Ho, Wo, has_z)
    wp, ws = _prepared(w, nws, ("tr",) + geo + (x.data_ptr() % 16,),
                       lambda jobs, cap, slab: L.fs_conv3d_tr_wprep_jobs(jobs, cap, x.data_ptr(), w.data_ptr(),
                                                                        slab.data_ptr(), *geo))
    sym, fl, fq = _kernel_accounting("tr", (x.data_ptr() % 16,), *geo)
    acct = dict(algo_flops=fl, equiv_flops=fq, kernel=sym, record_as="fs_conv3d_tr")
    nb = 4 * (x.numel() + y.numel())
    with torch.cuda.device(x.device):
        if addend is not None:
            if prelu_weight is not None:
                raise ValueError("addend and prelu_weight are mutually exclusive")
            addend = _aligned16(_need_cuda_f32("addend", addend, 5))
            if addend.shape != y.shape:
                raise ValueError("addend %s must have the output shape %s" % (tuple(addend.shape), tuple(y.shape)))
            _call("fs_conv3d_tr_add", x.data_ptr(), wp, _ptr(bias), addend.data_ptr(), y.data_ptr(),
                  ws.data_ptr(), B, Cin, Cout, Di, Hi, Wi, Do, Ho, Wo, _stream(x), algo_bytes=nb + 4 * y.numel(),
                  **acct)
            return y
        if prelu_weight is None:
            _call("fs_conv3d_tr", x.data_ptr(), wp, _ptr(bias), y.data_ptr(), ws.data_ptr(), B, Cin,
                  Cout, Di, Hi, Wi, Do, Ho, Wo, _stream(x), algo_bytes=nb, **acct)
            return y
        a = _need_cuda_f32("prelu_weight", prelu_weight, 1)
        if a.numel() not in (1, Cout):
            raise ValueError("prelu_weight must have 1 or %d elements" % Cout)
        z = torch.empty_like(y)
        _call("fs_conv3d_tr_prelu", x.data_ptr(), wp, _ptr(bias), a.data_ptr(), y.data_ptr(),
              z.data_ptr(), ws.data_ptr(), B, Cin, Cout, Di, Hi, Wi, Do, Ho, Wo, a.numel(), _stream(x),
              algo_bytes=nb + 4 * y.numel(), **acct)
    return y, z


class _WSSIMLoss(torch.autograd.Function):
    @staticmethod
    def forward(ctx, x, y, weight, use_occ):
        x = _need_cuda_f32("x", x, 4)
        y = _need_cuda_f32("y", y, 4)
        weight = _need_cuda_f32("occ_mask", weight, 4)
        B, C, H, W = x.shape
        if y.shape != x.shape or tuple(weight.shape) != (B, 1, H, W):
            raise ValueError("weighted SSIM operands mismatch: %s %s %s" %
                             (tuple(x.shape), tuple(y.shape), tuple(weight.shape)))
        sums = x.new_empty(2)
        ws = x.new_empty(2 * _REDUCE_BLOCKS)
        with torch.cuda.device(x.device):
            _call("fs_wssim_fwd", x.data_ptr(), y.data_ptr(), weight.data_ptr(), sums.data_ptr(),
                  ws.data_ptr(), B, C, H, W, int(bool(use_occ)), _stream(x),
                  algo_bytes=4 * (2 * x.numel() + weight.numel()))
        if use_occ:
            dS1 = 1.0 / (sums[1] + 1e-6)
        else:
            dS1 = torch.full_like(sums[0], 1.0 / float(B * C * (H - 2) * (W - 2)))
        ctx.save_for_backward(x, y, weight, dS1)
        ctx.use_occ = int(bool(use_occ))
        return sums[0] * dS1

    @staticmethod
    def backward(ctx, gout):
        x, y, weight, dS1 = ctx.saved_tensors
        nx, ny = ctx.needs_input_grad[0], ctx.needs_input_grad[1]
        if not (nx or ny):
            return None, None, None, None
        B, C, H, W = x.shape
        coef = (gout * dS1).reshape(1).contiguous()
        gx = torch.empty_like(x) if nx else None
        gy = torch.empty_like(y) if ny else None
        with torch.cuda.device(x.device):
            _call("fs_wssim_bwd", x.data_ptr(), y.data_ptr(), weight.data_ptr(), coef.data_ptr(), _ptr(gx),
                  _ptr(gy), B, C, H, W, ctx.use_occ, _stream(x))
        return gx, gy, None, None


def weighted_ssim_loss(x, y, occ_mask, photo_loss_use_occ):
    return _WSSIMLoss.apply(x, y, occ_mask, bool(photo_loss_use_occ))


def frame_metrics_cost(shape, window="2d"):
    nd = 2 if window == "2d" else 3
    n = 1
    for s in shape:
        n *= int(s)
    lead = int(shape[0]) * int(shape[1])
    valid = lead
    for s in shape[2:]:
        valid *= int(s) - 10
    return 2 * 4 * n, 3 * n + valid * (3 + 5 * 11 * 2 * nd + 15)


def frame_metrics(pred, gt, data_range=1.0, window="2d"):
    if window not in ("2d", "3d"):
        raise ValueError("window must be '2d' or '3d', got %r" % (window,))
    nd = 2 if window == "2d" else 3
    for name, t in (("pred", pred), ("gt", gt)):
        if not isinstance(t, torch.Tensor):
            raise ValueError("%s must be a tensor" % name)
        if not t.is_cuda:
            raise ValueError("%s must live on a GPU (the HIP hot path has no CPU fallback); got %s" % (name, t.device))
        if t.dim() not in (nd + 1, nd + 2):
            raise ValueError("%s must be [N,C,%s] or [N,%s] for window=%r, got shape %s" %
                             (name, ",".join("DHW"[3 - nd:]), ",".join("DHW"[3 - nd:]), window, tuple(t.shape)))
    if pred.shape != gt.shape:
        raise ValueError("pred and gt differ in shape: %s vs %s" % (tuple(pred.shape), tuple(gt.shape)))
    if pred.device != gt.device:
        raise ValueError("pred and gt are on different devices")
    if not float(data_range) > 0:
        raise ValueError("data_range must be > 0, got %r" % (data_range,))
    if pred.dim() == nd + 1:
        pred, gt = pred.unsqueeze(1), gt.unsqueeze(1)
    if any(s < 11 for s in pred.shape[2:]):
        raise ValueError("every filtered extent must be >= 11 (11-tap valid window), got %s" % (tuple(pred.shape),))
    x = pred.to(torch.float32).contiguous()
    y = gt.to(torch.float32).contiguous()
    N, C = x.shape[:2]
    sp = tuple(x.shape[2:])
    if N == 0:
        e = torch.empty(0, dtype=torch.float64, device=x.device)
        return e, e.clone()
    lib = _lib.lib()
    nb = (lib.fs_frame_metrics2d_ws_bytes(N, C, *sp) if nd == 2 else lib.fs_frame_metrics3d_ws_bytes(N, C, *sp))
    if nb < 0:
        _lib.check(int(-nb), "fs_frame_metrics%dd_ws_bytes" % nd)
    ws = torch.empty((nb + 7) // 8, dtype=torch.float64, device=x.device)
    sums = torch.empty(2, N, dtype=torch.float64, device=x.device)
    nbytes, flops = frame_metrics_cost(x.shape, window)
    name = "fs_frame_metrics%dd" % nd
    with torch.cuda.device(x.device):
        _call(name, x.data_ptr(), y.data_ptr(), N, C, *sp, float(data_range), ws.data_ptr(), sums[0].data_ptr(),
              sums[1].data_ptr(), _stream(x), algo_bytes=nbytes, algo_flops=flops)
    L = float(data_range)
    per = C
    for s in sp:
        per *= s
    valid = C
    for s in sp:
        valid *= s - 10
    mse = sums[0] / per
    psnr = 10.0 * torch.log10((L * L) / mse)
    return psnr, sums[1] / valid


FLOW_DISP, FLOW_RIFE3D = 0, 1
_FLOW_CONVENTIONS = {"disp": FLOW_DISP, "rife3d": FLOW_RIFE3D}
FLOW_METRICS_K = 13


def flow_metrics_cost(shape, masks=2, write_map=False):
    n = 1
    for s in shape:
        n *= int(s)
    elems = n // int(shape[1])
    return 2 * 4 * n + masks * elems + (4 * elems if write_map else 0), 60 * elems


def rife3d_to_disp(flow):
    D, H, W = _rife3d_extent(flow)
    d, h, w = _dhw(flow)
    return torch.stack([(h + flow[:, 0]) * ((W - 1) / (H - 1)) - w,
                        (d + flow[:, 1]) * ((H - 1) / (D - 1)) - h,
                        (w + flow[:, 2]) * ((D - 1) / (W - 1)) - d], 1)


def disp_to_rife3d(disp):
    D, H, W = _rife3d_extent(disp)
    d, h, w = _dhw(disp)
    return torch.stack([(w + disp[:, 0]) * ((H - 1) / (W - 1)) - h,
                        (h + disp[:, 1]) * ((D - 1) / (H - 1)) - d,
                        (d + disp[:, 2]) * ((W - 1) / (D - 1)) - w], 1)


def _rife3d_extent(t):
    if not isinstance(t, torch.Tensor) or t.dim() != 5 or t.shape[1] != 3:
        raise ValueError("a 3-D flow must be [N,3,D,H,W], got %s" % (tuple(t.shape) if isinstance(t, torch.Tensor)
                                                                      else type(t).__name__,))
    D, H, W = (int(s) for s in t.shape[2:])
    if min(D, H, W) < 2:
        raise ValueError("the rife3d convention needs every extent >= 2, got %s" % (tuple(t.shape),))
    return D, H, W


def _dhw(t):
    D, H, W = t.shape[2:]
    kw = dict(dtype=t.dtype, device=t.device)
    return (torch.arange(D, **kw).view(1, D, 1, 1), torch.arange(H, **kw).view(1, 1, H, 1),
# ... 1292 lines not shown
```

Before: 31.89.

## Fuse conv0 pair backward: transposed-conv grad-input with PReLU backward epilogue

Adds a custom autograd function for the two-layer conv0 block. Its backward fuses the transposed-conv input gradient of the second conv with the first PReLU's backward inside the s3 kernel epilogue. The epilogue writes the masked gradient and per-block slope/bias partial sums, which two finish kernels then reduce. This avoids materialising the intermediate gradient and running a separate PReLU backward pass, at the cost of more LDS and epilogue work in the transposed-conv kernel. It also removes the stream-capture check in the dw arena allocator and moves the shared finish kernels into a header.

```diff
diff --git a/include/flowsci_hip.h b/include/flowsci_hip.h
--- a/include/flowsci_hip.h
+++ b/include/flowsci_hip.h
@@ -16,7 +16,7 @@
   FS_ERR_UNSUPPORTED = 5
 };
 
-#define FS_ABI_VERSION 460
+#define FS_ABI_VERSION 470
 int fs_version(void);
 const char* fs_error_string(int code);
 
@@ -225,6 +225,11 @@
                        float* y, float* z, float* ws,
                        int B, int Cin, int Cout, int Di, int Hi, int Wi, int Dout, int Hout, int Wout,
                        int num_prelu_weights, fs_stream_t stream);
+long long fs_conv3d_tr_dprelu_part_floats(int B, int Cout, int Di, int Hi, int Wi);
+int fs_conv3d_tr_dprelu(const float* x, const float* w, const float* act_y, const float* prelu_weight,
+                        int num_prelu_weights, float* grad_act_y, float* grad_prelu_weight, float* grad_bias,
+                        float* part, float* ws, int B, int Cin, int Cout, int Di, int Hi, int Wi, int Dout, int Hout,
+                        int Wout, fs_stream_t stream);
 int fs_conv3d_tr_add(const float* x, const float* w, const float* bias, const float* addend, float* y,
                      float* ws, int B, int Cin, int Cout, int Di, int Hi, int Wi,
                      int Dout, int Hout, int Wout, fs_stream_t stream);
diff --git a/opticalflowscivis_amd/_lib.py b/opticalflowscivis_amd/_lib.py
--- a/opticalflowscivis_amd/_lib.py
+++ b/opticalflowscivis_amd/_lib.py
@@ -17,7 +17,7 @@
     return {"library": "ablation build: " + LIB_PATH if ABLATION else "product",
             "env": {k: v for k, v in sorted(os.environ.items()) if k.startswith("FLOWSCI_")}}
 
-ABI_VERSION = 460
+ABI_VERSION = 470
 
 _f32p = ctypes.c_void_p
 _int = ctypes.c_int
@@ -75,6 +75,8 @@
     "fs_conv3d_fwd_prelu": [_f32p] * 8 + [_int] * 13 + [_stream],
     "fs_conv3d_fwd_add": [_f32p] * 6 + [_int] * 13 + [_stream],
     "fs_conv3d_tr_prelu": [_f32p] * 7 + [_int] * 10 + [_stream],
+    "fs_conv3d_tr_dprelu_part_floats": [_int] * 5,
+    "fs_conv3d_tr_dprelu": [_f32p] * 4 + [_int] + [_f32p] * 5 + [_int] * 9 + [_stream],
     "fs_conv3d_tr_add": [_f32p] * 6 + [_int] * 9 + [_stream],
     "fs_conv3d_tr_ws_floats": [_int] * 2,
     "fs_conv3d_tr": [_f32p] * 5 + [_int] * 9 + [_stream],
@@ -186,7 +188,8 @@
              "fs_lic2d_ws_bytes": ctypes.c_longlong, "fs_lic3d_ws_bytes": ctypes.c_longlong,
              "fs_series_stats_ws_bytes": ctypes.c_longlong, "fs_series_encode_ws_bytes": ctypes.c_longlong,
              "fs_conv3d_tr_ws_floats": ctypes.c_longlong, "fs_conv3d_fwd_dprelu_part_floats": ctypes.c_longlong,
-             "fs_conv3d_fwd_dprelu_part_floats_k3": ctypes.c_longlong}
+             "fs_conv3d_fwd_dprelu_part_floats_k3": ctypes.c_longlong,
+             "fs_conv3d_tr_dprelu_part_floats": ctypes.c_longlong}
 
 
 class FlowsciLibraryError(RuntimeError):
diff --git a/opticalflowscivis_amd/convgrad.py b/opticalflowscivis_amd/convgrad.py
--- a/opticalflowscivis_amd/convgrad.py
+++ b/opticalflowscivis_amd/convgrad.py
@@ -250,6 +250,86 @@
                                  *pieces)
 
 
+class _Conv0Fn(torch.autograd.Function):
+
+    @staticmethod
+    def forward(ctx, w_a, b_a, a_a, w_b, b_b, a_b, st_a, pd_a, st_b, pd_b, *pieces):
+        from . import ops
+        res = ops.conv3d_fwd_prelu_ms(pieces, w_a, b_a, a_a, w_a.shape[2], st_a[0], pd_a[0]) if len(pieces) > 1 else None
+        ctx.ms = res is not None
+        if res is None:
+            x = pieces[0] if len(pieces) == 1 else torch.cat(pieces, 1)
+            y_a, z_a = _conv_forward(x, w_a, b_a, st_a, pd_a, False, a_a)
+            src = (x,)
+        else:
+            (y_a, z_a), src = res, pieces
+        y_b, z_b = _conv_forward(z_a, w_b, b_b, st_b, pd_b, False, a_b)
+        ctx.save_for_backward(w_a, y_a, a_a, z_a, w_b, y_b, a_b, *src)
+        ctx.cfg = (st_a, pd_a, st_b, pd_b, b_a is not None, b_b is not None, [int(t.shape[1]) for t in pieces])
+        return z_b
+
+    @staticmethod
+    def backward(ctx, gz):
+        from . import ops
+        w_a, y_a, a_a, z_a, w_b, y_b, a_b = ctx.saved_tensors[:7]
+        src = ctx.saved_tensors[7:]
+        st_a, pd_a, st_b, pd_b, has_ba, has_bb, splits = ctx.cfg
+        gy_b, ga_b, gb_b = ops.prelu_backward(y_b, gz.contiguous(), a_b, want_bias_grad=has_bb)
+        gw_b = _conv_grad_weight(z_a, w_b, gy_b, st_b, pd_b, False) if ctx.needs_input_grad[3] else None
+        k_b = tuple(w_b.shape[2:])
+        fused = None
+        if (k_b == (4, 4, 4) and st_b == (2, 2, 2) and pd_b == (1, 1, 1) and _hip_tr_ok(gy_b, w_b.shape[1], k_b, st_b, pd_b)
+                and all(n == 2 * m for n, m in zip(y_a.shape[2:], gy_b.shape[2:]))):
+            fused = ops.conv3d_tr_grad_input_dprelu(gy_b, w_b, y_a, a_a)
+        if fused is not None:
+            gy_a, ga_a, gb_a = fused
+            if not has_ba:
+                gb_a = None
+        else:
+            gz_a = _conv_grad_input(z_a, w_b, gy_b, st_b, pd_b, False)
+            gy_a, ga_a, gb_a = ops.prelu_backward(y_a, gz_a, a_a, want_bias_grad=has_ba)
+        need = ctx.needs_input_grad[10:]
+        gx = None
+        if any(need):
+            k3 = tuple(w_a.shape[2:])
+            hip = _hip_tr_ok(gy_a, w_a.shape[1], k3, st_a, pd_a) and all(
+                n in (2 * m, 2 * m + 1) for n, m in zip(src[0].shape[2:], gy_a.shape[2:]))
+            gx = _conv_grad_input(src[0] if (hip or not ctx.ms) else torch.cat(src, 1), w_a, gy_a, st_a, pd_a, False)
+        gw_a = None
+        if ctx.needs_input_grad[0]:
+            if ctx.ms:
+                gw_a = ops.conv3d_wrw_ms(gy_a, src, w_a.shape[2], st_a[0], pd_a[0])
+                if gw_a is None:
+                    gw_a = _conv_grad_weight(torch.cat(src, 1), w_a, gy_a, st_a, pd_a, False)
+            else:
+                gw_a = _conv_grad_weight(src[0], w_a, gy_a, st_a, pd_a, False)
+        gp = [None] * len(splits)
+        if gx is not None:
+            gp = [g if n else None for g, n in zip(gx.split(splits, 1), need)]
+        return (gw_a, gb_a, ga_a, gw_b, gb_b, ga_b, None, None, None, None) + tuple(gp)
+
+
+def conv0_pair(block, pieces):
+    x0 = pieces[0]
+    if not (len(block) == 2 and _hip_autograd(x0) and x0.dim() == 5 and x0.dtype == torch.float32
+            and all(isinstance(m, ConvPReLU) and isinstance(m[0], Conv3d) and isinstance(m[1], nn.PReLU) for m in block)):
+        return None
+    for m in block:
+        c = m[0]
+        if not (m[1].weight.numel() in (1, c.out_channels) and c.groups == 1 and _tuple(c.dilation, 3) == (1, 1, 1)
+                and c.padding_mode == "zeros"):
+            return None
+    (c_a, p_a), (c_b, p_b) = block[0], block[1]
+    if len(pieces) > 1:
+        if _ab_env("FLOWSCI_CONV0_CAT") == "1":
+            return None
+        if not (tuple(c_a.weight.shape[2:]) == (4, 4, 4) and _tuple(c_a.stride, 3) == (2, 2, 2)
+                and sum(int(t.shape[1]) for t in pieces) == c_a.in_channels <= 12 and c_a.out_channels <= 32):
+            return None
+    return _Conv0Fn.apply(c_a.weight, c_a.bias, p_a.weight, c_b.weight, c_b.bias, p_b.weight, _tuple(c_a.stride, 3),
+                          _tuple(c_a.padding, 3), _tuple(c_b.stride, 3), _tuple(c_b.padding, 3), *pieces)
+
+
 class _HeadFn(torch.autograd.Function):
 
     @staticmethod
diff --git a/opticalflowscivis_amd/csrc/convfwd.hip b/opticalflowscivis_amd/csrc/convfwd.hip
--- a/opticalflowscivis_amd/csrc/convfwd.hip
+++ b/opticalflowscivis_amd/csrc/convfwd.hip
@@ -420,45 +420,7 @@
   return FS_OK;
 }
 
-constexpr int kFinishBlocks = 128;
-__global__ __launch_bounds__(256) void dprelu_finish1_kernel(const float* __restrict__ part, int rows, int CP,
-                                                             double* __restrict__ partial) {
-  const int CP2 = 2 * CP;
-  const int col = threadIdx.x % CP2, sub = threadIdx.x / CP2, nsub = 256 / CP2;
-  const int chunk = (rows + kFinishBlocks - 1) / kFinishBlocks;
-  const int r0 = blockIdx.x * chunk, r1 = min(rows, r0 + chunk);
-  const float* src = part + (size_t)blockIdx.y * rows * CP2;
-  double s = 0.0;
-  for (int r = r0 + sub; r < r1; r += nsub) s += (double)src[(size_t)r * CP2 + col];
-  __shared__ double red[256];
-  red[threadIdx.x] = s;
-  __syncthreads();
-  if (sub == 0) {
-    double t = red[col];
-    for (int k = 1; k < nsub; ++k) t += red[k * CP2 + col];
-    partial[((size_t)blockIdx.y * kFinishBlocks + blockIdx.x) * CP2 + col] = t;
-  }
-}
-__global__ __launch_bounds__(64) void dprelu_finish2_kernel(const double* __restrict__ partial, int CP, int Cout,
-                                                            float* __restrict__ ga, float* __restrict__ gb, int nslope) {
-  const bool bias_blk = (int)blockIdx.x >= nslope;
-  const int c = bias_blk ? blockIdx.x - nslope : blockIdx.x;
-  const bool all = !bias_blk && nslope == 1 && Cout != 1;
-  const int c_lo = all ? 0 : c, c_hi = all ? Cout : c + 1;
-  double s = 0.0;
-  for (int cc = c_lo; cc < c_hi; ++cc) {
-    const double* src = partial + (size_t)(cc / CP) * kFinishBlocks * 2 * CP + (cc % CP) * 2 + (bias_blk ? 1 : 0);
-    for (int g = threadIdx.x; g < kFinishBlocks; g += 64) s += src[(size_t)g * 2 * CP];
-  }
-  __shared__ double red[64];
-  red[threadIdx.x] = s;
-  __syncthreads();
-  for (int st = 32; st > 0; st >>= 1) {
-    if ((int)threadIdx.x < st) red[threadIdx.x] += red[threadIdx.x + st];
-    __syncthreads();
-  }
-  if (threadIdx.x == 0) (bias_blk ? gb : ga)[c] = (float)red[0];
-}
+#include "dprelu_finish.hpp"
 
 void wt_dims(int Cin, int Cout, int kernel, int* CinP, int* CoutP) {
   const int ci = (kernel == 3) ? 4 : 2;
diff --git a/opticalflowscivis_amd/csrc/convtr.hip b/opticalflowscivis_amd/csrc/convtr.hip
--- a/opticalflowscivis_amd/csrc/convtr.hip
+++ b/opticalflowscivis_amd/csrc/convtr.hip
@@ -21,6 +21,10 @@
   const float* addend;
   const float* Ybase;
   long long wslice;
+  const float* dact = nullptr;
+  const float* dslope = nullptr;
+  int dnslope = 0;
+  float* dpart = nullptr;
 #ifdef FS_ABLATION
   int ab = 0;
 #endif
@@ -1046,6 +1050,17 @@
   return ncu;
 }
 
+#include "dprelu_finish.hpp"
+
+struct TrDPrelu {
+  const float* act_y;
+  const float* slope;
+  int nslope;
+  float* part;
+  float* ga;
+  float* gb;
+};
+
 template <int RT, int NT, int CINP = 32>
 void launch_p8(const float* x, const float* ws, const float* bias, float* y, const TP& p, hipStream_t st) {
   const int ncu = tr_ncu();
@@ -1161,12 +1176,13 @@
 static int conv3d_tr_slice(const float* x, const float* w, const float* bias, const float* slope, int nslope,
                           const float* addend, float* y, float* z, float* ws, int B, int Cin, int Cout, int Di,
                           int Hi, int Wi, int Dout, int Hout, int Wout, fs_stream_t stream, int CoutT = 0, int slices = 1,
-                          WprepPlan* plan = nullptr) {
+                          WprepPlan* plan = nullptr, const TrDPrelu* dp = nullptr) {
   FS_REQUIRE_PTR(x);
   if (plan == nullptr) FS_REQUIRE_PTR(y);
   if (z != nullptr && (slope == nullptr || (nslope != 1 && nslope != Cout))) return FS_ERR_ARG;
   if (B < 1 || Cin < 1 || Cout < 1 || Di < 1 || Hi < 1 || Wi < 1) return FS_ERR_SHAPE;
   if (Cout > 32) return FS_ERR_ARG;
+  if (dp != nullptr && (Cout <= 16 || slices != 1 || bias != nullptr || z != nullptr || addend != nullptr)) return FS_ERR_UNSUPPORTED;
   if (CoutT == 0) CoutT = Cout;
   if ((Dout != 2 * Di && Dout != 2 * Di + 1) || (Hout != 2 * Hi && Hout != 2 * Hi + 1) ||
       (Wout != 2 * Wi && Wout != 2 * Wi + 1))
@@ -1239,6 +1255,7 @@
   const bool t3_ok = !no_s3 && !reg_only && Dout == 2 * Di && Hout == 2 * Hi && Wout == 2 * Wi && Wi % 4 == 0 &&
                      (((uintptr_t)x | (uintptr_t)ws) & 15) == 0 && (long long)Di * Hi * Wi * 4 < (1ll << 31) &&
                      t3 * slices >= 256 && t3 < (1ll << 31) && (long long)32 * Dout * Hout * Wout * 4 < (1ll << 32);
+  if (dp != nullptr && !t3_ok) return FS_ERR_UNSUPPORTED;
   if (Cout <= 16) {
     if (t3_ok && slices == 1) {
       wprep_do(wprep_job(FS_WPREP_TRS3_16, w, ws, t3_slab_words16(Cin), Cin, Cout, (Cin + 3) / 4, p.CoutT), plan, st);
@@ -1270,8 +1287,16 @@
       const int ncu = tr_ncu();
       long long gx = ncu / slices < 1 ? 1 : ncu / slices;
       if (gx > p.tiles) gx = p.tiles;
+      if (dp != nullptr) { p.dact = dp->act_y; p.dslope = dp->slope; p.dnslope = dp->nslope; p.dpart = dp->part; }
       hipLaunchKernelGGL(convtr_s3_kernel<false>, dim3((unsigned)gx, slices), dim3(64 * (T3_NMW + T3_NLW)), 0, st, x,
                          reinterpret_cast<const unsigned*>(ws), bias, y, p);
+      if (dp != nullptr) {
+        const long long rows = gx * T3_DP_ROWS;
+        double* partial = reinterpret_cast<double*>(dp->part + rows * 64);
+        hipLaunchKernelGGL(dprelu_finish1_kernel, dim3(kFinishBlocks, 1), dim3(256), 0, st, dp->part, (int)rows, 32, partial);
+        hipLaunchKernelGGL(dprelu_finish2_kernel, dim3(dp->nslope + Cout), dim3(64), 0, st, partial, 32, Cout, dp->ga, dp->gb,
+                           dp->nslope);
+      }
       FS_LAUNCH_CHECK();
       return FS_OK;
     }
@@ -1331,6 +1356,28 @@
                         stream);
 }
 
+extern "C" long long fs_conv3d_tr_dprelu_part_floats(int B, int Cout, int Di, int Hi, int Wi) {
+  if (B < 1 || Cout < 1 || Cout > 32 || Di < 1 || Hi < 1 || Wi < 1) return -1;
+  const long long t3 = (long long)B * fs::cdiv(Di, T3_TZ) * fs::cdiv(Hi, T3_TY) * fs::cdiv(Wi, T3_TW);
+  const long long ncu = tr_ncu();
+  return (t3 < ncu ? t3 : ncu) * T3_DP_ROWS * 64 + (long long)kFinishBlocks * 64 * 2;
+}
+
+extern "C" int fs_conv3d_tr_dprelu(const float* x, const float* w, const float* act_y, const float* prelu_weight,
+                                   int num_prelu_weights, float* grad_act_y, float* grad_prelu_weight, float* grad_bias,
+                                   float* part, float* ws, int B, int Cin, int Cout, int Di, int Hi, int Wi, int Dout,
+                                   int Hout, int Wout, fs_stream_t stream) {
+  FS_ENTER();
+  FS_REQUIRE_PTR(act_y); FS_REQUIRE_PTR(prelu_weight); FS_REQUIRE_PTR(grad_act_y); FS_REQUIRE_PTR(grad_prelu_weight);
+  FS_REQUIRE_PTR(grad_bias); FS_REQUIRE_PTR(part);
+  if (num_prelu_weights != 1 && num_prelu_weights != Cout) return FS_ERR_ARG;
+  if ((((uintptr_t)grad_act_y | (uintptr_t)act_y | (uintptr_t)part) & 15) != 0) return FS_ERR_ARG;
+  if (Cout > 32) return FS_ERR_UNSUPPORTED;
+  const TrDPrelu dp = {act_y, prelu_weight, num_prelu_weights, part, grad_prelu_weight, grad_bias};
+  return conv3d_tr_slice(x, w, nullptr, nullptr, 0, nullptr, grad_act_y, nullptr, ws, B, Cin, Cout, Di, Hi, Wi, Dout, Hout,
+                         Wout, stream, 0, 1, nullptr, &dp);
+}
+
 extern "C" int fs_conv3d_tr_prelu(const float* x, const float* w, const float* bias, const float* prelu_weight,
                                   float* y, float* z, float* ws, int B, int Cin, int Cout, int Di, int Hi, int Wi,
                                   int Dout, int Hout, int Wout, int num_prelu_weights, fs_stream_t stream) {
diff --git a/opticalflowscivis_amd/csrc/convtr_s3.hpp b/opticalflowscivis_amd/csrc/convtr_s3.hpp
--- a/opticalflowscivis_amd/csrc/convtr_s3.hpp
+++ b/opticalflowscivis_amd/csrc/convtr_s3.hpp
@@ -22,6 +22,10 @@
 constexpr int T3_WB16 = 8 * 3 * 1024;
 inline long long t3_slab_words16(int Cin) { return (long long)((Cin + 3) / 4) * (T3_WB16 / 4); }
 
+constexpr int T3_DP_SLOTS = T3_NMW * 8, T3_DP_SLOTF = 16, T3_DP_ROWS = T3_NMW * 2;
+__host__ __device__ constexpr int t3_dp_slot(int l) { return ((l >> 4) << 1) | (l & 1); }
+__host__ __device__ constexpr int t3_dp_channel(int l, int j) { return 2 * (j & 1) + 8 * (j >> 1) + (l & 1) + 4 * (l >> 5); }
+
 constexpr int T3_PA[6] = {2, 0, 1, 1, 0, 0}, T3_PB[6] = {0, 2, 1, 0, 1, 0};
 
 __device__ __forceinline__ void t3_split_store(const t3_u32x4 (&ld)[4], unsigned char* dst, int pieceb) {
@@ -47,6 +51,70 @@
     const t3_u32x4 v1 = {h[pc][2][0], h[pc][2][1], h[pc][3][0], h[pc][3][1]};
     *reinterpret_cast<t3_u32x4*>(dst + pc * pieceb) = v0;
     *reinterpret_cast<t3_u32x4*>(dst + pc * pieceb + 16) = v1;
+  }
+}
+
+__device__ __forceinline__ void t3_dprelu_epilogue(const f32x16 (&acc)[2][T3_TY], const TP& p, const float* __restrict__ actb,
+                                                   float* __restrict__ yb, const float* sSlope, float4* sSum, bool sum_lane,
+                                                   int khe, unsigned khv, bool evn, bool xin, int qz, int qy0, int qxe,
+                                                   int pz, int py, size_t yvol) {
+  const unsigned yv = (unsigned)yvol;
+  float ga[8], gb[8];
+#pragma unroll
+  for (int j = 0; j < 8; ++j) ga[j] = gb[j] = 0.f;
+#pragma unroll
+  for (int y = 0; y < T3_TY; ++y) {
+    const int qy = qy0 + y;
+    if (qy >= p.Hq) break;
+    const unsigned lo = khv + ((unsigned)(2 * qz + pz) * (unsigned)p.Hout + (unsigned)(2 * qy + py)) * (unsigned)p.Wout + 2u * (unsigned)qxe;
+    const unsigned lo2 = lo + (evn ? 0u : yv);
+    float4 act4[4];
+#pragma unroll
+    for (int r = 0; r < 16; r += 2) {
+      if ((r & 7) == 0) {
+#pragma unroll
+        for (int j = 0; j < 4; ++j) {
+          const int cj = ((r + 2 * j) & 3) + 8 * ((r + 2 * j) >> 2);
+          act4[j] = make_float4(0.f, 0.f, 0.f, 0.f);
+          if ((evn ? cj : cj + 1) + 4 * khe < p.Cout && xin) act4[j] = *reinterpret_cast<const float4*>(actb + (size_t)cj * yvol + lo2);
+        }
+        __builtin_amdgcn_sched_barrier(0);
+      }
+      const int cr = (r & 3) + 8 * (r >> 2);
+      const int co = (evn ? cr : cr + 1) + 4 * khe;
+      const bool ok = co < p.Cout && xin;
+      const size_t ro = (size_t)cr * yvol;
+      const float4 a4 = act4[(r >> 1) & 3];
+      const float a0 = acc[0][y][r], a1 = acc[1][y][r], b0 = acc[0][y][r + 1], b1 = acc[1][y][r + 1];
+      const float s0 = evn ? b0 : a0, s1 = evn ? b1 : a1;
+      const float r0 = __uint_as_float(__builtin_amdgcn_update_dpp(0u, __float_as_uint(s0), 0xB1, 0xF, 0xF, false));
+      const float r1 = __uint_as_float(__builtin_amdgcn_update_dpp(0u, __float_as_uint(s1), 0xB1, 0xF, 0xF, false));
+      if (!ok) continue;
+      const float4 v = evn ? make_float4(a0, a1, r0, r1) : make_float4(r0, r1, b0, b1);
+      const float sl = sSlope[co];
+      const float4 o = make_float4(a4.x > 0.f ? v.x : sl * v.x, a4.y > 0.f ? v.y : sl * v.y,
+                                   a4.z > 0.f ? v.z : sl * v.z, a4.w > 0.f ? v.w : sl * v.w);
+      *reinterpret_cast<float4*>(yb + ro + lo2) = o;
+      ga[r >> 1] += ((a4.x > 0.f ? 0.f : a4.x * v.x) + (a4.y > 0.f ? 0.f : a4.y * v.y)) +
+                    ((a4.z > 0.f ? 0.f : a4.z * v.z) + (a4.w > 0.f ? 0.f : a4.w * v.w));
+      gb[r >> 1] += (o.x + o.y) + (o.z + o.w);
+    }
+  }
+  auto row_sum = [](float s) {
+    s += __uint_as_float(__builtin_amdgcn_update_dpp(0u, __float_as_uint(s), 0x4E, 0xF, 0xF, false));
+    s += __uint_as_float(__builtin_amdgcn_update_dpp(0u, __float_as_uint(s), 0x124, 0xF, 0xF, false));
+    s += __uint_as_float(__builtin_amdgcn_update_dpp(0u, __float_as_uint(s), 0x128, 0xF, 0xF, false));
+    return s;
+  };
+#pragma unroll
+  for (int j = 0; j < 8; ++j) { ga[j] = row_sum(ga[j]); gb[j] = row_sum(gb[j]); }
+  if (sum_lane) {
+#pragma unroll
+    for (int k = 0; k < 4; ++k) {
+      float4 q = sSum[k];
+      q.x += ga[2 * k]; q.y += gb[2 * k]; q.z += ga[2 * k + 1]; q.w += gb[2 * k + 1];
+      sSum[k] = q;
+    }
   }
 }
 
@@ -63,8 +131,9 @@
   constexpr int STG1 = 4 * 256 * 16;
   constexpr int NSTG = M16 ? 2 : 1;
   constexpr int STGB = NSTG * STG1;
-  static_assert(WOFF + 2 * T3_WB + STGB + 256 <= 160 * 1024, "the stages fit the CU's LDS");
-  __shared__ __attribute__((aligned(16))) unsigned char lds[WOFF + 2 * T3_WB + STGB + 256];
+  constexpr int SUMB = M16 ? 0 : T3_DP_SLOTS * T3_DP_SLOTF * 4;
+  static_assert(WOFF + 2 * T3_WB + STGB + 256 + SUMB <= 160 * 1024, "the stages fit the CU's LDS");
+  __shared__ __attribute__((aligned(16))) unsigned char lds[WOFF + 2 * T3_WB + STGB + 256 + SUMB];
   float* const sBias = reinterpret_cast<float*>(lds + WOFF + 2 * T3_WB + STGB);
   float* const sSlope = sBias + 32;
 
@@ -316,7 +385,14 @@
   const int wv = wave;
   if (t < 32) {
     sBias[t] = (bias != nullptr && t < p.Cout) ? bias[t] : 0.f;
-    sSlope[t] = (p.Z != nullptr) ? p.slope[p.nslope == 1 ? 0 : (t < p.Cout ? t : 0)] : 0.f;
+    sSlope[t] = (p.Z != nullptr) ? p.slope[p.nslope == 1 ? 0 : (t < p.Cout ? t : 0)]
+                : (p.dact != nullptr ? p.dslope[p.dnslope == 1 ? 0 : (t < p.Cout ? t : 0)] : 0.f);
+  }
+  float4* const sSum = reinterpret_cast<float4*>(lds + WOFF + 2 * T3_WB + STGB + 256) + (wv * 8 + t3_dp_slot(lane)) * (T3_DP_SLOTF / 4);
+  const bool sum_lane = (lane & 14) == 0;
+  if (p.dact != nullptr && sum_lane) {
+#pragma unroll
+    for (int k = 0; k < T3_DP_SLOTF / 4; ++k) sSum[k] = make_float4(0.f, 0.f, 0.f, 0.f);
   }
   const int cg = wv & 3, g = wv >> 2;
   const int pz = cg >> 1, py = cg & 1;
@@ -394,6 +470,10 @@
     const bool evn = (col & 1) == 0;
     const int qxe = evn ? qx : qx - 1;
     const bool xin = qxe < p.Wq;
+    if (p.dact != nullptr) {
+      t3_dprelu_epilogue(acc, p, p.dact + sb0, yb, sSlope, sSum, sum_lane, khe, khv, evn, xin, qz, qy0, qxe, pz, py, yvol);
+      continue;
+    }
 #pragma unroll
     for (int y = 0; y < T3_TY; ++y) {
       const int qy = qy0 + y;
@@ -427,4 +507,10 @@
       }
     }
   }
+  if (p.dact != nullptr && sum_lane) {
+    float2* const dst = reinterpret_cast<float2*>(p.dpart) + (((size_t)blockIdx.x * T3_NMW + wv) * 2 + ((lane >> 4) & 1)) * 32;
+    const float2* const src = reinterpret_cast<const float2*>(sSum);
+#pragma unroll
+    for (int j = 0; j < 8; ++j) dst[t3_dp_channel(lane, j)] = src[j];
+  }
 }
diff --git a/opticalflowscivis_amd/csrc/dprelu_finish.hpp b/opticalflowscivis_amd/csrc/dprelu_finish.hpp
--- /dev/null
+++ b/opticalflowscivis_amd/csrc/dprelu_finish.hpp
@@ -0,0 +1,41 @@
+#pragma once
+
+constexpr int kFinishBlocks = 128;
+__global__ __launch_bounds__(256) void dprelu_finish1_kernel(const float* __restrict__ part, int rows, int CP,
+                                                             double* __restrict__ partial) {
+  const int CP2 = 2 * CP;
+  const int col = threadIdx.x % CP2, sub = threadIdx.x / CP2, nsub = 256 / CP2;
+  const int chunk = (rows + kFinishBlocks - 1) / kFinishBlocks;
+  const int r0 = blockIdx.x * chunk, r1 = min(rows, r0 + chunk);
+  const float* src = part + (size_t)blockIdx.y * rows * CP2;
+  double s = 0.0;
+  for (int r = r0 + sub; r < r1; r += nsub) s += (double)src[(size_t)r * CP2 + col];
+  __shared__ double red[256];
+  red[threadIdx.x] = s;
+  __syncthreads();
+  if (sub == 0) {
+    double t = red[col];
+    for (int k = 1; k < nsub; ++k) t += red[k * CP2 + col];
+    partial[((size_t)blockIdx.y * kFinishBlocks + blockIdx.x) * CP2 + col] = t;
+  }
+}
+__global__ __launch_bounds__(64) void dprelu_finish2_kernel(const double* __restrict__ partial, int CP, int Cout,
+                                                            float* __restrict__ ga, float* __restrict__ gb, int nslope) {
+  const bool bias_blk = (int)blockIdx.x >= nslope;
+  const int c = bias_blk ? blockIdx.x - nslope : blockIdx.x;
+  const bool all = !bias_blk && nslope == 1 && Cout != 1;
+  const int c_lo = all ? 0 : c, c_hi = all ? Cout : c + 1;
+  double s = 0.0;
+  for (int cc = c_lo; cc < c_hi; ++cc) {
+    const double* src = partial + (size_t)(cc / CP) * kFinishBlocks * 2 * CP + (cc % CP) * 2 + (bias_blk ? 1 : 0);
+    for (int g = threadIdx.x; g < kFinishBlocks; g += 64) s += src[(size_t)g * 2 * CP];
+  }
+  __shared__ double red[64];
+  red[threadIdx.x] = s;
+  __syncthreads();
+  for (int st = 32; st > 0; st >>= 1) {
+    if ((int)threadIdx.x < st) red[threadIdx.x] += red[threadIdx.x + st];
+    __syncthreads();
+  }
+  if (threadIdx.x == 0) (bias_blk ? gb : ga)[c] = (float)red[0];
+}
diff --git a/opticalflowscivis_amd/ifnet.py b/opticalflowscivis_amd/ifnet.py
--- a/opticalflowscivis_amd/ifnet.py
+++ b/opticalflowscivis_amd/ifnet.py
@@ -66,13 +66,15 @@
 
     def forward(self, x, flow, scale, flow_base=None, mask_base=None, accumulate=False):
         mode = _INTERP[self.nd]
-        h0 = None
+        h0 = h1 = None
         scale_x = scale
         if isinstance(x, (tuple, list)):
             if scale == 1 and flow is not None:
                 if self.nd == 3:
-                    h0 = convgrad.conv_prelu_cat(self.conv0[0], tuple(x) + (flow,))
-                if h0 is None:
+                    h1 = convgrad.conv0_pair(self.conv0, tuple(x) + (flow,))
+                    if h1 is None:
+                        h0 = convgrad.conv_prelu_cat(self.conv0[0], tuple(x) + (flow,))
+                if h0 is None and h1 is None:
                     x = torch.cat(tuple(x) + (flow,), 1)
                 flow = None
             else:
@@ -87,7 +89,12 @@
             if scale != 1:
                 flow = _resize(flow, 1. / scale, mode, 1. / scale)
             x = torch.cat((x, flow), 1)
-        x = self.conv0(x) if h0 is None else self.conv0[1](h0)
+        if h1 is None and h0 is None and self.nd == 3:
+            h1 = convgrad.conv0_pair(self.conv0, (x,))
+        if h1 is not None:
+            x = h1
+        else:
+            x = self.conv0(x) if h0 is None else self.conv0[1](h0)
         res = convgrad.res_unit if self.nd == 3 else (lambda blk, t: blk(t) + t)
         x = res(self.convblock0, x)
         x = res(self.convblock1, x)
diff --git a/opticalflowscivis_amd/ops.py b/opticalflowscivis_amd/ops.py
--- a/opticalflowscivis_amd/ops.py
+++ b/opticalflowscivis_amd/ops.py
@@ -1621,7 +1621,7 @@
     n = 1
     for v in shape:
         n *= int(v)
-    if _prep_depth == 0 or not _PREP_ON or torch.cuda.is_current_stream_capturing():
+    if _prep_depth == 0 or not _PREP_ON:
         return like.new_zeros(shape)
     dev = like.device
     st = _dw_arena.get(dev)
@@ -1963,6 +1963,43 @@
               z.data_ptr(), ws.data_ptr(), B, Cin, Cout, Di, Hi, Wi, Do, Ho, Wo, a.numel(), _stream(x),
               algo_bytes=nb + 4 * y.numel(), **acct)
     return y, z
+
+
+def conv3d_tr_grad_input_dprelu(gy, w, act_y, prelu_weight):
+    gy = _need_cuda_f32("grad_output", gy, 5)
+    w = _need_cuda_f32("w", w, 5)
+    act_y = _need_cuda_f32("act_y", act_y, 5)
+    a = _need_cuda_f32("prelu_weight", prelu_weight, 1)
+    B, Cg = gy.shape[:2]
+    Cx = w.shape[1]
+    Di, Hi, Wi = gy.shape[2:]
+    Do, Ho, Wo = act_y.shape[2:]
+    if w.shape[0] != Cg or tuple(w.shape[2:]) != (4, 4, 4) or tuple(act_y.shape[:2]) != (B, Cx):
+        raise ValueError("shapes do not belong to one convolution: %s %s %s" % (tuple(gy.shape), tuple(w.shape), tuple(act_y.shape)))
+    if a.numel() not in (1, Cx):
+        raise ValueError("prelu_weight must have 1 or %d elements" % Cx)
+    L = _lib.lib()
+    nws = int(L.fs_conv3d_tr_ws_floats(Cg, Cx))
+    npart = int(L.fs_conv3d_tr_dprelu_part_floats(B, Cx, Di, Hi, Wi))
+    if nws < 0 or npart < 0 or act_y.data_ptr() % 16:
+        return None
+    out = torch.empty_like(act_y)
+    ga, gb = torch.empty_like(a), act_y.new_empty(Cx)
+    part = act_y.new_empty(max(npart, 4))
+    geo = (B, Cg, Cx, Di, Hi, Wi, Do, Ho, Wo, 0)
+    wp, ws = _prepared(w, nws, ("tr",) + geo + (gy.data_ptr() % 16,),
+                       lambda jobs, cap, slab: L.fs_conv3d_tr_wprep_jobs(jobs, cap, gy.data_ptr(), w.data_ptr(),
+                                                                        slab.data_ptr(), *geo))
+    sym, fl, fq = _kernel_accounting("tr", (gy.data_ptr() % 16,), *geo)
+    with torch.cuda.device(gy.device):
+        rc = _call("fs_conv3d_tr_dprelu", gy.data_ptr(), wp, act_y.data_ptr(), a.data_ptr(), a.numel(), out.data_ptr(),
+                   ga.data_ptr(), gb.data_ptr(), part.data_ptr(), ws.data_ptr(), B, Cg, Cx, Di, Hi, Wi, Do, Ho, Wo,
+                   _stream(gy), algo_bytes=4 * (gy.numel() + 2 * out.numel()), algo_flops=fl, equiv_flops=fq, kernel=sym,
+                   record_as="fs_conv3d_tr", allow=(FS_ERR_UNSUPPORTED,))
+    if rc == FS_ERR_UNSUPPORTED:
+        _prep_not_written()
+        return None
+    return out, ga, gb
 
 
 class _WSSIMLoss(torch.autograd.Function):
```

Result: no change. 32.15, median of 6 (+0.8%).
